# kalenforn/clip-based-cross-modal-hash

Hardware: AMD Instinct MI355X
Metric: Hamming query x gallery pairs/sec (fused mAP@all pass, DCMHT COCO-shaped 64-bit) (higher is better)
Workload: dtype u32; 1 GPU; configs[1] DCMHT COCO 64-bit retrieval: Q=5000 queries x R=117218 gallery items per GPU (x1 GPUs, contiguous shards), K=64 bits, C=80 classes, mAP@all; Q=5000, R_per_gpu=117218, K=64, C=80, parallelism=gallery-shard x1, query_blocks=1

## Files before the change

clip-based-cross-modal-hash_amd/csrc/xmh_scan.hip:

```cpp
#include "xmh_common.h"
#include <atomic>
#include <math.h>
#include <mutex>
#include <string.h>
#include <vector>
#include "xmh_scan_bits.h"
#include "xmh_scan_mfma.h"
#include "xmh_scan_kernels.h"

#include <stdlib.h>
#include <type_traits>

namespace {

constexpr int kSlotBudget64 = 9 * 1024;
constexpr int kSlotBudget32 = 5 * 1024;
constexpr int slots_for(int W, bool tern, int counter_bytes) {
    const int nbmax = (tern ? 64 : 32) * W + 1;
    const int budget = counter_bytes == 8 ? kSlotBudget64 : kSlotBudget32;
    const int cap = W > 8 ? 64 : 8;
    int S = 2;
    while (S < cap && nbmax * (64 / S) * counter_bytes > budget) S *= 2;
    return S;
}
inline int instance_words(int W) { return W <= 1 ? 1 : (W <= 2 ? 2 : (W <= 4 ? 4 : (W <= 8 ? 8 : (W <= 16 ? 16 : (W <= 32 ? 32 : 64))))); }
constexpr bool pair_cache_shape(int W, bool tern) { return !tern && (W == 1 || W == 2 || W == 4 || W == 8); }
template <int W, bool TERN>
constexpr bool kPairCacheShape = pair_cache_shape(W, TERN);
constexpr int cache_slots(int W) { return W <= 2 ? 4 : 8; }
static_assert(slots_for(2, false, 4) == 4 && slots_for(2, false, 8) == 4 && slots_for(4, false, 4) == 8 && slots_for(4, false, 8) == 8 &&
              slots_for(8, false, 4) == 8 && slots_for(8, false, 8) == 8, "33..256 bits: the cache geometry is the uncached kernels' own");
constexpr int waves_for(int W, bool tern) { return (W >= 32 && !tern) ? 8 : 1; }
inline size_t aos_ring_bytes(int W, int LW, bool tern) { return (size_t)64 * (((W * (tern ? 2 : 1) + LW) + 3) / 4 * 4) * 4; }

struct WsLayout {
    size_t chunk_hist, below, tot, dpre, cap, tick, gate, ap_part, pair_cache, total;
};

bool r2_selfcheck_ok();
inline bool mfma_env_on() {
    const char* e = getenv("XMH_SCAN_MFMA");
    return !(e && atoi(e) == 0);
}
struct Overrides {
    int mfma = -1;
    bool masked = false;
    bool describe = false;
};
enum class Family { kValu, kR2, kR2w, kBits, kTBits };
Family pass1_family(int K, bool ternary, const Overrides& ov) {
    if (ov.mfma == 0 || !mfma_env_on()) return Family::kValu;
    if (ternary) return K <= 256 ? Family::kTBits : Family::kValu;
    if (K > 128) return K <= 256 ? Family::kBits : Family::kValu;
    if (ov.mfma < 0 && !r2_selfcheck_ok()) return Family::kValu;
    return K <= 64 ? Family::kR2 : Family::kR2w;
}
inline int tbits_tiles(int K) { return K <= 64 ? 2 : (K <= 128 ? 4 : 8); }
inline int ap_r2_mode() {
    const char* e = getenv("XMH_SCAN_AP_R2");
    return e ? (atoi(e) != 0 ? 1 : 0) : 2;
}
constexpr int kAp2Waves = 4, kAp2Groups = 2;
constexpr int kMfmaWaves = 4;
static_assert(xmh::kScanBitsWaves == kMfmaWaves, "k_scan_hist_b takes the plan's query tiles of 64");
constexpr int kBitsMaxChunk = 24192;
struct R2Geom { int nw, nq, blocks_per_cu; int queries() const { return nw * nq * 16; } };
inline R2Geom r2_geom(int K) { return K <= 32 ? R2Geom{4, 4, 1} : (K <= 64 ? R2Geom{4, 4, 2} : R2Geom{4, 2, 2}); }

inline long long cache_cap_mb() {
    const char* cap_env = getenv("XMH_SCAN_CACHE_MB");
    return cap_env ? atoll(cap_env) : 131072;
}
inline bool ap_c_on() {
    const char* e = getenv("XMH_SCAN_AP_C");
    return !(e && atoi(e) == 0);
}
size_t pair_cache_bytes(const xmh_scan_plan& p, int K, bool ternary, Family f) {
    const long long cap_mb = cache_cap_mb();
    const bool tb = f == Family::kTBits;
    if ((ternary && !tb) || K > 256 || cap_mb <= 0 || (!tb && K <= 32 && f != Family::kR2)) return 0;
    if (f == Family::kR2 && ap_r2_mode() == 1) return 0;
    const int S = tb ? 8 : (K <= 64 ? 4 : 8);
    const size_t bytes = (size_t)p.nchunk * (size_t)(p.nqtile * S) * (size_t)((p.chunk + 63) / 64) * (S == 4 ? 1024 : 64 * 4 * xmh::kCache12Dwords);
    return bytes <= (size_t)cap_mb << 20 ? bytes : 0;
}

WsLayout ws_layout(const xmh_scan_plan& p, size_t cache_bytes) {
    WsLayout L;
    const size_t cells = (size_t)p.nchunk * p.nbuckets * p.qpad;
    size_t o = 0;
    auto take = [&](size_t bytes) {
        const size_t at = o;
        o += (bytes + 255) & ~(size_t)255;
        return at;
    };
    L.chunk_hist = take(cells * 4);
    L.below = take(cells * 8);
    L.tot = take((size_t)p.nbuckets * p.qpad * 8);
    L.dpre = take((size_t)p.nbuckets * p.qpad * 8);
    L.cap = take((size_t)p.qpad * 4);
    L.tick = take((size_t)p.nqtile * 4);
    L.gate = take(256 + 8 * 4096);
    L.ap_part = take((size_t)p.nchunk * p.qpad * 4);
    L.pair_cache = take(cache_bytes);
    L.total = o;
    return L;
}

size_t cache_for_workspace(const xmh_scan_plan& p, int K, bool ternary, Family f, size_t ws_bytes) {
    const size_t c = pair_cache_bytes(p, K, ternary, f);
    return c && ws_bytes < ws_layout(p, c).total ? 0 : c;
}

int make_plan(int64_t Q, int64_t R, int K, int ternary, xmh_scan_plan* p, const Overrides& ov = {}) {
    if (Q <= 0 || R <= 0 || K <= 0) return xmh::fail(XMH_EINVAL, "scan plan: bad shape Q=%lld R=%lld K=%d", (long long)Q, (long long)R, K);
    if (R >= (1ll << 24) || Q >= (1ll << 24)) return xmh::fail(XMH_ENOTSUP, "scan plan: shard too large (R=%lld, Q=%lld)", (long long)R, (long long)Q);
    const int64_t nb = ternary ? 2 * (int64_t)K + 1 : (int64_t)K + 1;
    const int Wd = (K + 31) / 32;
    if (Wd > 64 || (ternary && Wd > 8))
        return xmh::fail(XMH_ENOTSUP, "scan plan: K=%d%s (at most 2048 code bits, 256 with zero planes)", K, ternary ? " ternary" : "");
    const int S64 = slots_for(instance_words(Wd), ternary != 0, 8);
    const int64_t lds_ap = nb * (64 / S64) * 8;
    if (lds_ap > 150 * 1024) return xmh::fail(XMH_ENOTSUP, "scan plan: %lld distance buckets need %lld B of LDS per wave; K=%d%s", (long long)nb, (long long)lds_ap, K, ternary ? " ternary" : "");
    const Family fam = pass1_family(K, ternary != 0, ov);
    const bool r2 = fam == Family::kR2 || fam == Family::kR2w;
    int64_t nqt = xmh::ceil_div(Q, 64);
    const int r2q = r2_geom(K).queries();
    if (r2) {
        int64_t l = r2q;
        while (l % 64) l += r2q;
        nqt = xmh::ceil_div(nqt * 64, l) * l / 64;
    }
    const int64_t wpc = 8;
    const int64_t slots = (int64_t)xmh::device_cu_count() * wpc;
    const bool cache_shape = !ternary && K > 32 && K <= 64 && cache_cap_mb() > 0;
    const int64_t rounds = nb <= 33 ? 3 : (nb <= 65 && !cache_shape ? 2 : 1);
    int64_t nchunk = rounds * slots / nqt;
    if (S64 > 8) nchunk = nchunk * 8 / S64;
    const bool mfma = fam != Family::kValu;
    if (mfma) {
        int64_t bsets = nb <= 129 ? 6 : 3;
        if (const char* e = xmh_experiment_env("XMH_BITS_SETS")) bsets = atoi(e) > 0 ? atoi(e) : bsets;
        nchunk = bsets * xmh::device_cu_count() / nqt;
        if (r2) {
            int sets = K > 32 && K <= 64 ? 1 : 2;
            if (const char* e = xmh_experiment_env("XMH_R2_SETS")) sets = atoi(e) > 0 ? atoi(e) : sets;
            nchunk = (int64_t)sets * xmh::device_cu_count() * r2_geom(K).blocks_per_cu / (nqt * 64 / r2q);
        }
    }
    if (nchunk < 1) nchunk = 1;
    if (nchunk > 8) nchunk = (nchunk + 4) / 8 * 8;
    int64_t chunk = xmh::ceil_div(R, nchunk);
    if (chunk < kMinChunk) chunk = kMinChunk;
    if (chunk > kMaxChunk) chunk = kMaxChunk;
    chunk = xmh::ceil_div(chunk, 8) * 8;
    if (mfma) {
        chunk = xmh::ceil_div(chunk, 64) * 64;
        int64_t bits_max = kBitsMaxChunk;
        if (const char* e = xmh_experiment_env("XMH_BITS_MAX_CHUNK")) bits_max = atoll(e) / 64 * 64 > 0 ? atoll(e) / 64 * 64 : bits_max;
        if (!r2 && chunk > bits_max) {
            nchunk = xmh::ceil_div(xmh::ceil_div(R, bits_max), 8) * 8;
            chunk = xmh::ceil_div(xmh::ceil_div(R, nchunk), 64) * 64;
        }
    }
    nchunk = xmh::ceil_div(R, chunk);
    p->chunk = chunk;
    p->nchunk = nchunk;
    p->nqtile = nqt;
    p->qpad = nqt * 64;
    p->nbuckets = nb;
    p->ws_bytes = ws_layout(*p, pair_cache_bytes(*p, K, ternary != 0, fam)).total;
    return XMH_OK;
}

int lane_order_ok(hipStream_t st) {
    static int cached[64];
    static bool have[64];
    static std::mutex mu;
    int dev = 0;
    if (hipGetDevice(&dev) != hipSuccess || dev < 0 || dev >= 64) return 0;
    if (getenv("XMH_SCAN_MASKED") != nullptr) return 0;
    std::lock_guard<std::mutex> lock(mu);
    if (have[dev]) return cached[dev];
    int ok = 0;
    {
        const char* fe = getenv("XMH_SCAN_PROBE_FAULT");
        const int fault = fe && atoi(fe) != 0;
        uint32_t* flag = nullptr;
        float* sink = nullptr;
        if (hipMalloc(&flag, 8) == hipSuccess && hipMalloc(&sink, 256) == hipSuccess) {
            uint32_t h[2] = {0, 1};
            int cus = xmh::device_cu_count();
            if (hipMemsetAsync(flag, 0, 8, st) == hipSuccess) {
                hipLaunchKernelGGL(k_probe_lane_order, dim3(1), dim3(64), 0, st, flag);
                hipLaunchKernelGGL(k_probe_lane_order_load, dim3((unsigned)(cus * 25)), dim3(64), 0, st, flag + 1, fault, sink);
                if (hipGetLastError() == hipSuccess && hipMemcpyAsync(h, flag, 8, hipMemcpyDeviceToHost, st) == hipSuccess && hipStreamSynchronize(st) == hipSuccess)
                    ok = h[0] == 1u && h[1] == 0u;
            }
        }
        if (flag) (void)hipFree(flag);
        if (sink) (void)hipFree(sink);
        if (!ok)
            fprintf(stderr, "xmh: the lane-order probe FAILED on device %d%s: same-address returning LDS adds are not served in lane order here; "
                            "pass 2 runs the masked kernels (about 2x slower, same results).\n", dev, fault ? " (XMH_SCAN_PROBE_FAULT set: forced)" : "");
    }
    cached[dev] = ok;
    have[dev] = true;
    return ok;
}

struct DevBuf {
    void* p = nullptr;
    ~DevBuf() { if (p) (void)hipFree(p); }
    bool alloc(size_t n) { return hipMalloc(&p, n) == hipSuccess; }
    template <typename T> T* as() { return static_cast<T*>(p); }
};

template <bool TERN, typename F>
int dispatch_shape(int W, int LW, F&& f) {
#define XMH_CASE(WW, LL) \
    if (W == WW && LW == LL) return f(std::integral_constant<int, WW>{}, std::integral_constant<int, LL>{});
    XMH_CASE(1, 1) XMH_CASE(1, 2) XMH_CASE(1, 3) XMH_CASE(1, 4)
    XMH_CASE(2, 1) XMH_CASE(2, 2) XMH_CASE(2, 3) XMH_CASE(2, 4)
    XMH_CASE(4, 1) XMH_CASE(4, 2) XMH_CASE(4, 3) XMH_CASE(4, 4)
    XMH_CASE(8, 1) XMH_CASE(8, 2) XMH_CASE(8, 3) XMH_CASE(8, 4)
    if constexpr (!TERN) {
        XMH_CASE(1, 8) XMH_CASE(2, 8) XMH_CASE(4, 8) XMH_CASE(8, 8)
    }
    if constexpr (!TERN) {
        XMH_CASE(16, 1) XMH_CASE(16, 2) XMH_CASE(16, 3) XMH_CASE(16, 4)
        XMH_CASE(32, 1) XMH_CASE(32, 2) XMH_CASE(32, 3) XMH_CASE(32, 4)
        XMH_CASE(64, 1) XMH_CASE(64, 2) XMH_CASE(64, 3) XMH_CASE(64, 4)
    }
#undef XMH_CASE
    return xmh::fail(XMH_ENOTSUP, "scan: unsupported shape W=%d code words (K in {<=32,64,128,256}, binary also 512,1024,2048), Lw=%d label words (C<=128; binary codes up to 256 bits also exactly 8 words: 129..256 classes)%s",
                     W, LW, TERN ? ", ternary" : "");
}

int packed_rank_bits(int K, int64_t R) {
    const char* e = getenv("XMH_SCAN_PACK32");
    if (e && e[0] == '0') return 0;
    if (!(K > 64 || (e && e[0] == 'a'))) return 0;
    const int64_t rank_max = R + 2;
    int rank_bits = 0;
    while ((1ll << rank_bits) < rank_max) ++rank_bits;
    return rank_bits > 24 ? 0 : rank_bits;
}

enum class Mode { kUnsharded, kBaseAll, kTotals, kAllToAll };
struct ScanCall {
    const uint32_t *qbits, *qzero, *qlab, *rbits, *rzero, *rlab;
    int64_t Q, R; int K, C;
    void* ws; size_t ws_bytes;
    bool tern;
};
struct Pass2 {
    Mode mode; int64_t k;
    double* ap_sum; int32_t* cap;
    double* map_out;
    const uint32_t *base_all = nullptr, *base_rel = nullptr, *nrel_total = nullptr;
    const uint32_t* hist_g = nullptr;
    int world = 0, rank = 0;
};
enum class Kern { kHistS, kHistR2, kHistR2w, kHistB, kApS, kApC, kApR2 };
enum Gate : unsigned {
    kBySize = 1,
    kByWrap = 2,
    kByWidth = 4,
};
struct Launch {
    Kern kern = Kern::kHistS;
    int W = 0, LW = 0;
    bool tern = false, cache = false;
    int S = 0, NW = 1;
    int nml = 0;
    int eb = 0; bool half = false;
    bool p32 = false, masked = false;
    unsigned gate = 0;
    bool stand_in = false;
};
struct ScanRoute {
    Launch p1;
    size_t cache_bytes = 0;
    int rank_bits = 0;
    Launch p2[3];
    int n2 = 0;
};

ScanRoute scan_route(const xmh_scan_plan& p, const ScanCall& c, Mode mode, const Overrides& ov, hipStream_t st) {
    ScanRoute r;
    const int K = c.K, C = c.C; const bool tern = c.tern; const int64_t R = c.R;
    const Family fam = pass1_family(K, tern, ov);
    const int W = ov.describe ? instance_words((K + 31) / 32) : (K + 31) / 32, LW = (C + 31) / 32;
    const bool lane_ok = ov.describe || (!ov.masked && lane_order_ok(st));
    r.cache_bytes = cache_for_workspace(p, K, tern, fam, c.ws_bytes);
    const bool cache = r.cache_bytes != 0;
    const bool mfma = fam != Family::kValu && LW <= 4 && lane_ok;
    Launch& h = r.p1;
    h.W = W; h.LW = LW; h.tern = tern; h.cache = cache; h.nml = LW <= 2 ? 1 : 2;
    if (!mfma) {
        h.cache = cache && pair_cache_shape(W, tern);
        h.S = h.cache ? cache_slots(W) : slots_for(W, tern, 4);
        h.NW = h.S == 64 ? waves_for(W, tern) : 1;
    } else if (fam == Family::kBits || fam == Family::kTBits) {
        h.kern = Kern::kHistB;
        h.S = fam == Family::kTBits ? tbits_tiles(K) : 4;
    } else {
        const R2Geom g = r2_geom(K);
        h.kern = fam == Family::kR2 ? Kern::kHistR2 : Kern::kHistR2w;
        h.NW = g.nw; h.S = g.nq;
    }
    const bool sharded = mode != Mode::kUnsharded;
    const bool masked = !lane_ok;
    const int rank_bits = sharded || masked ? 0 : packed_rank_bits(K, R);
    const bool fits_fb = sharded || R <= kFloatBitsMaxItems;
    const bool apc_on = ap_c_on();
    const bool byte128 = cache && mfma && fam == Family::kR2w;
    const bool tb = cache && mfma && fam == Family::kTBits;
    const bool apc = cache && apc_on && (byte128 || (K <= 64 && rank_bits == 0)) && !tern && !masked && (mode != Mode::kBaseAll || byte128) && fits_fb;
    const bool apr2 = !cache && mfma && fam == Family::kR2 && ap_r2_mode() != 0 && !masked && mode != Mode::kBaseAll && rank_bits == 0 && fits_fb;
    const bool apc16 = cache && apc_on && ((K > 128 && K <= 256 && !tern) || tb) && !masked && !sharded && R <= kFloatBitsMaxItems;
    const unsigned size_gate = sharded && (apc || apr2) ? kBySize : 0u;
    r.rank_bits = byte128 && apc ? 0 : rank_bits;
    auto add = [&](Kern kern, unsigned gate) -> Launch& { Launch& l = r.p2[r.n2++]; l.kern = kern; l.gate = gate; return l; };
    if (apc) {
        Launch& l = add(Kern::kApC, size_gate | (byte128 ? kByWrap : 0u));
        l.eb = 8; l.half = byte128; l.S = byte128 ? 8 : 4;
    }
    if (apr2) {
        Launch& l = add(Kern::kApR2, size_gate);
        l.W = W; l.LW = LW; l.nml = h.nml; l.NW = kAp2Waves; l.S = kAp2Groups;
    }
    if (apc16) {
        Launch& l = add(Kern::kApC, kByWidth);
        l.eb = 16; l.S = 8;
    }
    if ((apc || apr2) && !size_gate && !byte128) return r;
    Launch s;
    s.kern = Kern::kApS; s.W = tb ? 8 : W; s.LW = LW; s.tern = tern && !tb; s.masked = masked;
    s.cache = cache && !byte128 && !masked && pair_cache_shape(s.W, s.tern);
    s.stand_in = byte128 && apc;
    s.gate = size_gate | (s.stand_in ? kByWrap : 0u) | (r.rank_bits ? kByWidth : 0u);
    for (const bool p32 : {true, false}) {
        if (p32 ? r.rank_bits == 0 : apc16) continue;
        s.p32 = p32;
        s.S = s.cache ? cache_slots(s.W) : slots_for(s.W, s.tern, p32 ? 4 : 8);
        s.NW = s.S == 64 ? waves_for(s.W, s.tern) : 1;
        r.p2[r.n2++] = s;
    }
    return r;
}

int describe_launch(const Launch& l, char* out, size_t n) {
    static const char* const tf[2] = {"false", "true"};
    auto exists = [&](auto tern_c) { return dispatch_shape<decltype(tern_c)::value>(l.W, l.LW, [](auto, auto) { return (int)XMH_OK; }); };
    switch (l.kern) {
    case Kern::kHistS:
    case Kern::kApS:
        if (const int rc = l.tern ? exists(std::true_type{}) : exists(std::false_type{})) return rc;
        if (l.kern == Kern::kHistS) snprintf(out, n, "k_scan_hist_s<%d, %d, %s, %d, %d, %s>", l.W, l.LW, tf[l.tern], l.S, l.NW, tf[l.cache]);
        else
            snprintf(out, n, "k_scan_ap_s<%d, %d, %s, %s, %d, %s, %s, %d, %s>", l.W, l.cache ? 1 : l.LW, tf[l.tern], tf[!l.cache], l.S, tf[l.p32], tf[l.masked],
                     l.NW, tf[l.cache]);
        break;
    case Kern::kHistR2:
    case Kern::kHistR2w:
        snprintf(out, n, "k_scan_hist_%s<%d, %d, %d, %s>", l.kern == Kern::kHistR2 ? "r2" : "r2w", l.nml, l.NW, l.S, tf[l.cache]);
        break;
    case Kern::kHistB: {
        int nsh, nqt;
        xmh::scan_hist_bits_shape(l.S, l.tern, &nsh, &nqt);
        snprintf(out, n, "k_scan_hist_b<%d, %d, %d, %d, %s, %s>", l.S, kMfmaWaves, nsh, nqt, tf[l.cache], tf[l.tern]);
        break;
    }
    case Kern::kApC: snprintf(out, n, "k_scan_ap_c<false, %d, %s>", l.eb, tf[l.half]); break;
    case Kern::kApR2: snprintf(out, n, "k_scan_ap_r2<%d, %d, %d, false>", l.nml, l.NW, l.S); break;
    }
    return XMH_OK;
}

int check_common(const char* who, const ScanCall& c, const xmh_scan_plan& p) {
    if (!c.qbits || !c.rbits || !c.qlab || !c.rlab || !c.ws) return xmh::fail(XMH_EINVAL, "%s: null pointer", who);
    if ((c.qzero == nullptr) != (c.rzero == nullptr)) return xmh::fail(XMH_EINVAL, "%s: zero masks must be given for both sides or neither", who);
    if (c.C <= 0) return xmh::fail(XMH_EINVAL, "%s: C=%d", who, c.C);
    const size_t need = ws_layout(p, 0).total;
    if (c.ws_bytes < need) return xmh::fail(XMH_EINVAL, "%s: workspace too small (%zu < %zu; %zu with the pair cache)", who, c.ws_bytes, need, (size_t)p.ws_bytes);
    return XMH_OK;
}

ScanArgs make_args(const ScanCall& c, const xmh_scan_plan& p) {
    return ScanArgs{c.qbits, c.qzero, c.qlab, c.rbits, c.rzero, c.rlab, (int)c.Q, (int)c.R, c.K, (int)p.chunk, (int)p.nchunk, (int)p.nqtile, (int)p.qpad,
                    (int)p.nbuckets, nullptr};
}

MfmaArgs r2_args(const ScanCall& c, const Launch& l, const xmh_scan_plan& p, int nqt) {
    MfmaArgs a{c.qbits, (int)c.Q, (int)c.R, c.K, l.W, (int)p.chunk, (int)p.nchunk, nqt, (int)p.nbuckets, (int)p.qpad};
    a.rbits = c.rbits; a.rlab = c.rlab; a.qlab = c.qlab; a.LW = l.LW;
    return a;
}

struct Geom { unsigned grid, block; size_t lds; int nqt; };
Geom launch_geom(const Launch& l, const xmh_scan_plan& p) {
    const size_t nb = (size_t)p.nbuckets;
    const bool ap = l.kern == Kern::kApS || l.kern == Kern::kApC || l.kern == Kern::kApR2;
    Geom g{0, 64u * (unsigned)l.NW, 0, 0};
    if (l.kern == Kern::kHistS || l.kern == Kern::kApS) {
        g.lds = ((nb * (64 / l.S) * (ap && !l.p32 ? 2 : 1) + 3) & ~(size_t)3) * 4 * l.NW + (ap && l.cache ? 0 : aos_ring_bytes(l.W, l.LW, l.tern));
        g.nqt = (int)p.nqtile * l.S / l.NW;
    } else if (l.kern == Kern::kApC) {
        g.lds = nb * (64 / l.S) * 8; g.nqt = (int)p.nqtile * l.S;
    } else if (l.kern == Kern::kHistB) {
        g.nqt = (int)(p.qpad / (16 * kMfmaWaves));
    } else {
        g.lds = (size_t)l.NW * l.S * nb * 16 * (ap ? 8 : 4); g.nqt = (int)(p.qpad / (l.NW * l.S * 16));
    }
    g.grid = (unsigned)(8 * g.nqt * xmh::ceil_div(p.nchunk, 8));
    return g;
}

template <typename KernT, typename... Args>
int start(const char* who, const Launch& l, const Geom& g, hipStream_t st, KernT kern, int S, int NW, bool cache, Args... args) {
    if (l.S != S || l.NW != NW || l.cache != cache)
        return xmh::fail(XMH_ENOTSUP, "%s: the route names an instance with S=%d NW=%d cache=%d, the one compiled for W=%d LW=%d has S=%d NW=%d cache=%d", who, l.S,
                         l.NW, (int)l.cache, l.W, l.LW, S, NW, (int)cache);
    if (const int rc = xmh::raise_dynamic_lds(reinterpret_cast<const void*>(kern), g.lds, who)) return rc;
    hipLaunchKernelGGL(kern, dim3(g.grid), dim3(g.block), g.lds, st, args...);
    return XMH_OK;
}

struct ScanCtx {
    const ScanCall& c;
    hipStream_t st;
    xmh_scan_plan p;
    ScanRoute r;
    WsLayout L;
    ScanArgs a;
    uint32_t kcap = 0xffffffffu;
    bool capped = false;
    template <typename T> T* at(size_t off) const { return reinterpret_cast<T*>(static_cast<char*>(c.ws) + off); }
    uint32_t* chunk_hist() const { return at<uint32_t>(L.chunk_hist); }
    const uint2* below() const { return at<uint2>(L.below); }
    uint2* tot() const { return at<uint2>(L.tot); }
    uint2* dpre() const { return at<uint2>(L.dpre); }
    uint32_t* cap_ws() const { return at<uint32_t>(L.cap); }
    float* ap_part() const { return at<float>(L.ap_part); }
    ScanArgs args(const Geom& g, bool cached) const { ScanArgs as = a; as.nqt = g.nqt; as.pair_cache = cached ? pair_cache() : nullptr; return as; }
    uint32_t* gate(int word = 0) const { return at<uint32_t>(L.gate) + word; }
    const uint32_t* gate_if(const Launch& l, unsigned g, int word) const { return (l.gate & g) ? gate(word) : nullptr; }
    uint4* pair_cache() const { return r.cache_bytes ? at<uint4>(L.pair_cache) : nullptr; }
};

int plan_call(const char* who, ScanCtx& x, const Overrides& ov) {
    if (const int rc = make_plan(x.c.Q, x.c.R, x.c.K, x.c.tern, &x.p, ov)) return rc;
    return check_common(who, x.c, x.p);
}
void route_call(ScanCtx& x, Mode mode, const Overrides& ov) {
    x.r = scan_route(x.p, x.c, mode, ov, x.st);
    x.a = make_args(x.c, x.p);
    x.L = ws_layout(x.p, x.r.cache_bytes);
}

int valu_hist(const ScanCtx& x) {
    const Launch& h = x.r.p1;
    const Geom g = launch_geom(h, x.p);
    const ScanArgs as = x.args(g, h.cache);
    auto go = [&](auto kern, int S, int NW, bool cache) {
        xmh::ProfScope prof("scan_hist", x.st);
        return start("xmh_hamming_hist", h, g, x.st, kern, S, NW, cache, as, x.chunk_hist());
    };
    auto launch = [&](auto tern_c) {
        constexpr bool T = decltype(tern_c)::value;
        return dispatch_shape<T>(h.W, h.LW, [&](auto w, auto l) {
            constexpr int WW = decltype(w)::value, LL = decltype(l)::value;
            if constexpr (kPairCacheShape<WW, T>) {
                if (h.cache) return go(k_scan_hist_s<WW, LL, T, cache_slots(WW), 1, true>, cache_slots(WW), 1, true);
            }
            constexpr int S = slots_for(WW, T, 4);
            constexpr int NW = S == 64 ? waves_for(WW, T) : 1;
            return go(k_scan_hist_s<WW, LL, T, S, NW, false>, S, NW, false);
        });
    };
    return h.tern ? launch(std::true_type{}) : launch(std::false_type{});
}

int mfma_hist(const ScanCtx& x) {
    const Launch& h = x.r.p1;
    const xmh_scan_plan& p = x.p;
    const Geom g = launch_geom(h, p);
    uint32_t* chunk_hist = x.chunk_hist();
    uint4* cache = x.pair_cache();
    if (h.kern == Kern::kHistB) {
        xmh::ScanBitsArgs a{x.c.rbits, x.c.rlab, x.c.qbits, x.c.qlab, (int)x.c.Q, (int)x.c.R, x.c.K, h.W, h.LW, (int)p.chunk, (int)p.nchunk, g.nqt,
                            (int)p.nbuckets, (int)p.qpad};
        a.rzero = x.c.rzero; a.qzero = x.c.qzero;
        return xmh::launch_scan_hist_bits(a, h.S, chunk_hist, cache, x.st);
    }
    hipLaunchKernelGGL(k_scan_touch, dim3((unsigned)(8 * kTouchPerChunk * xmh::ceil_div(p.nchunk, 8))), dim3(256), 0, x.st, x.c.rbits, x.c.rlab, x.c.R, h.W, h.LW,
                       p.chunk, (int)p.nchunk, x.at<uint32_t>(x.L.tick), (int)((x.L.gate + 256 - x.L.tick) / 4));
    XMH_LAUNCH_CHECK("xmh_hamming_hist control words");
    const MfmaArgs a = r2_args(x.c, h, p, g.nqt);
    xmh::ProfScope prof("scan_hist", x.st);
    auto go = [&](auto kern, int NW, int NQ, bool cached, auto... wrap_word) { return start("xmh_hamming_hist", h, g, x.st, kern, NQ, NW, cached, a, chunk_hist, cache, wrap_word...); };
    if (h.kern == Kern::kHistR2w) {
        uint32_t* ovf = x.gate(kGateWrapped);
        return h.nml == 1 ? (h.cache ? go(k_scan_hist_r2w<1, 4, 2, true>, 4, 2, true, ovf) : go(k_scan_hist_r2w<1, 4, 2, false>, 4, 2, false, ovf))
                          : (h.cache ? go(k_scan_hist_r2w<2, 4, 2, true>, 4, 2, true, ovf) : go(k_scan_hist_r2w<2, 4, 2, false>, 4, 2, false, ovf));
    }
    return h.nml == 1 ? (h.cache ? go(k_scan_hist_r2<1, 4, 4, true>, 4, 4, true) : go(k_scan_hist_r2<1, 4, 4, false>, 4, 4, false))
                      : (h.cache ? go(k_scan_hist_r2<2, 4, 4, true>, 4, 4, true) : go(k_scan_hist_r2<2, 4, 4, false>, 4, 4, false));
}

int hamming_hist_impl(const ScanCall& c, uint32_t* hist_all, uint32_t* hist_rel, xmh_stream_t stream, const Overrides& ov) {
    ScanCtx x{c, xmh::as_stream(stream)};
    if (const int rc = plan_call("xmh_hamming_hist", x, ov)) return rc;
    route_call(x, Mode::kUnsharded, ov);
    const xmh_scan_plan& p = x.p;
    const Kern kern = x.r.p1.kern;
    if (kern == Kern::kHistS || kern == Kern::kHistB) XMH_HIP(hipMemsetAsync(x.at<char>(x.L.tick), 0, x.L.gate + 256 - x.L.tick, x.st));
    if (const int rc = kern == Kern::kHistS ? valu_hist(x) : mfma_hist(x)) return rc;
    XMH_LAUNCH_CHECK("xmh_hamming_hist");
    hipLaunchKernelGGL(k_scan_below, dim3((unsigned)p.nqtile, (unsigned)xmh::ceil_div(p.nbuckets, 4)), dim3(256), 0, x.st, x.chunk_hist(), (int)p.qpad,
                       (int)p.nbuckets, (int)p.nchunk, kern != Kern::kHistS ? kRelHi16 : 0u, x.at<uint2>(x.L.below), x.tot(), x.at<uint32_t>(x.L.tick), (int)c.Q, x.dpre(),
                       x.cap_ws(), x.gate(), hist_all, hist_rel);
    XMH_LAUNCH_CHECK("xmh_hamming_hist below");
    return XMH_OK;
}

}

extern "C" int xmh_scan_plan_make(int64_t Q, int64_t R, int K, int ternary, xmh_scan_plan* plan_host) {
    if (!plan_host) return xmh::fail(XMH_EINVAL, "xmh_scan_plan_make: null plan");
    return make_plan(Q, R, K, ternary, plan_host);
}

extern "C" size_t xmh_scan_pair_cache_bytes(int64_t Q, int64_t R, int K, int ternary) {
    xmh_scan_plan p;
    if (make_plan(Q, R, K, ternary, &p)) return 0;
    return pair_cache_bytes(p, K, ternary != 0, pass1_family(K, ternary != 0, {}));
}

extern "C" size_t xmh_scan_pair_cache_offset(int64_t Q, int64_t R, int K, int ternary) {
    xmh_scan_plan p;
    if (make_plan(Q, R, K, ternary, &p)) return (size_t)-1;
    return ws_layout(p, 0).pair_cache;
}

extern "C" size_t xmh_scan_ws_bytes_nocache(int64_t Q, int64_t R, int K, int ternary) {
    xmh_scan_plan p;
    if (make_plan(Q, R, K, ternary, &p)) return 0;
    return ws_layout(p, 0).total;
}

extern "C" int xmh_scan_describe(int64_t Q, int64_t R, int K, int C, int ternary, char* out, size_t out_bytes) {
    if (!out || out_bytes < 64) return xmh::fail(XMH_EINVAL, "xmh_scan_describe: buffer too small");
    xmh_scan_plan p;
    if (const int rc = make_plan(Q, R, K, ternary, &p)) return rc;
    Overrides ov;
    ov.describe = true;
    const ScanCall c{nullptr, nullptr, nullptr, nullptr, nullptr, nullptr, Q, R, K, C, nullptr, (size_t)p.ws_bytes, ternary != 0};
    const ScanRoute r = scan_route(p, c, Mode::kUnsharded, ov, nullptr);
    char p1[160], p2[200] = "", one[120];
    if (const int rc = describe_launch(r.p1, p1, sizeof(p1))) return rc;
    for (const bool p32 : {true, false})
        for (int i = 0; i < r.n2; ++i) {
            if (r.p2[i].stand_in || r.p2[i].p32 != p32) continue;
            if (const int rc = describe_launch(r.p2[i], one, sizeof(one))) return rc;
            const size_t at = strlen(p2);
            snprintf(p2 + at, sizeof(p2) - at, "%s%s", at ? "|" : "", one);
        }
    if ((size_t)snprintf(out, out_bytes, "pass1=%s;pass2=%s", p1, p2) >= out_bytes) return xmh::fail(XMH_EINVAL, "xmh_scan_describe: buffer too small");
    return XMH_OK;
}

extern "C" int xmh_hamming_hist(const uint32_t* qbits, const uint32_t* qzero, const uint32_t* qlab,
                                const uint32_t* rbits, const uint32_t* rzero, const uint32_t* rlab, int64_t Q, int64_t R,
                                int K, int C, void* ws, size_t ws_bytes, uint32_t* hist_all, uint32_t* hist_rel,
                                xmh_stream_t stream) {
    XMH_RANGE("xmh_hamming_hist (pass 1)");
    const ScanCall c{qbits, qzero, qlab, rbits, rzero, rlab, Q, R, K, C, ws, ws_bytes, qzero != nullptr};
    return hamming_hist_impl(c, hist_all, hist_rel, stream, {});
}

namespace {
int ap_offsets(const ScanCtx& x, const Pass2& o) {
    const xmh_scan_plan& p = x.p;
    if (o.mode == Mode::kUnsharded) return XMH_OK;
    if (o.mode == Mode::kAllToAll)
        hipLaunchKernelGGL(k_shard_scatter_offsets, dim3((unsigned)xmh::ceil_div(p.qpad, 256), (unsigned)p.nbuckets + 1), dim3(256), 0, x.st,
                           reinterpret_cast<const uint2*>(o.hist_g), (int)p.nbuckets, (int)(p.qpad / o.world), (int)x.c.Q, (int)p.qpad, o.k, x.dpre(), x.cap_ws(),
                           o.cap, x.gate(2));
    else if (o.mode == Mode::kTotals)
        hipLaunchKernelGGL(k_shard_offsets_dpre, dim3((unsigned)p.nqtile), dim3(256), 0, x.st, reinterpret_cast<const uint2*>(o.hist_g), o.world, o.rank,
                           (int)x.c.Q, (int)p.qpad, (int)p.nbuckets, o.k, x.dpre(), x.cap_ws(), o.cap, x.gate(2));
    else
        hipLaunchKernelGGL(k_scan_dpre, dim3((unsigned)p.nqtile), dim3(256), 0, x.st, (const uint2*)x.tot(), (int)x.c.Q, (int)p.qpad, (int)p.nbuckets, o.base_all,
                           o.base_rel, o.nrel_total, o.k, x.dpre(), x.cap_ws(), o.cap, (uint32_t*)nullptr, (uint32_t*)nullptr, (uint32_t*)nullptr, x.gate(2));
    XMH_LAUNCH_CHECK(o.mode == Mode::kAllToAll ? "xmh_hamming_map_sharded_offsets scatter" : (o.mode == Mode::kTotals ? "xmh_hamming_map_sharded offsets" : "xmh_hamming_ap dpre"));
    return XMH_OK;
}

int ap_launch_c(const ScanCtx& x, const Launch& l) {
    const Geom g = launch_geom(l, x.p);
    const ScanArgs as = x.args(g, true);
    xmh::ProfScope prof("scan_ap", x.st);
    auto go = [&](auto kc, int S) {
        return start("xmh_hamming_ap", l, g, x.st, kc, S, 1, l.cache, as, x.below(), (const uint2*)x.dpre(), (const uint32_t*)x.cap_ws(), x.ap_part(),
                     x.gate_if(l, kBySize, 2), x.kcap, x.gate_if(l, kByWrap, kGateWrapped), x.gate_if(l, kByWidth, 0), l.gate & kByWidth ? x.r.rank_bits : 0);
    };
    if (l.eb == 16) return x.capped ? go(k_scan_ap_c<true, 16>, 8) : go(k_scan_ap_c<false, 16>, 8);
    if (l.half) return x.capped ? go(k_scan_ap_c<true, 8, true>, 8) : go(k_scan_ap_c<false, 8, true>, 8);
    return x.capped ? go(k_scan_ap_c<true, 8>, 4) : go(k_scan_ap_c<false, 8>, 4);
}

int ap_launch_r2(const ScanCtx& x, const Launch& l) {
    const Geom g = launch_geom(l, x.p);
    const MfmaArgs ma = r2_args(x.c, l, x.p, g.nqt);
    xmh::ProfScope prof("scan_ap", x.st);
    auto go = [&](auto kern) {
        return start("xmh_hamming_ap", l, g, x.st, kern, kAp2Groups, kAp2Waves, l.cache, ma, x.below(), (const uint2*)x.dpre(), (const uint32_t*)x.cap_ws(), x.ap_part(),
                     x.gate_if(l, kBySize, 2), x.kcap);
    };
    return l.nml == 1 ? (x.capped ? go(k_scan_ap_r2<1, kAp2Waves, kAp2Groups, true>) : go(k_scan_ap_r2<1, kAp2Waves, kAp2Groups, false>))
                      : (x.capped ? go(k_scan_ap_r2<2, kAp2Waves, kAp2Groups, true>) : go(k_scan_ap_r2<2, kAp2Waves, kAp2Groups, false>));
}

int ap_launch_s(const ScanCtx& x, const Launch& l) {
    const Geom g = launch_geom(l, x.p);
    const ScanArgs as = x.args(g, l.cache);
    auto go = [&](auto kern, int S, int NW, bool cache, const uint32_t* run_if) {
        xmh::ProfScope prof(l.p32 ? "scan_ap32" : "scan_ap", x.st);
        return start("xmh_hamming_ap", l, g, x.st, kern, S, NW, cache, as, x.below(), (const uint2*)x.dpre(), (const uint32_t*)x.cap_ws(), x.ap_part(),
                     (const uint32_t*)x.gate(), x.r.rank_bits, x.kcap, x.gate_if(l, kBySize, 2), run_if);
    };
    auto by_shape = [&](auto tern_c, auto cap_c, auto p32_c, auto masked_c) {
        constexpr bool T = decltype(tern_c)::value, CP = decltype(cap_c)::value, P32 = decltype(p32_c)::value, MK = decltype(masked_c)::value;
        return dispatch_shape<T>(l.W, l.LW, [&](auto w, auto lw) {
            constexpr int WW = decltype(w)::value, LL = decltype(lw)::value;
            if constexpr (P32 && MK) return xmh::fail(XMH_ENOTSUP, "xmh_hamming_ap: the masked fallback runs 64-bit counters only");
            else {
                if constexpr (kPairCacheShape<WW, T> && !MK) {
                    if (l.cache)
                        return go(k_scan_ap_s<WW, 1, T, CP, cache_slots(WW), P32, MK, 1, true>, cache_slots(WW), 1, true, nullptr);
                }
                (void)CP;
                constexpr int S = slots_for(WW, T, P32 ? 4 : 8);
                constexpr int NW = S == 64 ? waves_for(WW, T) : 1;
                return go(k_scan_ap_s<WW, LL, T, true, S, P32, MK, NW, false>, S, NW, false, x.gate_if(l, kByWrap, kGateWrapped));
            }
        });
    };
    using T1 = std::true_type; using T0 = std::false_type;
    auto by_mask = [&](auto t, auto c, auto w) { return l.masked ? by_shape(t, c, w, T1{}) : by_shape(t, c, w, T0{}); };
    auto by_width = [&](auto t, auto c) { return l.p32 ? by_mask(t, c, T1{}) : by_mask(t, c, T0{}); };
    auto by_cap = [&](auto t) { return x.capped ? by_width(t, T1{}) : by_width(t, T0{}); };
    return l.tern ? by_cap(T1{}) : by_cap(T0{});
}

int ap_reduce(const ScanCtx& x, const Pass2& o) {
    const int64_t Q = x.c.Q;
    const unsigned nred = (unsigned)xmh::ceil_div(Q, 64);
    if (o.map_out && nred <= 4096) {
        hipLaunchKernelGGL(k_ap_reduce_map, dim3(nred), dim3(256), 0, x.st, (const float*)x.ap_part(), (int)Q, (int)x.p.qpad, (int)x.p.nchunk,
                           (const uint32_t*)x.cap_ws(), x.kcap, o.cap, o.ap_sum, x.at<double>(x.L.gate + 256), x.gate(1), o.map_out);
        XMH_LAUNCH_CHECK("xmh_hamming_map reduce+finalize");
        return XMH_OK;
    }
    hipLaunchKernelGGL(k_ap_reduce, dim3(nred), dim3(256), 0, x.st, (const float*)x.ap_part(), (int)Q, (int)x.p.qpad, (int)x.p.nchunk, o.ap_sum,
                       o.mode != Mode::kUnsharded ? (const uint32_t*)nullptr : (const uint32_t*)x.cap_ws(), x.kcap, o.cap);
    XMH_LAUNCH_CHECK("xmh_hamming_ap reduce");
    if (o.map_out) {
        hipLaunchKernelGGL(k_map_finalize, dim3(1), dim3(256), 0, x.st, (const double*)o.ap_sum, (const int32_t*)o.cap, Q, o.map_out);
        XMH_LAUNCH_CHECK("xmh_hamming_map finalize");
    }
    return XMH_OK;
}

static std::atomic<int> g_verify{0};
constexpr int XMH_EVERIFY_CODE = -74;

int hamming_ap_impl(const ScanCall& c, const Pass2& o, xmh_stream_t stream, const Overrides& ov);

int verify_against_masked(const ScanCall& c, const Pass2& o, xmh_stream_t stream) {
    hipStream_t st = xmh::as_stream(stream);
    const int64_t Q = c.Q;
    std::vector<double> a1((size_t)Q), a0((size_t)Q);
    std::vector<int32_t> c1((size_t)Q), c0((size_t)Q);
    XMH_HIP(hipMemcpyAsync(a1.data(), o.ap_sum, (size_t)Q * 8, hipMemcpyDeviceToHost, st));
    XMH_HIP(hipMemcpyAsync(c1.data(), o.cap, (size_t)Q * 4, hipMemcpyDeviceToHost, st));
    XMH_HIP(hipStreamSynchronize(st));
    Overrides ov;
    ov.mfma = 0;
    ov.masked = true;
    xmh_scan_plan p;
    if (const int rc = make_plan(Q, c.R, c.K, c.tern, &p, ov)) return rc;
    const size_t small = ws_layout(p, 0).total;
    DevBuf ws2, ap2, cap2;
    if (!ws2.alloc(small) || !ap2.alloc((size_t)Q * 8) || !cap2.alloc((size_t)Q * 4))
        return xmh::fail(XMH_ENOMEM, "xmh_scan_verify: no room for the second evaluation (%zu bytes)", small);
    ScanCall again = c; again.ws = ws2.p; again.ws_bytes = small;
    const Pass2 o2{Mode::kUnsharded, o.k, ap2.as<double>(), cap2.as<int32_t>(), nullptr};
    if (const int rc = hamming_hist_impl(again, nullptr, nullptr, stream, ov)) return rc;
    if (const int rc = hamming_ap_impl(again, o2, stream, ov)) return rc;
    XMH_HIP(hipMemcpyAsync(a0.data(), ap2.p, (size_t)Q * 8, hipMemcpyDeviceToHost, st));
    XMH_HIP(hipMemcpyAsync(c0.data(), cap2.p, (size_t)Q * 4, hipMemcpyDeviceToHost, st));
    XMH_HIP(hipStreamSynchronize(st));
    if (const char* fe = getenv("XMH_SCAN_VERIFY_FAULT")) {
        const int64_t at = atoll(fe) % Q;
        a1[(size_t)at] *= 1.0 + 1e-3;
    }
    int64_t bad = -1, nbad = 0;
    for (int64_t i = 0; i < Q; ++i) {
        const bool same = c1[(size_t)i] == c0[(size_t)i] && fabs(a1[(size_t)i] - a0[(size_t)i]) <= 4e-6 * fabs(a0[(size_t)i]) + 1e-9;
        if (!same) { if (bad < 0) bad = i; ++nbad; }
    }
    if (nbad)
        return xmh::fail(XMH_EVERIFY_CODE, "xmh_scan_verify: %lld of %lld queries differ between the lane-order kernels and the masked re-derivation "
                         "(first: query %lld, AP sum %.9g vs %.9g, divisor %d vs %d)", (long long)nbad, (long long)Q, (long long)bad, a1[(size_t)bad], a0[(size_t)bad],
                         c1[(size_t)bad], c0[(size_t)bad]);
    return XMH_OK;
}

int hamming_ap_impl(const ScanCall& c, const Pass2& o, xmh_stream_t stream, const Overrides& ov) {
    ScanCtx x{c, xmh::as_stream(stream)};
    if (const int rc = plan_call("xmh_hamming_ap", x, ov)) return rc;
    if (!o.ap_sum || !o.cap) return xmh::fail(XMH_EINVAL, "xmh_hamming_ap: null output");
    const int ext = (o.base_all != nullptr) + (o.base_rel != nullptr) + (o.nrel_total != nullptr);
    if (ext != 0 && ext != 3) return xmh::fail(XMH_EINVAL, "xmh_hamming_ap: base_all, base_rel and nrel_total go together");
    route_call(x, o.mode, ov);
    x.kcap = o.k > 0 && o.k < (int64_t)0xffffffffll ? (uint32_t)o.k : 0xffffffffu;
    x.capped = o.k > 0;
    if (const int rc = ap_offsets(x, o)) return rc;
    for (int i = 0; i < x.r.n2; ++i) {
        const Launch& l = x.r.p2[i];
        if (const int rc = l.kern == Kern::kApC ? ap_launch_c(x, l) : (l.kern == Kern::kApR2 ? ap_launch_r2(x, l) : ap_launch_s(x, l))) return rc;
        XMH_LAUNCH_CHECK("xmh_hamming_ap");
    }
    if (const int rc = ap_reduce(x, o)) return rc;
    if (g_verify.load(std::memory_order_relaxed) && !ov.masked && o.mode == Mode::kUnsharded) return verify_against_masked(c, o, stream);
    return XMH_OK;
}

bool selfcheck_eval(const ScanCall& c, int force, std::vector<uint32_t>& hist, std::vector<double>& ap, std::vector<int32_t>& cap) {
    Overrides ov;
    ov.mfma = force;
    const int64_t Q = c.Q;
    xmh_scan_plan p;
    if (make_plan(Q, c.R, c.K, 0, &p, ov) != XMH_OK) return false;
    const size_t nb = (size_t)p.nbuckets;
    DevBuf ws, dh, dap, dcap;
    if (!ws.alloc(p.ws_bytes) || !dh.alloc(2 * Q * nb * 4) || !dap.alloc(Q * 8) || !dcap.alloc(Q * 4)) return false;
    ScanCall run = c; run.ws = ws.p; run.ws_bytes = p.ws_bytes;
    const Pass2 o{Mode::kUnsharded, 0, dap.as<double>(), dcap.as<int32_t>(), nullptr};
    uint32_t* h = dh.as<uint32_t>();
    if (hamming_hist_impl(run, h, h + Q * nb, nullptr, ov) != XMH_OK) return false;
    if (hamming_ap_impl(run, o, nullptr, ov) != XMH_OK) return false;
    hist.resize(2 * Q * nb); ap.resize(Q); cap.resize(Q);
    if (hipDeviceSynchronize() != hipSuccess) return false;
    return hipMemcpy(hist.data(), dh.p, hist.size() * 4, hipMemcpyDeviceToHost) == hipSuccess && hipMemcpy(ap.data(), dap.p, Q * 8, hipMemcpyDeviceToHost) == hipSuccess &&
           hipMemcpy(cap.data(), dcap.p, Q * 4, hipMemcpyDeviceToHost) == hipSuccess;
}

bool r2_selfcheck_ok() {
    static int state[64];
    static std::mutex mu;
    int dev = 0;
    if (hipGetDevice(&dev) != hipSuccess || dev < 0 || dev >= 64) return true;
    const char* e = getenv("XMH_SCAN_M2_SELFCHECK");
    if (e && atoi(e) == 0) return true;
    std::lock_guard<std::mutex> lock(mu);
    if (state[dev]) return state[dev] == 1;
    state[dev] = 1;
    const int64_t Q = 200, R = 9000;
    const int C = 80, LW = 3;
    bool same = true, ran = true;
    for (int K : {64, 40, 16, 100}) {
        const int W = (K + 31) / 32;
        std::vector<uint32_t> qb(Q * W), ql(Q * LW), rb(R * W), rl(R * LW);
        uint64_t x = 0x9E3779B97F4A7C15ull ^ (uint64_t)K;
        auto rnd = [&]() { x ^= x << 13; x ^= x >> 7; x ^= x << 17; return (uint32_t)(x >> 16); };
        const uint32_t last = K % 32 ? (1u << (K % 32)) - 1 : 0xffffffffu;
        for (auto& v : qb) v = rnd();
        for (int64_t i = 0; i < R; ++i)
            for (int w = 0; w < W; ++w) rb[i * W + w] = (i > 64 && (rnd() & 3) == 0) ? rb[(rnd() % 64) * W + w] : rnd();
        for (int64_t i = 0; i < Q; ++i) qb[i * W + W - 1] &= last;
        for (int64_t i = 0; i < R; ++i) rb[i * W + W - 1] &= last;
        for (int64_t i = 0; i < Q * LW; ++i) ql[i] = rnd() & rnd() & rnd() & (i % LW == LW - 1 ? 0xffffu : 0xffffffffu);
        for (int64_t i = 0; i < R * LW; ++i) rl[i] = rnd() & rnd() & rnd() & (i % LW == LW - 1 ? 0xffffu : 0xffffffffu);
        for (int64_t i = 0; i < Q; ++i) ql[i * LW] |= 1u;
        for (int64_t i = 0; i < R; i += 7) rl[i * LW] |= 1u;
        std::vector<uint32_t> h1, h0;
        std::vector<double> a1, a0;
        std::vector<int32_t> c1, c0;
        DevBuf dq, dql, dr, drl;
        auto up = [](DevBuf& d, const std::vector<uint32_t>& v) { return d.alloc(v.size() * 4) && hipMemcpy(d.p, v.data(), v.size() * 4, hipMemcpyHostToDevice) == hipSuccess; };
        if (!up(dq, qb) || !up(dql, ql) || !up(dr, rb) || !up(drl, rl)) { ran = false; break; }
        const ScanCall c{dq.as<uint32_t>(), nullptr, dql.as<uint32_t>(), dr.as<uint32_t>(), nullptr, drl.as<uint32_t>(), Q, R, K, C, nullptr, 0, false};
        if (!selfcheck_eval(c, 1, h1, a1, c1) || !selfcheck_eval(c, 0, h0, a0, c0)) { ran = false; break; }
        bool ap_close = true;
        for (int64_t i = 0; i < Q; ++i) ap_close = ap_close && fabs(a1[i] - a0[i]) <= 4e-6 * fabs(a0[i]) + 1e-9;
        if (h1 != h0 || c1 != c0 || !ap_close) { same = false; break; }
    }
    if (e && atoi(e) == 2) same = false;
    if (!ran) {
        state[dev] = 0;
        return true;
    }
    if (!same) {
        state[dev] = 2;
        fprintf(stderr, "xmh: k_scan_hist_r2 self-check FAILED on device %d (results differ from the VALU kernels): falling back to the VALU scan "
                        "for this process.  Please report the hipcc / ROCm versions.\n", dev);
    }
    return state[dev] == 1;
}
}

extern "C" int xmh_scan_verify(int on) {
    g_verify.store(on != 0 ? 1 : 0, std::memory_order_relaxed);
    return XMH_OK;
}

extern "C" int xmh_hamming_ap(const uint32_t* qbits, const uint32_t* qzero, const uint32_t* qlab, const uint32_t* rbits,
                              const uint32_t* rzero, const uint32_t* rlab, int64_t Q, int64_t R, int K, int C, void* ws,
                              size_t ws_bytes, const uint32_t* base_all, const uint32_t* base_rel,
                              const uint32_t* nrel_total, int64_t k, double* ap_sum, int32_t* cap, xmh_stream_t stream) {
    XMH_RANGE("xmh_hamming_ap (pass 2)");
    const ScanCall c{qbits, qzero, qlab, rbits, rzero, rlab, Q, R, K, C, ws, ws_bytes, qzero != nullptr};
    Pass2 o{base_all ? Mode::kBaseAll : Mode::kUnsharded, k, ap_sum, cap, nullptr};
    o.base_all = base_all; o.base_rel = base_rel; o.nrel_total = nrel_total;
    return hamming_ap_impl(c, o, stream, {});
}

extern "C" int xmh_hamming_map(const uint32_t* qbits, const uint32_t* qzero, const uint32_t* qlab, const uint32_t* rbits,
                               const uint32_t* rzero, const uint32_t* rlab, int64_t Q, int64_t R, int K, int C, void* ws,
                               size_t ws_bytes, int64_t k, double* ap_sum, int32_t* cap, double* map_out, xmh_stream_t stream) {
    XMH_RANGE("xmh_hamming_map (pass 2 + mean)");
    if (!map_out) return xmh::fail(XMH_EINVAL, "xmh_hamming_map: null output");
    const ScanCall c{qbits, qzero, qlab, rbits, rzero, rlab, Q, R, K, C, ws, ws_bytes, qzero != nullptr};
    return hamming_ap_impl(c, Pass2{Mode::kUnsharded, k, ap_sum, cap, map_out}, stream, {});
}

extern "C" size_t xmh_scan_totals_offset(int64_t Q, int64_t R, int K, int ternary, size_t* bytes) {
    xmh_scan_plan p;
    if (make_plan(Q, R, K, ternary, &p)) return (size_t)-1;
    if (bytes) *bytes = (size_t)p.nbuckets * p.qpad * 8;
    return ws_layout(p, 0).tot;
}

extern "C" int xmh_hamming_map_sharded(const uint32_t* qbits, const uint32_t* qzero, const uint32_t* qlab, const uint32_t* rbits,
                                       const uint32_t* rzero, const uint32_t* rlab, int64_t Q, int64_t R, int K, int C, void* ws,
                                       size_t ws_bytes, const uint32_t* hist_gathered, int world, int rank, int64_t k, double* ap_sum,
                                       int32_t* cap, double* map_partial, xmh_stream_t stream) {
    XMH_RANGE("xmh_hamming_map_sharded (pass 2)");
    if (!hist_gathered || !map_partial) return xmh::fail(XMH_EINVAL, "xmh_hamming_map_sharded: null pointer");
    if (world <= 0 || rank < 0 || rank >= world) return xmh::fail(XMH_EINVAL, "xmh_hamming_map_sharded: bad world=%d rank=%d", world, rank);
    const ScanCall c{qbits, qzero, qlab, rbits, rzero, rlab, Q, R, K, C, ws, ws_bytes, qzero != nullptr};
    Pass2 o{Mode::kTotals, k, ap_sum, cap, map_partial};
    o.hist_g = hist_gathered; o.world = world; o.rank = rank;
    return hamming_ap_impl(c, o, stream, {});
}

extern "C" int xmh_shard_slice_offsets(const uint32_t* totals_slices, int world, int nbuckets, int slice, uint32_t* offsets_out, xmh_stream_t stream) {
    XMH_RANGE("xmh_shard_slice_offsets");
    if (!totals_slices || !offsets_out) return xmh::fail(XMH_EINVAL, "xmh_shard_slice_offsets: null pointer");
    if (world <= 0 || nbuckets <= 0 || slice <= 0) return xmh::fail(XMH_EINVAL, "xmh_shard_slice_offsets: bad arguments (world=%d nb=%d slice=%d)", world, nbuckets, slice);
    hipLaunchKernelGGL(k_shard_slice_offsets, dim3((unsigned)xmh::ceil_div(slice, 64)), dim3(256), 0, xmh::as_stream(stream),
                       reinterpret_cast<const uint2*>(totals_slices), world, nbuckets, slice, reinterpret_cast<uint2*>(offsets_out));
    XMH_LAUNCH_CHECK("xmh_shard_slice_offsets");
    return XMH_OK;
}

extern "C" int xmh_hamming_map_sharded_offsets(const uint32_t* qbits, const uint32_t* qzero, const uint32_t* qlab, const uint32_t* rbits,
                                               const uint32_t* rzero, const uint32_t* rlab, int64_t Q, int64_t R, int K, int C, void* ws,
                                               size_t ws_bytes, const uint32_t* offsets, int world, int64_t k, double* ap_sum, int32_t* cap,
                                               double* map_partial, xmh_stream_t stream) {
    XMH_RANGE("xmh_hamming_map_sharded_offsets (pass 2)");
    if (!offsets || !map_partial) return xmh::fail(XMH_EINVAL, "xmh_hamming_map_sharded_offsets: null pointer");
    const ScanCall c{qbits, qzero, qlab, rbits, rzero, rlab, Q, R, K, C, ws, ws_bytes, qzero != nullptr};
    xmh_scan_plan p;
    if (const int rc = make_plan(Q, R, K, c.tern, &p)) return rc;
    if (world <= 0 || p.qpad % world) return xmh::fail(XMH_EINVAL, "xmh_hamming_map_sharded_offsets: qpad=%lld is not a multiple of world=%d", (long long)p.qpad, world);
    Pass2 o{Mode::kAllToAll, k, ap_sum, cap, map_partial};
    o.hist_g = offsets; o.world = world;
    return hamming_ap_impl(c, o, stream, {});
}

extern "C" int xmh_map_finalize(const double* ap_sum, const int32_t* cap, int64_t Q, double* map_out, xmh_stream_t stream) {
    XMH_RANGE("xmh_map_finalize");
    if (!ap_sum || !cap || !map_out || Q <= 0) return xmh::fail(XMH_EINVAL, "xmh_map_finalize: bad arguments");
    hipLaunchKernelGGL(k_map_finalize, dim3(1), dim3(256), 0, xmh::as_stream(stream), ap_sum, cap, Q, map_out);
    XMH_LAUNCH_CHECK("xmh_map_finalize");
    return XMH_OK;
}

extern "C" int xmh_shard_offsets(const uint32_t* hist_gathered, int world, int rank, int64_t Q, int nbuckets, uint32_t* base_all,
                                 uint32_t* base_rel, uint32_t* nrel_total, xmh_stream_t stream) {
    XMH_RANGE("xmh_shard_offsets");
    if (!hist_gathered || !base_all || !base_rel || !nrel_total) return xmh::fail(XMH_EINVAL, "xmh_shard_offsets: null pointer");
    if (world <= 0 || rank < 0 || rank >= world || Q <= 0 || nbuckets <= 0 || Q >= (1ll << 24))
        return xmh::fail(XMH_EINVAL, "xmh_shard_offsets: bad arguments (world=%d rank=%d Q=%lld nb=%d)", world, rank, (long long)Q, nbuckets);
    hipLaunchKernelGGL(k_shard_offsets, dim3((unsigned)Q), dim3(64), 0, xmh::as_stream(stream), hist_gathered, world, rank, (int)Q, nbuckets,
                       base_all, base_rel, nrel_total);
    XMH_LAUNCH_CHECK("xmh_shard_offsets");
    return XMH_OK;
}
```

clip-based-cross-modal-hash_amd/csrc/xmh_scan_mfma.h:

```cpp
#pragma once
#include "xmh_common.h"
#include <type_traits>

namespace {

constexpr int kMaxChunk = 32768;
constexpr uint32_t kF23 = 0x4B000000u;
constexpr int64_t kFloatBitsMaxItems = (1ll << 23) - 3;
constexpr int kMinChunk = 256;

struct ScanArgs {
    const uint32_t* qbits;
    const uint32_t* qzero;
    const uint32_t* qlab;
    const uint32_t* rbits;
    const uint32_t* rzero;
    const uint32_t* rlab;
    int Q, R, K;
    int chunk, nchunk, nqt, qpad, nb;
    uint4* pair_cache;
};

__device__ __forceinline__ bool map_block(const ScanArgs& a, int& chunk_id, int& qtile) {
    const int b = blockIdx.x;
    const int xcd = b & 7;
    const int t = b >> 3;
    qtile = t % a.nqt;
    chunk_id = xcd + 8 * (t / a.nqt);
    return chunk_id < a.nchunk;
}

typedef int v4i __attribute__((ext_vector_type(4)));

struct MfmaArgs {
    const uint32_t* qbits;
    int Q, R, K, W;
    int chunk, nchunk, nqt, nb, qpad;
    const uint32_t* rbits = nullptr;
    const uint32_t* rlab = nullptr;
    const uint32_t* qlab = nullptr;
    int LW = 0;
};

__device__ __forceinline__ bool mfma_map_block(const MfmaArgs& a, int& chunk_id, int& qtile) {
    const int b = blockIdx.x;
    const int xcd = b & 7, t = b >> 3;
    qtile = t % a.nqt;
    chunk_id = xcd + 8 * (t / a.nqt);
    return chunk_id < a.nchunk;
}

template <int NML, int NW, int NQ, bool CACHE>
__device__ __forceinline__ void scan_hist_r2_body(const MfmaArgs& a, uint32_t* __restrict__ chunk_hist, uint4* __restrict__ pair_cache) {
    constexpr int NMI = 1 + NML, NMQ = 2 + NML;
    constexpr bool REGS = true;
    extern __shared__ __attribute__((aligned(16))) uint32_t lds[];
    int chunk_id, qtile;
    if (!mfma_map_block(a, chunk_id, qtile)) return;
    const int lane = threadIdx.x & 63, wave = threadIdx.x >> 6;
    const int ql = lane & 15, slot = lane >> 4;
    const int t16 = (qtile * NW + wave) * NQ;
    const int ncell = a.nb * 16;
    uint32_t* cnt = lds + (wave * NQ) * ncell;
    for (int e = lane; e < NQ * ncell; e += 64) cnt[e] = 0u;
    v4i bq[NQ][NMQ], cq[NQ], kqv[REGS ? NQ : 1];
    bool valid[NQ];
    const int rsh = 4 * (slot & 1), rwi = slot >> 1;
#pragma unroll
    for (int h = 0; h < NQ; ++h) {
        valid[h] = (t16 + h) * 16 + ql < a.Q;
        int pcq = 0;
        {
            const int64_t q = (int64_t)(t16 + h) * 16 + ql;
            uint32_t qw = 0u;
            if (valid[h]) {
                for (int w = 0; w < a.W; ++w) pcq += __popc(a.qbits[q * a.W + w]);
                if (rwi < a.W) qw = a.qbits[q * a.W + rwi];
            }
            qw >>= rsh;
#pragma unroll
            for (int j = 0; j < 4; ++j) {
                const uint32_t t = (qw >> j) & 0x01010101u;
                const bool on = valid[h] && rwi < a.W;
                if (j & 1) {
                    bq[h][0][j] = on ? (int)(0x20202020u ^ (t * 0xc0u)) : 0;
                    bq[h][1][j] = on ? (int)(0x01010101u ^ (t * 0xfeu)) : 0;
                } else {
                    bq[h][0][j] = on ? (int)(0x40404040u ^ (t << 7)) : 0;
                    bq[h][1][j] = on ? (int)(0x02020202u ^ (t * 0xfcu)) : 0;
                }
            }
#pragma unroll
            for (int m = 0; m < NML; ++m) {
                uint32_t lw = 0u;
                if (valid[h] && 2 * m + rwi < a.LW) lw = a.qlab[q * a.LW + 2 * m + rwi];
                lw >>= rsh;
#pragma unroll
                for (int j = 0; j < 4; ++j) bq[h][2 + m][j] = (int)((lw >> j) & 0x01010101u);
            }
            const int k2 = 2 * pcq;
            kqv[h] = v4i{k2, k2, k2, k2};
        }
        const int c0 = (int)(uint32_t)(uintptr_t)(__attribute__((address_space(3))) uint32_t*)(cnt + h * ncell) + ql * 4 + (valid[h] ? 64 * pcq : 0);
        cq[h] = v4i{c0, c0, c0, c0};
    }
    v4i lab0 = {0x10000, 0x10000, 0x10000, 0x10000};
    asm volatile("" : "+v"(lab0));
#pragma unroll
    for (int h = 0; h < NQ; ++h) asm volatile("" : "+v"(cq[h]));
#pragma unroll
    for (int h = 0; h < (REGS ? NQ : 1); ++h) asm volatile("" : "+v"(kqv[h]));
    const int64_t lo = (int64_t)chunk_id * a.chunk;
    const int64_t hi = (lo + a.chunk < a.R) ? lo + a.chunk : a.R;
    const int nbat = (int)((hi - lo + 63) >> 6);
    const int64_t bat0 = lo >> 6;
    uint4* crow[NQ];
#pragma unroll
    for (int h = 0; h < NQ; ++h)
        crow[h] = CACHE ? pair_cache + ((int64_t)chunk_id * (a.qpad >> 4) + (t16 + h)) * ((a.chunk + 63) >> 6) * 64 + lane : nullptr;
    uint32_t wcur[4][NMI], wnxt[4][NMI];
    const int ritem = 4 * (lane & 3) + ((lane & 15) >> 2);
    const int wi_c = rwi < a.W ? rwi : a.W - 1;
    int wi_l[NML];
#pragma unroll
    for (int m = 0; m < NML; ++m) wi_l[m] = 2 * m + rwi < a.LW ? 2 * m + rwi : (a.LW > 0 ? a.LW - 1 : 0);
    auto load_words = [&](int64_t batch, uint32_t (&w)[4][NMI]) {
        const int64_t first = batch * 64;
        if (first + 64 <= (int64_t)a.R) {
            const uint32_t* __restrict__ pc = a.rbits + (first + ritem) * a.W + wi_c;
            const uint32_t* __restrict__ pl = a.rlab + (first + ritem) * a.LW;
#pragma unroll
            for (int g = 0; g < 4; ++g) {
                w[g][0] = pc[g * 16 * a.W];
#pragma unroll
                for (int m = 0; m < NML; ++m) w[g][1 + m] = pl[g * 16 * a.LW + wi_l[m]];
            }
        } else {
#pragma unroll
            for (int g = 0; g < 4; ++g) {
                const int64_t item = first + g * 16 + ritem;
                const int64_t it = item < a.R ? item : (int64_t)a.R - 1;
                const uint32_t ok = item < a.R ? 0xffffffffu : 0u;
                w[g][0] = a.rbits[it * a.W + wi_c] & ok;
#pragma unroll
                for (int m = 0; m < NML; ++m) w[g][1 + m] = a.rlab[it * a.LW + wi_l[m]] & ok;
            }
        }
    };
    auto build = [&](v4i (&At)[NMI], const uint32_t (&w)[NMI]) {
        const uint32_t xa = w[0] >> rsh, xb = w[0] >> (rsh + 2);
        At[0][0] = (int)(xa & 0x01010101u);
        At[0][1] = (int)(xa & 0x02020202u);
        At[0][2] = (int)(xb & 0x01010101u);
        At[0][3] = (int)(xb & 0x02020202u);
#pragma unroll
        for (int m = 1; m < NMI; ++m) {
            const uint32_t y = w[m] >> rsh;
#pragma unroll
            for (int j = 0; j < 4; ++j) At[m][j] = (int)(y & (0x01010101u << j));
        }
    };
    load_words(bat0, wcur);
#ifdef XMH_ABL_NOBUILD
    v4i A[4][NMI];
#endif
    for (int i = 0; i < nbat; ++i) {
#ifdef XMH_ABL_NOLOADW
        if (i == 0) load_words(bat0, wnxt);
#else
        load_words(bat0 + (i + 1 < nbat ? i + 1 : i), wnxt);
#endif
#ifndef XMH_ABL_NOBUILD
        v4i A[REGS ? 4 : 2][NMI];
#endif
        uint32_t cw[NQ][4];
        v4i addr_p, d2_p, lab_p;
#ifndef XMH_R2_NOPS
#define XMH_R2_NOPS 0
#endif
#if XMH_R2_NOPS == 0
#define XMH_R2_OPEN "s_nop 3\n\t"
#define XMH_R2_EVAL_CLOSE "s_nop 7"
#define XMH_R2_TAIL "s_nop 7\n\ts_nop 3"
#elif XMH_R2_NOPS == 1
#define XMH_R2_OPEN "s_nop 1\n\t"
#define XMH_R2_EVAL_CLOSE "s_nop 7"
#define XMH_R2_TAIL "s_nop 7\n\ts_nop 3"
#elif XMH_R2_NOPS == 2
#define XMH_R2_OPEN ""
#define XMH_R2_EVAL_CLOSE "s_nop 7"
#define XMH_R2_TAIL "s_nop 7\n\ts_nop 3"
#elif XMH_R2_NOPS == 3
#define XMH_R2_OPEN "s_nop 1\n\t"
#define XMH_R2_EVAL_CLOSE "s_nop 3"
#define XMH_R2_TAIL "s_nop 1"
#else
#define XMH_R2_OPEN ""
#define XMH_R2_EVAL_CLOSE "s_nop 3"
#define XMH_R2_TAIL "s_nop 1"
#endif
#ifdef XMH_ABL_NOMIN
#define XMH_VMIN "; "
#else
#define XMH_VMIN "v_min_u32 "
#endif
#ifdef XMH_ABL_MINFULL
#undef XMH_VMIN
#define XMH_VMIN "v_and_b32 "
#endif
#ifdef XMH_ABL_NOADD
#define XMH_ADD(A, D) "s_nop 0\n\t"
#else
#define XMH_ADD(A, D) "ds_add_u32 " A ", " D "\n\t"
#endif
#ifdef XMH_ABL_NOMFMA
#define XMH_MFMA(D, A, B, C) "s_nop 0\n\t"
#else
#define XMH_MFMA(D, A, B, C) "v_mfma_i32_16x16x64_i8 " D ", " A ", " B ", " C "\n\t"
#endif
#define XMH_SDWA(J) "dst_sel:BYTE_" #J " dst_unused:UNUSED_PRESERVE src0_sel:BYTE_0 src1_sel:BYTE_0\n\t"
        auto fused = [&](const v4i (&At)[NMI], int h, v4i& addr, v4i& d2, v4i& lab, uint32_t& w) {
            uint32_t i0, i1, i2, i3;
            if (NML == 2 && CACHE) {
                asm volatile(
                    XMH_R2_OPEN XMH_MFMA("%0", "%8", "%9", "%10")
                    XMH_VMIN "%4, 0x10001, %26\n\t" XMH_VMIN "%5, 0x10001, %27\n\t" XMH_VMIN "%6, 0x10001, %28\n\t"
                    XMH_MFMA("%0", "%11", "%12", "%0")
                    XMH_VMIN "%7, 0x10001, %29\n\t"
                    "v_or_b32_sdwa %3, %18, %4 dst_sel:BYTE_0 dst_unused:UNUSED_PAD src0_sel:BYTE_0 src1_sel:BYTE_0\n\t"
                    XMH_ADD("%22", "%4")
                    XMH_MFMA("%1", "%13", "%14", "%15")
                    "v_or_b32_sdwa %3, %19, %5 " XMH_SDWA(1) XMH_ADD("%23", "%5") "v_or_b32_sdwa %3, %20, %6 " XMH_SDWA(2)
                    XMH_MFMA("%2", "%13", "%16", "%17")
                    XMH_ADD("%24", "%6") "v_or_b32_sdwa %3, %21, %7 " XMH_SDWA(3) XMH_ADD("%25", "%7")
                    : "=&v"(lab), "=&v"(addr), "=&v"(d2), "=&v"(w), "=&v"(i0), "=&v"(i1), "=&v"(i2), "=&v"(i3)
                    : "v"(At[1]), "v"(bq[h][2]), "v"(lab0), "v"(At[NMI - 1]), "v"(bq[h][NMQ - 1]), "v"(At[0]), "v"(bq[h][0]), "v"(cq[h]), "v"(bq[h][1]), "v"(kqv[REGS ? h : 0]),
                      "v"(d2_p[0]), "v"(d2_p[1]), "v"(d2_p[2]), "v"(d2_p[3]), "v"(addr_p[0]), "v"(addr_p[1]), "v"(addr_p[2]), "v"(addr_p[3]),
                      "v"(lab_p[0]), "v"(lab_p[1]), "v"(lab_p[2]), "v"(lab_p[3])
                    : "memory");
            } else if (NML == 2) {
                asm volatile(
                    XMH_R2_OPEN XMH_MFMA("%0", "%6", "%7", "%8")
                    XMH_VMIN "%2, 0x10001, %18\n\t" XMH_VMIN "%3, 0x10001, %19\n\t" XMH_VMIN "%4, 0x10001, %20\n\t"
                    XMH_MFMA("%0", "%9", "%10", "%0")
                    XMH_VMIN "%5, 0x10001, %21\n\t" XMH_ADD("%14", "%2") XMH_ADD("%15", "%3")
                    XMH_MFMA("%1", "%11", "%12", "%13")
                    XMH_ADD("%16", "%4") XMH_ADD("%17", "%5")
                    : "=&v"(lab), "=&v"(addr), "=&v"(i0), "=&v"(i1), "=&v"(i2), "=&v"(i3)
                    : "v"(At[1]), "v"(bq[h][2]), "v"(lab0), "v"(At[NMI - 1]), "v"(bq[h][NMQ - 1]), "v"(At[0]), "v"(bq[h][0]), "v"(cq[h]),
                      "v"(addr_p[0]), "v"(addr_p[1]), "v"(addr_p[2]), "v"(addr_p[3]), "v"(lab_p[0]), "v"(lab_p[1]), "v"(lab_p[2]), "v"(lab_p[3])
                    : "memory");
            } else if (CACHE) {
                asm volatile(
                    XMH_R2_OPEN XMH_MFMA("%0", "%8", "%9", "%10")
                    XMH_VMIN "%4, 0x10001, %24\n\t" XMH_VMIN "%5, 0x10001, %25\n\t" XMH_VMIN "%6, 0x10001, %26\n\t" XMH_VMIN "%7, 0x10001, %27\n\t"
                    "v_or_b32_sdwa %3, %16, %4 dst_sel:BYTE_0 dst_unused:UNUSED_PAD src0_sel:BYTE_0 src1_sel:BYTE_0\n\t"
                    XMH_ADD("%20", "%4")
                    XMH_MFMA("%1", "%11", "%12", "%13")
                    "v_or_b32_sdwa %3, %17, %5 " XMH_SDWA(1) XMH_ADD("%21", "%5") "v_or_b32_sdwa %3, %18, %6 " XMH_SDWA(2)
                    XMH_MFMA("%2", "%11", "%14", "%15")
                    XMH_ADD("%22", "%6") "v_or_b32_sdwa %3, %19, %7 " XMH_SDWA(3) XMH_ADD("%23", "%7")
                    : "=&v"(lab), "=&v"(addr), "=&v"(d2), "=&v"(w), "=&v"(i0), "=&v"(i1), "=&v"(i2), "=&v"(i3)
                    : "v"(At[1]), "v"(bq[h][2]), "v"(lab0), "v"(At[0]), "v"(bq[h][0]), "v"(cq[h]), "v"(bq[h][1]), "v"(kqv[REGS ? h : 0]),
                      "v"(d2_p[0]), "v"(d2_p[1]), "v"(d2_p[2]), "v"(d2_p[3]), "v"(addr_p[0]), "v"(addr_p[1]), "v"(addr_p[2]), "v"(addr_p[3]),
                      "v"(lab_p[0]), "v"(lab_p[1]), "v"(lab_p[2]), "v"(lab_p[3])
                    : "memory");
            } else {
                asm volatile(
                    XMH_R2_OPEN XMH_MFMA("%0", "%6", "%7", "%8")
                    XMH_VMIN "%2, 0x10001, %16\n\t" XMH_VMIN "%3, 0x10001, %17\n\t" XMH_VMIN "%4, 0x10001, %18\n\t" XMH_VMIN "%5, 0x10001, %19\n\t"
                    XMH_MFMA("%1", "%9", "%10", "%11")
                    XMH_ADD("%12", "%2") XMH_ADD("%13", "%3") XMH_ADD("%14", "%4") XMH_ADD("%15", "%5")
                    : "=&v"(lab), "=&v"(addr), "=&v"(i0), "=&v"(i1), "=&v"(i2), "=&v"(i3)
                    : "v"(At[1]), "v"(bq[h][2]), "v"(lab0), "v"(At[0]), "v"(bq[h][0]), "v"(cq[h]),
                      "v"(addr_p[0]), "v"(addr_p[1]), "v"(addr_p[2]), "v"(addr_p[3]), "v"(lab_p[0]), "v"(lab_p[1]), "v"(lab_p[2]), "v"(lab_p[3])
                    : "memory");
            }
        };
        auto evaluate = [&](const v4i (&At)[NMI], int h, v4i& addr, v4i& d2, v4i& lab) {
            if (NML == 2 && CACHE) {
                asm volatile(XMH_R2_OPEN XMH_MFMA("%0", "%3", "%4", "%5") XMH_MFMA("%0", "%6", "%7", "%0")
                             XMH_MFMA("%1", "%8", "%9", "%10") XMH_MFMA("%2", "%8", "%11", "%12") XMH_R2_EVAL_CLOSE
                             : "=&v"(lab), "=&v"(addr), "=&v"(d2)
                             : "v"(At[1]), "v"(bq[h][2]), "v"(lab0), "v"(At[NMI - 1]), "v"(bq[h][NMQ - 1]), "v"(At[0]), "v"(bq[h][0]), "v"(cq[h]),
                               "v"(bq[h][1]), "v"(kqv[REGS ? h : 0]));
            } else if (NML == 2) {
                asm volatile(XMH_R2_OPEN XMH_MFMA("%0", "%2", "%3", "%4") XMH_MFMA("%0", "%5", "%6", "%0")
                             XMH_MFMA("%1", "%7", "%8", "%9") XMH_R2_EVAL_CLOSE
                             : "=&v"(lab), "=&v"(addr)
                             : "v"(At[1]), "v"(bq[h][2]), "v"(lab0), "v"(At[NMI - 1]), "v"(bq[h][NMQ - 1]), "v"(At[0]), "v"(bq[h][0]), "v"(cq[h]));
            } else if (CACHE) {
                asm volatile(XMH_R2_OPEN XMH_MFMA("%0", "%3", "%4", "%5") XMH_MFMA("%1", "%6", "%7", "%8")
                             XMH_MFMA("%2", "%6", "%9", "%10") XMH_R2_EVAL_CLOSE
                             : "=&v"(lab), "=&v"(addr), "=&v"(d2)
                             : "v"(At[1]), "v"(bq[h][2]), "v"(lab0), "v"(At[0]), "v"(bq[h][0]), "v"(cq[h]), "v"(bq[h][1]), "v"(kqv[REGS ? h : 0]));
            } else {
                asm volatile(XMH_R2_OPEN XMH_MFMA("%0", "%2", "%3", "%4") XMH_MFMA("%1", "%5", "%6", "%7") XMH_R2_EVAL_CLOSE
                             : "=&v"(lab), "=&v"(addr)
                             : "v"(At[1]), "v"(bq[h][2]), "v"(lab0), "v"(At[0]), "v"(bq[h][0]), "v"(cq[h]));
            }
        };
        auto consume = [&](uint32_t& w, const v4i (&live)[NMI]) {
            uint32_t i0, i1, i2, i3;
            if (CACHE) {
                asm volatile(
                    XMH_VMIN "%1, 0x10001, %5\n\t" XMH_VMIN "%2, 0x10001, %6\n\t" XMH_VMIN "%3, 0x10001, %7\n\t" XMH_VMIN "%4, 0x10001, %8\n\t"
                    "v_or_b32_sdwa %0, %9, %1 dst_sel:BYTE_0 dst_unused:UNUSED_PAD src0_sel:BYTE_0 src1_sel:BYTE_0\n\t"
                    XMH_ADD("%13", "%1")
                    "v_or_b32_sdwa %0, %10, %2 " XMH_SDWA(1) XMH_ADD("%14", "%2") "v_or_b32_sdwa %0, %11, %3 " XMH_SDWA(2)
                    XMH_ADD("%15", "%3") "v_or_b32_sdwa %0, %12, %4 " XMH_SDWA(3) XMH_ADD("%16", "%4")
                    : "=&v"(w), "=&v"(i0), "=&v"(i1), "=&v"(i2), "=&v"(i3)
                    : "v"(lab_p[0]), "v"(lab_p[1]), "v"(lab_p[2]), "v"(lab_p[3]), "v"(d2_p[0]), "v"(d2_p[1]), "v"(d2_p[2]), "v"(d2_p[3]), "v"(addr_p[0]),
                      "v"(addr_p[1]), "v"(addr_p[2]), "v"(addr_p[3]), "v"(live[0]), "v"(live[1]), "v"(live[NMI - 1])
                    : "memory");
            } else {
                asm volatile(
                    XMH_VMIN "%0, 0x10001, %4\n\t" XMH_VMIN "%1, 0x10001, %5\n\t" XMH_VMIN "%2, 0x10001, %6\n\t" XMH_VMIN "%3, 0x10001, %7\n\t"
                    XMH_ADD("%8", "%0") XMH_ADD("%9", "%1") XMH_ADD("%10", "%2") XMH_ADD("%11", "%3")
                    : "=&v"(i0), "=&v"(i1), "=&v"(i2), "=&v"(i3)
                    : "v"(lab_p[0]), "v"(lab_p[1]), "v"(lab_p[2]), "v"(lab_p[3]), "v"(addr_p[0]), "v"(addr_p[1]), "v"(addr_p[2]), "v"(addr_p[3]), "v"(live[0]),
                      "v"(live[1]), "v"(live[NMI - 1])
                    : "memory");
            }
        };
#undef XMH_SDWA
#undef XMH_ADD
#undef XMH_MFMA
        auto group = [&](auto gc) {
            constexpr int G = decltype(gc)::value;
            constexpr int SET = REGS ? G : (G & 1);
#pragma unroll
            for (int h = 0; h < NQ; ++h) {
                v4i addr, d2, lab;
                if (G == 0 && h == 0) evaluate(A[SET], h, addr, d2, lab);
                else fused(A[SET], h, addr, d2, lab, cw[(h + NQ - 1) % NQ][h == 0 ? G - 1 : G]);
                addr_p = addr; d2_p = d2; lab_p = lab;
                if (REGS && G > 0 && h == 0) {
                    if constexpr (NMI == 2) asm volatile("" ::"v"(A[REGS ? G - 1 : 0][0]), "v"(A[REGS ? G - 1 : 0][1]));
                    else asm volatile("" ::"v"(A[REGS ? G - 1 : 0][0]), "v"(A[REGS ? G - 1 : 0][1]), "v"(A[REGS ? G - 1 : 0][NMI - 1]));
                }
            }
        };
#ifdef XMH_ABL_NOBUILD
        if (i == 0) {
#endif
        build(A[0], wcur[0]);
        build(A[1], wcur[1]);
        build(A[2], wcur[2]);
        build(A[3], wcur[3]);
#ifdef XMH_ABL_NOBUILD
        }
#endif
        group(std::integral_constant<int, 0>{});
        group(std::integral_constant<int, 1>{});
        group(std::integral_constant<int, 2>{});
        group(std::integral_constant<int, 3>{});
        asm volatile(XMH_R2_TAIL ::: "memory");
        consume(cw[NQ - 1][3], A[3]);
#ifdef XMH_ABL_NOSTORE
        if (CACHE && a.Q < 0) {
#else
        if (CACHE) {
#endif
#pragma unroll
            for (int h = 0; h < NQ; ++h) {
                uint4* dst = crow[h] + (int64_t)i * 64;
                __builtin_nontemporal_store(cw[h][0], &dst->x);
                __builtin_nontemporal_store(cw[h][1], &dst->y);
                __builtin_nontemporal_store(cw[h][2], &dst->z);
                __builtin_nontemporal_store(cw[h][3], &dst->w);
            }
        }
#pragma unroll
        for (int g = 0; g < 4; ++g)
#pragma unroll
            for (int m = 0; m < NMI; ++m) wcur[g][m] = wnxt[g][m];
    }
    const int npad = nbat * 64 - (int)(hi - lo);
    asm volatile("s_waitcnt lgkmcnt(0)" ::: "memory");
    if (npad > 0 && slot == 0) {
#pragma unroll
        for (int h = 0; h < NQ; ++h) {
            if (!valid[h]) continue;
            const int64_t q = (int64_t)(t16 + h) * 16 + ql;
            int dpad = 0;
            for (int w = 0; w < a.W; ++w) dpad += __popc(a.qbits[q * a.W + w]);
            cnt[h * ncell + dpad * 16 + ql] -= (uint32_t)npad << 16;
        }
    }
#pragma unroll
    for (int h = 0; h < NQ; ++h) {
        uint32_t* __restrict__ out = chunk_hist + ((int64_t)chunk_id * a.nb) * a.qpad + (t16 + h) * 16;
        for (int e = lane; e < ncell; e += 64) out[(int64_t)(e >> 4) * a.qpad + (e & 15)] = cnt[h * ncell + e];
    }
}

constexpr int kTouchPerChunk = 8;
__global__ __launch_bounds__(256) void k_scan_touch(const uint32_t* __restrict__ rbits, const uint32_t* __restrict__ rlab, int64_t R, int W, int LW, int64_t chunk,
                                                    int nchunk, uint32_t* __restrict__ ctl, int ctl_words) {
    if (blockIdx.x == 0)
        for (int e = threadIdx.x; e < ctl_words; e += 256) ctl[e] = 0u;
    const int b = blockIdx.x;
    const int c = (b & 7) + 8 * ((b >> 3) / kTouchPerChunk), sub = (b >> 3) % kTouchPerChunk;
    if (c >= nchunk) return;
    const int64_t lo = (int64_t)c * chunk, hi = lo + chunk < R ? lo + chunk : R;
    uint32_t acc = 0u;
    auto sweep = [&](const uint32_t* base, int64_t w0, int64_t w1) {
        for (int64_t w = w0 + ((int64_t)sub * 256 + threadIdx.x) * 32; w < w1; w += (int64_t)kTouchPerChunk * 256 * 32) acc ^= base[w];
    };
    sweep(rbits, lo * W, hi * W);
    sweep(rlab, lo * LW, hi * LW);
    asm volatile("" ::"v"(acc));
}

#ifndef XMH_R2_ATTR
#define XMH_R2_ATTR
#endif
template <int NML, int NW, int NQ, bool CACHE>
__global__ __launch_bounds__(64 * NW) XMH_R2_ATTR void k_scan_hist_r2(MfmaArgs a, uint32_t* __restrict__ chunk_hist, uint4* __restrict__ pair_cache) {
    scan_hist_r2_body<NML, NW, NQ, CACHE>(a, chunk_hist, pair_cache);
}

#define XMH_W_MFMA(D, A, B, C) "v_mfma_i32_16x16x64_i8 %[" D "], %[" A "], %[" B "], %[" C "]\n\t"
#define XMH_W_MIN(I, L) "v_min_u32 %[" I "], 0x10001, %[" L "]\n\t"
#define XMH_W_ADD(A, D) "ds_add_u32 %[" A "], %[" D "]\n\t"
template <int NML, int NW, int NQ, bool CACHE>
__global__ __launch_bounds__(64 * NW) void k_scan_hist_r2w(MfmaArgs a, uint32_t* __restrict__ chunk_hist, uint4* __restrict__ pair_cache,
                                                           uint32_t* __restrict__ ovf) {
    constexpr int NMC = 2, NMI = NMC + NML;
    extern __shared__ __attribute__((aligned(16))) uint32_t lds[];
    int chunk_id, qtile;
    if (!mfma_map_block(a, chunk_id, qtile)) return;
    const int lane = threadIdx.x & 63, wave = threadIdx.x >> 6;
    const int ql = lane & 15, slot = lane >> 4;
    const int t16 = (qtile * NW + wave) * NQ;
    const int ncell = a.nb * 16;
    uint32_t* cnt = lds + (wave * NQ) * ncell;
    for (int e = lane; e < NQ * ncell; e += 64) cnt[e] = 0u;
    const int rsh = 4 * (slot & 1), rwi = slot >> 1;
    v4i bA[NQ][NMC], bD[NQ][NMC], bL[NQ][NML], cq[NQ], kq[NQ];
    bool valid[NQ];
#pragma unroll
    for (int h = 0; h < NQ; ++h) {
        const int64_t q = (int64_t)(t16 + h) * 16 + ql;
        valid[h] = q < a.Q;
        int pcq = 0;
        if (valid[h])
            for (int w = 0; w < a.W; ++w) pcq += __popc(a.qbits[q * a.W + w]);
#pragma unroll
        for (int c = 0; c < NMC; ++c) {
            const int wi = 2 * c + rwi;
            const bool on = valid[h] && wi < a.W;
            const uint32_t qw = (on ? a.qbits[q * a.W + wi] : 0u) >> rsh;
#pragma unroll
            for (int j = 0; j < 4; ++j) {
                const uint32_t t = (qw >> j) & 0x01010101u;
                if (j & 1) {
                    bA[h][c][j] = on ? (int)(0x20202020u ^ (t * 0xc0u)) : 0;
                    bD[h][c][j] = on ? (int)(0x01010101u ^ (t * 0xfeu)) : 0;
                } else {
                    bA[h][c][j] = on ? (int)(0x40404040u ^ (t << 7)) : 0;
                    bD[h][c][j] = on ? (int)(0x02020202u ^ (t * 0xfcu)) : 0;
                }
            }
        }
#pragma unroll
        for (int m = 0; m < NML; ++m) {
            uint32_t lw = 0u;
            if (valid[h] && 2 * m + rwi < a.LW) lw = a.qlab[q * a.LW + 2 * m + rwi];
            lw >>= rsh;
#pragma unroll
            for (int j = 0; j < 4; ++j) bL[h][m][j] = (int)((lw >> j) & 0x01010101u);
        }
        const int c0 = (int)(uint32_t)(uintptr_t)(__attribute__((address_space(3))) uint32_t*)(cnt + h * ncell) + ql * 4 + (valid[h] ? 64 * pcq : 0);
        const int k2 = valid[h] ? 2 * pcq : 0;
        cq[h] = v4i{c0, c0, c0, c0};
        kq[h] = v4i{k2, k2, k2, k2};
    }
    v4i lab0 = {0x10000, 0x10000, 0x10000, 0x10000};
    asm volatile("" : "+v"(lab0));
#pragma unroll
    for (int h = 0; h < NQ; ++h) asm volatile("" : "+v"(cq[h]), "+v"(kq[h]));
    const int64_t lo = (int64_t)chunk_id * a.chunk;
    const int64_t hi = (lo + a.chunk < a.R) ? lo + a.chunk : a.R;
    const int nbat = (int)((hi - lo + 63) >> 6);
    const int64_t bat0 = lo >> 6;
    uint4* crow[NQ];
#pragma unroll
    for (int h = 0; h < NQ; ++h)
        crow[h] = CACHE ? pair_cache + ((int64_t)chunk_id * (a.qpad >> 4) + (t16 + h)) * ((a.chunk + 63) >> 6) * 64 + lane : nullptr;
    uint32_t wcur[4][NMI], wnxt[4][NMI];
    const int ritem = 4 * (lane & 3) + ((lane & 15) >> 2);
    int wi_c[NMC], wi_l[NML];
#pragma unroll
    for (int c = 0; c < NMC; ++c) wi_c[c] = 2 * c + rwi < a.W ? 2 * c + rwi : a.W - 1;
#pragma unroll
    for (int m = 0; m < NML; ++m) wi_l[m] = 2 * m + rwi < a.LW ? 2 * m + rwi : (a.LW > 0 ? a.LW - 1 : 0);
    auto load_words = [&](int64_t batch, uint32_t (&w)[4][NMI]) {
        const int64_t first = batch * 64;
        if (first + 64 <= (int64_t)a.R) {
            const uint32_t* __restrict__ pc = a.rbits + (first + ritem) * a.W;
            const uint32_t* __restrict__ pl = a.rlab + (first + ritem) * a.LW;
#pragma unroll
            for (int g = 0; g < 4; ++g) {
#pragma unroll
                for (int c = 0; c < NMC; ++c) w[g][c] = pc[g * 16 * a.W + wi_c[c]];
#pragma unroll
                for (int m = 0; m < NML; ++m) w[g][NMC + m] = pl[g * 16 * a.LW + wi_l[m]];
            }
        } else {
#pragma unroll
            for (int g = 0; g < 4; ++g) {
                const int64_t item = first + g * 16 + ritem;
                const int64_t it = item < a.R ? item : (int64_t)a.R - 1;
                const uint32_t ok = item < a.R ? 0xffffffffu : 0u;
#pragma unroll
                for (int c = 0; c < NMC; ++c) w[g][c] = a.rbits[it * a.W + wi_c[c]] & ok;
#pragma unroll
                for (int m = 0; m < NML; ++m) w[g][NMC + m] = a.rlab[it * a.LW + wi_l[m]] & ok;
            }
        }
    };
    auto build = [&](v4i (&At)[NMI], const uint32_t (&w)[NMI]) {
#pragma unroll
        for (int c = 0; c < NMC; ++c) {
            const uint32_t xa = w[c] >> rsh, xb = w[c] >> (rsh + 2);
            At[c][0] = (int)(xa & 0x01010101u);
            At[c][1] = (int)(xa & 0x02020202u);
            At[c][2] = (int)(xb & 0x01010101u);
            At[c][3] = (int)(xb & 0x02020202u);
        }
#pragma unroll
        for (int m = 0; m < NML; ++m) {
            const uint32_t y = w[NMC + m] >> rsh;
#pragma unroll
            for (int j = 0; j < 4; ++j) At[NMC + m][j] = (int)(y & (0x01010101u << j));
        }
    };
    uint32_t dmax = 0u;
    load_words(bat0, wcur);
    for (int i = 0; i < nbat; ++i) {
        load_words(bat0 + (i + 1 < nbat ? i + 1 : i), wnxt);
        v4i A[4][NMI];
        uint32_t cw[NQ][4];
        v4i addr_p = {0, 0, 0, 0}, d2_p = {0, 0, 0, 0}, lab_p = {0, 0, 0, 0};
        auto fused = [&](const v4i (&At)[NMI], int h, v4i& addr, v4i& d2, v4i& lab, uint32_t& i0, uint32_t& i1, uint32_t& i2, uint32_t& i3) {
            if (NML == 2 && CACHE) {
                asm volatile("s_nop 3\n\t" XMH_W_MFMA("lab", "al0", "bl0", "lab0") XMH_W_MIN("i0", "lp0") XMH_W_MIN("i1", "lp1") XMH_W_MIN("i2", "lp2")
                             XMH_W_MFMA("lab", "al1", "bl1", "lab") XMH_W_MIN("i3", "lp3") XMH_W_ADD("ap0", "i0") XMH_W_MFMA("addr", "a0", "ba0", "cq")
                             XMH_W_ADD("ap1", "i1") XMH_W_MFMA("addr", "a1", "ba1", "addr") XMH_W_ADD("ap2", "i2") XMH_W_MFMA("d2", "a0", "bd0", "kq")
                             XMH_W_ADD("ap3", "i3") XMH_W_MFMA("d2", "a1", "bd1", "d2")
                             : [lab] "=&v"(lab), [addr] "=&v"(addr), [d2] "=&v"(d2), [i0] "=&v"(i0), [i1] "=&v"(i1), [i2] "=&v"(i2), [i3] "=&v"(i3)
                             : [a0] "v"(At[0]), [a1] "v"(At[1]), [al0] "v"(At[2]), [al1] "v"(At[NMI - 1]), [ba0] "v"(bA[h][0]), [ba1] "v"(bA[h][1]),
                               [bd0] "v"(bD[h][0]), [bd1] "v"(bD[h][1]), [bl0] "v"(bL[h][0]), [bl1] "v"(bL[h][NML - 1]), [lab0] "v"(lab0), [cq] "v"(cq[h]),
                               [kq] "v"(kq[h]), [lp0] "v"(lab_p[0]), [lp1] "v"(lab_p[1]), [lp2] "v"(lab_p[2]), [lp3] "v"(lab_p[3]), [ap0] "v"(addr_p[0]),
                               [ap1] "v"(addr_p[1]), [ap2] "v"(addr_p[2]), [ap3] "v"(addr_p[3])
                             : "memory");
            } else if (NML == 2) {
                asm volatile("s_nop 3\n\t" XMH_W_MFMA("lab", "al0", "bl0", "lab0") XMH_W_MIN("i0", "lp0") XMH_W_MIN("i1", "lp1") XMH_W_MIN("i2", "lp2")
                             XMH_W_MFMA("lab", "al1", "bl1", "lab") XMH_W_MIN("i3", "lp3") XMH_W_ADD("ap0", "i0") XMH_W_ADD("ap1", "i1")
                             XMH_W_MFMA("addr", "a0", "ba0", "cq") XMH_W_ADD("ap2", "i2") XMH_W_ADD("ap3", "i3") XMH_W_MFMA("addr", "a1", "ba1", "addr")
                             : [lab] "=&v"(lab), [addr] "=&v"(addr), [i0] "=&v"(i0), [i1] "=&v"(i1), [i2] "=&v"(i2), [i3] "=&v"(i3)
                             : [a0] "v"(At[0]), [a1] "v"(At[1]), [al0] "v"(At[2]), [al1] "v"(At[NMI - 1]), [ba0] "v"(bA[h][0]), [ba1] "v"(bA[h][1]),
                               [bl0] "v"(bL[h][0]), [bl1] "v"(bL[h][NML - 1]), [lab0] "v"(lab0), [cq] "v"(cq[h]), [lp0] "v"(lab_p[0]), [lp1] "v"(lab_p[1]),
                               [lp2] "v"(lab_p[2]), [lp3] "v"(lab_p[3]), [ap0] "v"(addr_p[0]), [ap1] "v"(addr_p[1]), [ap2] "v"(addr_p[2]), [ap3] "v"(addr_p[3])
                             : "memory");
            } else if (CACHE) {
                asm volatile("s_nop 3\n\t" XMH_W_MFMA("lab", "al0", "bl0", "lab0") XMH_W_MIN("i0", "lp0") XMH_W_MIN("i1", "lp1") XMH_W_MIN("i2", "lp2")
                             XMH_W_MIN("i3", "lp3") XMH_W_ADD("ap0", "i0") XMH_W_MFMA("addr", "a0", "ba0", "cq") XMH_W_ADD("ap1", "i1")
                             XMH_W_MFMA("addr", "a1", "ba1", "addr") XMH_W_ADD("ap2", "i2") XMH_W_MFMA("d2", "a0", "bd0", "kq") XMH_W_ADD("ap3", "i3")
                             XMH_W_MFMA("d2", "a1", "bd1", "d2")
                             : [lab] "=&v"(lab), [addr] "=&v"(addr), [d2] "=&v"(d2), [i0] "=&v"(i0), [i1] "=&v"(i1), [i2] "=&v"(i2), [i3] "=&v"(i3)
                             : [a0] "v"(At[0]), [a1] "v"(At[1]), [al0] "v"(At[2]), [ba0] "v"(bA[h][0]), [ba1] "v"(bA[h][1]), [bd0] "v"(bD[h][0]),
                               [bd1] "v"(bD[h][1]), [bl0] "v"(bL[h][0]), [lab0] "v"(lab0), [cq] "v"(cq[h]), [kq] "v"(kq[h]), [lp0] "v"(lab_p[0]),
                               [lp1] "v"(lab_p[1]), [lp2] "v"(lab_p[2]), [lp3] "v"(lab_p[3]), [ap0] "v"(addr_p[0]), [ap1] "v"(addr_p[1]), [ap2] "v"(addr_p[2]),
                               [ap3] "v"(addr_p[3])
                             : "memory");
            } else {
                asm volatile("s_nop 3\n\t" XMH_W_MFMA("lab", "al0", "bl0", "lab0") XMH_W_MIN("i0", "lp0") XMH_W_MIN("i1", "lp1") XMH_W_MIN("i2", "lp2")
                             XMH_W_MIN("i3", "lp3") XMH_W_ADD("ap0", "i0") XMH_W_ADD("ap1", "i1") XMH_W_MFMA("addr", "a0", "ba0", "cq") XMH_W_ADD("ap2", "i2")
                             XMH_W_ADD("ap3", "i3") XMH_W_MFMA("addr", "a1", "ba1", "addr")
                             : [lab] "=&v"(lab), [addr] "=&v"(addr), [i0] "=&v"(i0), [i1] "=&v"(i1), [i2] "=&v"(i2), [i3] "=&v"(i3)
                             : [a0] "v"(At[0]), [a1] "v"(At[1]), [al0] "v"(At[2]), [ba0] "v"(bA[h][0]), [ba1] "v"(bA[h][1]), [bl0] "v"(bL[h][0]), [lab0] "v"(lab0),
                               [cq] "v"(cq[h]), [lp0] "v"(lab_p[0]), [lp1] "v"(lab_p[1]), [lp2] "v"(lab_p[2]), [lp3] "v"(lab_p[3]), [ap0] "v"(addr_p[0]),
                               [ap1] "v"(addr_p[1]), [ap2] "v"(addr_p[2]), [ap3] "v"(addr_p[3])
                             : "memory");
            }
        };
        auto pack = [&](uint32_t& w, const v4i& d, uint32_t i0, uint32_t i1, uint32_t i2, uint32_t i3) {
            uint32_t wb;
            asm volatile("v_or_b32_sdwa %[wa], %[d0], %[i0] dst_sel:BYTE_0 dst_unused:UNUSED_PAD src0_sel:BYTE_0 src1_sel:BYTE_0\n\t"
                         "v_or_b32_sdwa %[wb], %[d1], %[i1] dst_sel:BYTE_1 dst_unused:UNUSED_PAD src0_sel:BYTE_0 src1_sel:BYTE_0\n\t"
                         "v_max3_u32 %[mx], %[d0], %[d1], %[mx]\n\t"
                         "v_or_b32_sdwa %[wa], %[d2], %[i2] dst_sel:BYTE_2 dst_unused:UNUSED_PRESERVE src0_sel:BYTE_0 src1_sel:BYTE_0\n\t"
                         "v_or_b32_sdwa %[wb], %[d3], %[i3] dst_sel:BYTE_3 dst_unused:UNUSED_PRESERVE src0_sel:BYTE_0 src1_sel:BYTE_0\n\t"
                         "v_max3_u32 %[mx], %[d2], %[d3], %[mx]\n\t"
                         "v_or_b32 %[wa], %[wa], %[wb]"
                         : [wa] "=&v"(w), [wb] "=&v"(wb), [mx] "+v"(dmax)
                         : [d0] "v"(d[0]), [d1] "v"(d[1]), [d2] "v"(d[2]), [d3] "v"(d[3]), [i0] "v"(i0), [i1] "v"(i1), [i2] "v"(i2), [i3] "v"(i3));
        };
        auto evaluate = [&](const v4i (&At)[NMI], int h, v4i& addr, v4i& d2, v4i& lab) {
            if (NML == 2) {
                asm volatile("s_nop 3\n\t" XMH_W_MFMA("lab", "al0", "bl0", "lab0") XMH_W_MFMA("lab", "al1", "bl1", "lab")
                             : [lab] "=&v"(lab)
                             : [al0] "v"(At[2]), [al1] "v"(At[NMI - 1]), [bl0] "v"(bL[h][0]), [bl1] "v"(bL[h][NML - 1]), [lab0] "v"(lab0));
            } else {
                asm volatile("s_nop 3\n\t" XMH_W_MFMA("lab", "al0", "bl0", "lab0") : [lab] "=&v"(lab) : [al0] "v"(At[2]), [bl0] "v"(bL[h][0]), [lab0] "v"(lab0));
            }
            if (CACHE) {
                asm volatile("s_nop 3\n\t" XMH_W_MFMA("addr", "a0", "ba0", "cq") XMH_W_MFMA("addr", "a1", "ba1", "addr") XMH_W_MFMA("d2", "a0", "bd0", "kq")
                             XMH_W_MFMA("d2", "a1", "bd1", "d2") "s_nop 7"
                             : [addr] "=&v"(addr), [d2] "=&v"(d2)
                             : [a0] "v"(At[0]), [a1] "v"(At[1]), [ba0] "v"(bA[h][0]), [ba1] "v"(bA[h][1]), [bd0] "v"(bD[h][0]), [bd1] "v"(bD[h][1]), [cq] "v"(cq[h]),
                               [kq] "v"(kq[h]));
            } else {
                asm volatile("s_nop 3\n\t" XMH_W_MFMA("addr", "a0", "ba0", "cq") XMH_W_MFMA("addr", "a1", "ba1", "addr") "s_nop 7"
                             : [addr] "=&v"(addr)
                             : [a0] "v"(At[0]), [a1] "v"(At[1]), [ba0] "v"(bA[h][0]), [ba1] "v"(bA[h][1]), [cq] "v"(cq[h]));
            }
        };
        auto consume = [&](uint32_t& i0, uint32_t& i1, uint32_t& i2, uint32_t& i3, const v4i (&live)[NMI]) {
            if constexpr (NMI == 4) {
                asm volatile(XMH_W_MIN("i0", "lp0") XMH_W_MIN("i1", "lp1") XMH_W_MIN("i2", "lp2") XMH_W_MIN("i3", "lp3") XMH_W_ADD("ap0", "i0")
                             XMH_W_ADD("ap1", "i1") XMH_W_ADD("ap2", "i2") XMH_W_ADD("ap3", "i3")
                             : [i0] "=&v"(i0), [i1] "=&v"(i1), [i2] "=&v"(i2), [i3] "=&v"(i3)
                             : [lp0] "v"(lab_p[0]), [lp1] "v"(lab_p[1]), [lp2] "v"(lab_p[2]), [lp3] "v"(lab_p[3]), [ap0] "v"(addr_p[0]), [ap1] "v"(addr_p[1]),
                               [ap2] "v"(addr_p[2]), [ap3] "v"(addr_p[3]), "v"(live[0]), "v"(live[1]), "v"(live[2]), "v"(live[3])
                             : "memory");
            } else {
                asm volatile(XMH_W_MIN("i0", "lp0") XMH_W_MIN("i1", "lp1") XMH_W_MIN("i2", "lp2") XMH_W_MIN("i3", "lp3") XMH_W_ADD("ap0", "i0")
                             XMH_W_ADD("ap1", "i1") XMH_W_ADD("ap2", "i2") XMH_W_ADD("ap3", "i3")
                             : [i0] "=&v"(i0), [i1] "=&v"(i1), [i2] "=&v"(i2), [i3] "=&v"(i3)
                             : [lp0] "v"(lab_p[0]), [lp1] "v"(lab_p[1]), [lp2] "v"(lab_p[2]), [lp3] "v"(lab_p[3]), [ap0] "v"(addr_p[0]), [ap1] "v"(addr_p[1]),
                               [ap2] "v"(addr_p[2]), [ap3] "v"(addr_p[3]), "v"(live[0]), "v"(live[1]), "v"(live[2])
                             : "memory");
            }
        };
        auto group = [&](auto gc) {
            constexpr int G = decltype(gc)::value;
#pragma unroll
            for (int h = 0; h < NQ; ++h) {
                v4i addr, d2 = d2_p, lab;
                if (G == 0 && h == 0) {
                    evaluate(A[G], h, addr, d2, lab);
                } else {
                    uint32_t i0, i1, i2, i3;
                    fused(A[G], h, addr, d2, lab, i0, i1, i2, i3);
                    if (CACHE) pack(cw[(h + NQ - 1) % NQ][h == 0 ? G - 1 : G], d2_p, i0, i1, i2, i3);
                }
                addr_p = addr; d2_p = d2; lab_p = lab;
                if (G > 0 && h == 0) {
                    if constexpr (NMI == 4) asm volatile("" ::"v"(A[G > 0 ? G - 1 : 0][0]), "v"(A[G > 0 ? G - 1 : 0][1]), "v"(A[G > 0 ? G - 1 : 0][2]), "v"(A[G > 0 ? G - 1 : 0][3]));
                    else asm volatile("" ::"v"(A[G > 0 ? G - 1 : 0][0]), "v"(A[G > 0 ? G - 1 : 0][1]), "v"(A[G > 0 ? G - 1 : 0][2]));
                }
            }
        };
        build(A[0], wcur[0]);
        build(A[1], wcur[1]);
        build(A[2], wcur[2]);
        build(A[3], wcur[3]);
        group(std::integral_constant<int, 0>{});
        group(std::integral_constant<int, 1>{});
        group(std::integral_constant<int, 2>{});
        group(std::integral_constant<int, 3>{});
        asm volatile("s_nop 7\n\ts_nop 3" ::: "memory");
        {
            uint32_t i0, i1, i2, i3;
            consume(i0, i1, i2, i3, A[3]);
            if (CACHE) pack(cw[NQ - 1][3], d2_p, i0, i1, i2, i3);
        }
#ifdef XMH_ABL_NOSTORE
        if (CACHE && a.Q < 0) {
#else
        if (CACHE) {
#endif
#pragma unroll
            for (int h = 0; h < NQ; ++h) {
                uint4* dst = crow[h] + (int64_t)i * 64;
                __builtin_nontemporal_store(cw[h][0], &dst->x);
                __builtin_nontemporal_store(cw[h][1], &dst->y);
                __builtin_nontemporal_store(cw[h][2], &dst->z);
                __builtin_nontemporal_store(cw[h][3], &dst->w);
            }
        }
#pragma unroll
        for (int g = 0; g < 4; ++g)
#pragma unroll
            for (int m = 0; m < NMI; ++m) wcur[g][m] = wnxt[g][m];
    }
    const int npad = nbat * 64 - (int)(hi - lo);
    asm volatile("s_waitcnt lgkmcnt(0)" ::: "memory");
    if (npad > 0 && slot == 0) {
#pragma unroll
        for (int h = 0; h < NQ; ++h) {
            if (!valid[h]) continue;
            const int64_t q = (int64_t)(t16 + h) * 16 + ql;
            int dpad = 0;
            for (int w = 0; w < a.W; ++w) dpad += __popc(a.qbits[q * a.W + w]);
            cnt[h * ncell + dpad * 16 + ql] -= (uint32_t)npad << 16;
        }
    }
#pragma unroll
    for (int h = 0; h < NQ; ++h) {
        uint32_t* __restrict__ out = chunk_hist + ((int64_t)chunk_id * a.nb) * a.qpad + (t16 + h) * 16;
        for (int e = lane; e < ncell; e += 64) out[(int64_t)(e >> 4) * a.qpad + (e & 15)] = cnt[h * ncell + e];
    }
    if (CACHE && dmax >= 256u) *ovf = 1u;
}
#undef XMH_W_MFMA
#undef XMH_W_MIN
#undef XMH_W_ADD

template <bool CAPPED, int EB, bool HALF = false>
__global__ __launch_bounds__(64) void k_scan_ap_c(ScanArgs a, const uint2* __restrict__ below, const uint2* __restrict__ dpre,
                                                  const uint32_t* __restrict__ cap_ws, float* __restrict__ ap_part,
                                                  const uint32_t* __restrict__ items_total, uint32_t kcap, const uint32_t* __restrict__ skip_if = nullptr,
                                                  const uint32_t* __restrict__ nrel_max = nullptr, int rank_bits = 0) {
    static_assert(!HALF || EB == 8, "the 8 x 8 geometry on one-byte entries");
    constexpr int QW = HALF ? 8 : 128 / EB, LOG_QW = QW == 16 ? 4 : 3, S = 64 / QW, EPW = HALF ? 2 : 32 / EB;
    extern __shared__ __attribute__((aligned(16))) uint32_t lds[];
    int chunk_id, qtile;
    if (!map_block(a, chunk_id, qtile)) return;
    if (items_total && (int64_t)*items_total > kFloatBitsMaxItems) return;
    if (skip_if && *skip_if != 0u) return;
    if (nrel_max && rank_bits > 0 && (uint64_t)(*nrel_max) + 2 < (1ull << (32 - rank_bits))) return;
    const int lane = threadIdx.x & 63;
    const int ql = lane & (QW - 1), slot = lane >> LOG_QW;
    const int q0 = qtile * QW, q = q0 + ql;
    const int ncell = a.nb * QW;
    unsigned long long* cnt = reinterpret_cast<unsigned long long*>(lds);
    {
        const uint2* __restrict__ pb = below + ((int64_t)chunk_id * a.nb) * a.qpad + q0;
        const uint2* __restrict__ pd = dpre + q0;
        auto pack = [](uint2 x, uint2 y) {
            return (unsigned long long)(kF23 + x.x + y.x + 1u) | ((unsigned long long)(kF23 + (0x7fffffu - (x.y + y.y + 1u))) << 32);
        };
        int e = lane;
        for (; e + 7 * 64 < ncell; e += 8 * 64) {
            uint2 x[8], y[8];
#pragma unroll
            for (int j = 0; j < 8; ++j) {
                const int ee = e + j * 64;
                const int64_t at = (int64_t)(ee >> LOG_QW) * a.qpad + (ee & (QW - 1));
                x[j] = pb[at];
                y[j] = pd[at];
            }
#pragma unroll
            for (int j = 0; j < 8; ++j) cnt[e + j * 64] = pack(x[j], y[j]);
        }
        for (; e < ncell; e += 64) {
            const int64_t at = (int64_t)(e >> LOG_QW) * a.qpad + (e & (QW - 1));
            cnt[e] = pack(pb[at], pd[at]);
        }
    }
    const uint32_t cntbase = (uint32_t)(uintptr_t)(__attribute__((address_space(3))) uint32_t*)lds + ql * 8;
    const float capf = CAPPED ? (float)min(cap_ws[q], kcap) : 0.0f;
    const int64_t lo = (int64_t)chunk_id * a.chunk;
    const int64_t hi = (lo + a.chunk < a.R) ? lo + a.chunk : a.R;
    float acc = 0.0f;
    auto credit = [&](unsigned long long old, uint32_t m) {
        const float rank = __uint_as_float((uint32_t)old) - 8388608.0f;
        const float ord = 16777215.0f - __uint_as_float((uint32_t)(old >> 32));
        if (CAPPED) m = ord <= capf ? m : 0u;
#ifdef XMH_ABL_AP_NORCP
        acc = fmaf(ord, __uint_as_float(__float_as_uint(rank) & m), acc);
#else
        acc = fmaf(ord, __uint_as_float(__float_as_uint(__builtin_amdgcn_rcpf(rank)) & m), acc);
#endif
    };
    const uint32_t hoff = HALF ? 8u * (uint32_t)(slot >> 2) : 0u;
    const uint32_t hb0 = hoff, hb1 = hoff + 16u, hd0 = hoff + 1u, hd1 = hoff + 17u;
    auto issue1 = [&](uint32_t w, int j, unsigned long long& old, uint32_t& m) {
        uint32_t d;
        if (HALF) {
            m = (uint32_t)__builtin_amdgcn_sbfe((int)w, j ? hb1 : hb0, 1);
            d = __builtin_amdgcn_ubfe(w, j ? hd1 : hd0, EB - 1);
        } else if (EB == 16) {
            m = (uint32_t)__builtin_amdgcn_sbfe((int)w, j, 1);
            d = __builtin_amdgcn_ubfe(w, j + 1, 11);
        } else {
            m = (uint32_t)__builtin_amdgcn_sbfe((int)w, EB * j, 1);
            d = __builtin_amdgcn_ubfe(w, EB * j + 1, EB - 1);
        }
        uint32_t addr;
        if (QW == 16) asm("v_lshl_add_u32 %0, %1, 7, %2" : "=v"(addr) : "v"(d), "v"(cntbase));
        else asm("v_lshl_add_u32 %0, %1, 6, %2" : "=v"(addr) : "v"(d), "v"(cntbase));
        const unsigned long long inc = 1ull | ((unsigned long long)m << 32);
#ifdef XMH_ABL_AP_NOATOMIC
        old = ((unsigned long long)addr << 3) | inc;
        asm volatile("" : "+v"(old));
#else
        asm volatile("ds_add_rtn_u64 %0, %1, %2" : "=v"(old) : "v"(addr), "v"(inc) : "memory");
#endif
    };
    unsigned long long oldA[8], oldB[8];
    uint32_t mA[8], mB[8];
    constexpr bool kFourBatchIterations = true;
    auto issue = [&](unsigned long long (&old)[8], uint32_t (&m)[8], uint32_t wa, uint32_t wb, uint32_t wc, uint32_t wd) {
        if constexpr (EB == 16) {
            const uint32_t sx = __builtin_amdgcn_alignbit(wb, wa, 24), sy = __builtin_amdgcn_alignbit(wc, wb, 28);
#pragma unroll
            for (int u = 0; u < 8; ++u) issue1(XMH_CACHE12_WORD(u, wa, wb, wc, sx, sy), XMH_CACHE12_BIT(u), old[u], m[u]);
        } else {
#pragma unroll
            for (int u = 0; u < 8; ++u) {
                const int wi = u / EPW;
                issue1(wi == 0 ? wa : (wi == 1 ? wb : (wi == 2 ? wc : wd)), u % EPW, old[u], m[u]);
            }
        }
    };
    auto drain8 = [&](unsigned long long (&old)[8], uint32_t (&m)[8]) {
        asm volatile("s_waitcnt lgkmcnt(8)" : "+v"(old[0]), "+v"(old[1]), "+v"(old[2]), "+v"(old[3]), "+v"(old[4]), "+v"(old[5]), "+v"(old[6]), "+v"(old[7])::"memory");
#pragma unroll
        for (int u = 0; u < 8; ++u) credit(old[u], m[u]);
    };
    auto drain0 = [&](unsigned long long (&old)[8], uint32_t (&m)[8]) {
        asm volatile("s_waitcnt lgkmcnt(0)" : "+v"(old[0]), "+v"(old[1]), "+v"(old[2]), "+v"(old[3]), "+v"(old[4]), "+v"(old[5]), "+v"(old[6]), "+v"(old[7])::"memory");
#pragma unroll
        for (int u = 0; u < 8; ++u) credit(old[u], m[u]);
    };
    const int nbatch = (a.chunk + 63) >> 6;
    const uint4* crow = HALF ? a.pair_cache + ((int64_t)chunk_id * (a.nqt >> 1) + (qtile >> 1)) * nbatch * 64 + (slot & 3) * 16 + (qtile & 1) * 8 + ql
                             : a.pair_cache + ((int64_t)chunk_id * a.nqt + qtile) * nbatch * 64 + lane;
    const int nfull = (int)((hi - lo) >> 6);
    asm volatile("s_waitcnt lgkmcnt(0)" ::: "memory");
    const uint32_t* crow12 = reinterpret_cast<const uint32_t*>(a.pair_cache) + (((int64_t)chunk_id * a.nqt + qtile) * nbatch * 64 + lane) * xmh::kCache12Dwords;
    auto cache_words = [&](int64_t batch) -> uint4 {
        if constexpr (EB == 16) {
            typedef uint32_t u32x3_t __attribute__((ext_vector_type(3)));
            const u32x3_t v = __builtin_nontemporal_load(reinterpret_cast<const u32x3_t*>(crow12 + batch * 64 * xmh::kCache12Dwords));
            return make_uint4(v.x, v.y, v.z, 0u);
        } else {
#ifdef XMH_ABL_AP_PLAIN
            return crow[batch * 64];
#else
            typedef uint32_t u32x4_t __attribute__((ext_vector_type(4)));
            const u32x4_t v = __builtin_nontemporal_load(reinterpret_cast<const u32x4_t*>(crow + batch * 64));
            return make_uint4(v.x, v.y, v.z, v.w);
#endif
        }
    };
    uint4 cw = cache_words(0);
    uint4 nw = cache_words(1 < nbatch ? 1 : 0);
    auto next_words = [&](int bi) {
#ifdef XMH_ABL_AP_NOLOAD
        const uint4 nw2 = make_uint4(0x10203040u + bi + lane, 0x18283848u ^ lane, 0x11223344u + 3 * lane, 0x21314151u + bi);
#else
        const uint4 nw2 = cache_words(bi + 2 < nbatch ? bi + 2 : nbatch - 1);
#endif
        return nw2;
    };
    auto slow_batch = [&](const uint4& w4, int count) {
        const uint32_t sx = EB == 16 ? __builtin_amdgcn_alignbit(w4.y, w4.x, 24) : 0u, sy = EB == 16 ? __builtin_amdgcn_alignbit(w4.z, w4.y, 28) : 0u;
#pragma unroll
        for (int t = 0; t < QW; ++t) {
            if (t * S + slot < count) {
                const uint32_t w = EB == 16 ? XMH_CACHE12_WORD(t, w4.x, w4.y, w4.z, sx, sy) : (t < EPW ? w4.x : (t < 2 * EPW ? w4.y : (t < 3 * EPW ? w4.z : w4.w)));
                const uint32_t bit = EB == 16 ? (uint32_t)XMH_CACHE12_BIT(t) : (HALF ? hoff + 16u * (t % EPW) : (uint32_t)(EB * (t % EPW)));
                const uint32_t m = (uint32_t)__builtin_amdgcn_sbfe((int)w, bit, 1), d = __builtin_amdgcn_ubfe(w, bit + 1u, EB == 16 ? 11 : EB - 1);
                const unsigned long long o = atomicAdd(&cnt[d * QW + ql], 1ull | ((unsigned long long)m << 32));
                credit(o, m);
            }
        }
    };
    if (EB == 8 && !HALF) {
        int bi = 0;
        if (kFourBatchIterations) {
            for (; bi + 3 < nfull; bi += 4) {
                const uint4 n0 = next_words(bi);
                issue(oldA, mA, cw.x, cw.y, 0u, 0u);
                issue(oldB, mB, cw.z, cw.w, 0u, 0u);
                drain8(oldA, mA);
                cw = nw;
                nw = n0;
#pragma unroll
                for (int t = 1; t < 4; ++t) {
                    const uint4 nt = next_words(bi + t);
                    issue(oldA, mA, cw.x, cw.y, 0u, 0u);
                    drain8(oldB, mB);
                    issue(oldB, mB, cw.z, cw.w, 0u, 0u);
                    drain8(oldA, mA);
                    cw = nw;
                    nw = nt;
                }
                drain0(oldB, mB);
            }
        }
        for (; bi + 1 < nfull; bi += 2) {
            const uint4 nw2 = next_words(bi);
            issue(oldA, mA, cw.x, cw.y, 0u, 0u);
            issue(oldB, mB, cw.z, cw.w, 0u, 0u);
            drain8(oldA, mA);
            cw = nw;
            nw = nw2;
            const uint4 nw3 = next_words(bi + 1);
            issue(oldA, mA, cw.x, cw.y, 0u, 0u);
            drain8(oldB, mB);
            issue(oldB, mB, cw.z, cw.w, 0u, 0u);
            drain8(oldA, mA);
            drain0(oldB, mB);
            cw = nw;
            nw = nw3;
        }
        if (bi < nfull) {
            const uint4 nw2 = next_words(bi);
            issue(oldA, mA, cw.x, cw.y, 0u, 0u);
            issue(oldB, mB, cw.z, cw.w, 0u, 0u);
            drain8(oldA, mA);
            drain0(oldB, mB);
            cw = nw;
            nw = nw2;
        }
    } else {
        auto words_at = [&](int b) { return cache_words(b < nbatch ? b : nbatch - 1); };
        auto issue4 = [&](unsigned long long (&old)[8], uint32_t (&m)[8], const uint4& r) { issue(old, m, r.x, r.y, r.z, r.w); };
        uint4 r0 = cw, r1 = nw, r2 = words_at(2), r3 = words_at(3);
        int bi = 0;
        for (; bi + 3 < nfull; bi += 4) {
            issue4(oldA, mA, r0);
            r0 = words_at(bi + 4);
            issue4(oldB, mB, r1);
            r1 = words_at(bi + 5);
            drain8(oldA, mA);
            issue4(oldA, mA, r2);
            r2 = words_at(bi + 6);
            drain8(oldB, mB);
            issue4(oldB, mB, r3);
            r3 = words_at(bi + 7);
            drain8(oldA, mA);
            drain0(oldB, mB);
        }
        const int rem = nfull - bi;
        if (rem >= 2) {
            issue4(oldA, mA, r0);
            issue4(oldB, mB, r1);
            drain8(oldA, mA);
            drain0(oldB, mB);
            if (rem == 3) {
                issue4(oldA, mA, r2);
                drain0(oldA, mA);
            }
        } else if (rem == 1) {
            issue4(oldA, mA, r0);
            drain0(oldA, mA);
        }
        cw = rem == 0 ? r0 : (rem == 1 ? r1 : (rem == 2 ? r2 : r3));
    }
    const int cntb = (int)(hi - lo) - nfull * 64;
    slow_batch(cw, cntb);
#pragma unroll
    for (int o = QW; o < 64; o <<= 1) acc += __shfl_xor(acc, o, 64);
    if (slot == 0) ap_part[(int64_t)chunk_id * a.qpad + q] = acc;
}

#define XMH_AP2_SETA "v113", "v115", "v117", "v119", "v[112:113]", "v[114:115]", "v[116:117]", "v[118:119]"
#define XMH_AP2_SETB "v121", "v123", "v125", "v127", "v[120:121]", "v[122:123]", "v[124:125]", "v[126:127]"
#define XMH_AP2_MFMA(D, A, B, C) "v_mfma_i32_16x16x64_i8 %[" D "], %[" A "], %[" B "], " C "\n\t"
#define XMH_AP2_MAX(H, L) "v_max_i32 " H ", -1, %[" L "]\n\t"
#define XMH_AP2_ADD(O, A, P) "ds_add_rtn_u64 %[" O "], %[" A "], " P "\n\t"
#define XMH_AP2_FUSED2_(H0, H1, H2, H3, P0, P1, P2, P3)                                                                                   \
    "s_nop 3\n\t" XMH_AP2_MFMA("lab", "a1", "q1", "0") XMH_AP2_MAX(H0, "l0") XMH_AP2_MAX(H1, "l1") XMH_AP2_MAX(H2, "l2")                \
    XMH_AP2_MFMA("lab", "a2", "q2", "%[lab]") XMH_AP2_MAX(H3, "l3") XMH_AP2_ADD("o0", "p0", P0) XMH_AP2_ADD("o1", "p1", P1)            \
    XMH_AP2_MFMA("addr", "a0", "q0", "%[c0]") XMH_AP2_ADD("o2", "p2", P2) XMH_AP2_ADD("o3", "p3", P3)
#define XMH_AP2_FUSED1_(H0, H1, H2, H3, P0, P1, P2, P3)                                                                                   \
    "s_nop 3\n\t" XMH_AP2_MFMA("lab", "a1", "q1", "0") XMH_AP2_MAX(H0, "l0") XMH_AP2_MAX(H1, "l1") XMH_AP2_MAX(H2, "l2") XMH_AP2_MAX(H3, "l3") \
    XMH_AP2_MFMA("addr", "a0", "q0", "%[c0]") XMH_AP2_ADD("o0", "p0", P0) XMH_AP2_ADD("o1", "p1", P1) XMH_AP2_ADD("o2", "p2", P2)       \
    XMH_AP2_ADD("o3", "p3", P3)
#define XMH_AP2_TAIL_(H0, H1, H2, H3, P0, P1, P2, P3)                                                                                     \
    XMH_AP2_MAX(H0, "l0") XMH_AP2_MAX(H1, "l1") XMH_AP2_MAX(H2, "l2") XMH_AP2_MAX(H3, "l3") XMH_AP2_ADD("o0", "p0", P0)                   \
    XMH_AP2_ADD("o1", "p1", P1) XMH_AP2_ADD("o2", "p2", P2) XMH_AP2_ADD("o3", "p3", P3)
#define XMH_AP2_FUSED2(...) XMH_AP2_FUSED2_(__VA_ARGS__)
#define XMH_AP2_FUSED1(...) XMH_AP2_FUSED1_(__VA_ARGS__)
#define XMH_AP2_TAIL(...) XMH_AP2_TAIL_(__VA_ARGS__)
template <int NML, int NW, int NQ, bool CAPPED>
__global__ __launch_bounds__(64 * NW) void k_scan_ap_r2(MfmaArgs a, const uint2* __restrict__ below, const uint2* __restrict__ dpre,
                                                        const uint32_t* __restrict__ cap_ws, float* __restrict__ ap_part,
                                                        const uint32_t* __restrict__ items_total, uint32_t kcap) {
    using u64 = unsigned long long;
    constexpr int NMI = 1 + NML;
    extern __shared__ __attribute__((aligned(16))) uint32_t lds[];
    int chunk_id, qtile;
    if (!mfma_map_block(a, chunk_id, qtile)) return;
    if (items_total && (int64_t)*items_total > kFloatBitsMaxItems) return;
    const int lane = threadIdx.x & 63, wave = threadIdx.x >> 6;
    const int ql = lane & 15, slot = lane >> 4;
    const int t16 = (qtile * NW + wave) * NQ;
    const int ncell = a.nb * 16;
    u64* cnt = reinterpret_cast<u64*>(lds) + (wave * NQ) * ncell;
    auto pack = [](uint2 x, uint2 y) {
        return (u64)(kF23 + x.x + y.x + 1u) | ((u64)(kF23 + (0x7fffffu - (x.y + y.y + 1u))) << 32);
    };
#pragma unroll
    for (int h = 0; h < NQ; ++h) {
        const uint2* __restrict__ pb = below + ((int64_t)chunk_id * a.nb) * a.qpad + (t16 + h) * 16;
        const uint2* __restrict__ pd = dpre + (t16 + h) * 16;
        u64* c = cnt + h * ncell;
        auto cell = [&](int e) { return e; };
        int e = lane;
        for (; e + 3 * 64 < ncell; e += 4 * 64) {
            uint2 x[4], y[4];
#pragma unroll
            for (int j = 0; j < 4; ++j) {
                const int ee = e + j * 64;
                const int64_t at = (int64_t)(ee >> 4) * a.qpad + (ee & 15);
                x[j] = pb[at];
                y[j] = pd[at];
            }
#pragma unroll
            for (int j = 0; j < 4; ++j) c[cell(e + j * 64)] = pack(x[j], y[j]);
        }
        for (; e < ncell; e += 64) {
            const int64_t at = (int64_t)(e >> 4) * a.qpad + (e & 15);
            c[cell(e)] = pack(pb[at], pd[at]);
        }
    }
    v4i bq[NQ], bl[NQ][NML], cq[NQ];
    float capf[NQ], acc[NQ];
    const int rsh = 4 * (slot & 1), rwi = slot >> 1;
#pragma unroll
    for (int h = 0; h < NQ; ++h) {
        const int64_t q = (int64_t)(t16 + h) * 16 + ql;
        const bool valid = q < a.Q;
        int pcq = 0;
        uint32_t qw = 0u;
        if (valid) {
            for (int w = 0; w < a.W; ++w) pcq += __popc(a.qbits[q * a.W + w]);
            if (rwi < a.W) qw = a.qbits[q * a.W + rwi];
        }
        qw >>= rsh;
        const bool on = valid && rwi < a.W;
#pragma unroll
        for (int j = 0; j < 4; ++j) {
            const uint32_t t = (qw >> j) & 0x01010101u;
            if (j & 1) bq[h][j] = on ? (int)(0x20202020u ^ (t * 0xc0u)) : 0;
            else bq[h][j] = on ? (int)(0x40404040u ^ (t << 7)) : 0;
        }
#pragma unroll
        for (int m = 0; m < NML; ++m) {
            uint32_t lw = 0u;
            if (valid && 2 * m + rwi < a.LW) lw = a.qlab[q * a.LW + 2 * m + rwi];
            lw >>= rsh;
#pragma unroll
            for (int j = 0; j < 4; ++j) bl[h][m][j] = (int)(((lw >> j) & 0x01010101u) * 0xffu);
        }
        const int c0 = (int)(uint32_t)(uintptr_t)(__attribute__((address_space(3))) u64*)(cnt + h * ncell) + ql * 8 + (valid ? 128 * pcq : 0);
        cq[h] = v4i{c0, c0, c0, c0};
        asm volatile("" : "+v"(cq[h]));
        capf[h] = CAPPED ? (float)min(cap_ws[q], kcap) : 0.0f;
        acc[h] = 0.0f;
    }
    const int64_t lo = (int64_t)chunk_id * a.chunk;
    const int64_t hi = (lo + a.chunk < a.R) ? lo + a.chunk : a.R;
    const int nbat = (int)((hi - lo + 63) >> 6);
    const int64_t bat0 = lo >> 6;
    uint32_t wcur[4][NMI], wnxt[4][NMI];
    const int ritem = 4 * (lane & 3) + ((lane & 15) >> 2);
    const int wi_c = rwi < a.W ? rwi : a.W - 1;
    int wi_l[NML];
#pragma unroll
    for (int m = 0; m < NML; ++m) wi_l[m] = 2 * m + rwi < a.LW ? 2 * m + rwi : (a.LW > 0 ? a.LW - 1 : 0);
    auto load_words = [&](int64_t batch, uint32_t (&w)[4][NMI]) {
        const int64_t first = batch * 64;
        if (first + 64 <= (int64_t)a.R) {
            const uint32_t* __restrict__ pc = a.rbits + (first + ritem) * a.W + wi_c;
            const uint32_t* __restrict__ pl = a.rlab + (first + ritem) * a.LW;
#pragma unroll
            for (int g = 0; g < 4; ++g) {
                w[g][0] = pc[g * 16 * a.W];
#pragma unroll
                for (int m = 0; m < NML; ++m) w[g][1 + m] = pl[g * 16 * a.LW + wi_l[m]];
            }
        } else {
#pragma unroll
            for (int g = 0; g < 4; ++g) {
                const int64_t item = first + g * 16 + ritem;
                const int64_t it = item < a.R ? item : (int64_t)a.R - 1;
                const uint32_t ok = item < a.R ? 0xffffffffu : 0u;
                w[g][0] = a.rbits[it * a.W + wi_c] & ok;
#pragma unroll
                for (int m = 0; m < NML; ++m) w[g][1 + m] = a.rlab[it * a.LW + wi_l[m]] & ok;
            }
        }
    };
    const uint32_t rot_a = (uint32_t)(rsh + 31) & 31u, rot_b = (uint32_t)rsh + 1u;
    auto build = [&](v4i (&At)[NMI], const uint32_t (&w)[NMI]) {
        const uint32_t xa = __builtin_amdgcn_alignbit(w[0], w[0], rot_a), xb = __builtin_amdgcn_alignbit(w[0], w[0], rot_b);
        At[0][0] = (int)(xa & 0x02020202u);
        At[0][1] = (int)(xa & 0x04040404u);
        At[0][2] = (int)(xb & 0x02020202u);
        At[0][3] = (int)(xb & 0x04040404u);
#pragma unroll
        for (int m = 1; m < NMI; ++m) {
            const uint32_t y = w[m] >> rsh;
#pragma unroll
            for (int j = 0; j < 4; ++j) At[m][j] = (int)(y & (0x01010101u << j));
        }
    };
    auto credit = [&](u64 old, uint32_t m, int h) {
        const float rank = __uint_as_float((uint32_t)old) - 8388608.0f;
        const float ord = 16777215.0f - __uint_as_float((uint32_t)(old >> 32));
        if (CAPPED) m = ord <= capf[h] ? m : 0u;
        acc[h] = fmaf(ord, __uint_as_float(__float_as_uint(__builtin_amdgcn_rcpf(rank)) & m), acc[h]);
    };
    v4i incA01 = {1, 0, 1, 0}, incA23 = {1, 0, 1, 0}, incB01 = {1, 0, 1, 0}, incB23 = {1, 0, 1, 0};
    asm volatile("" : "+{v[112:115]}"(incA01), "+{v[116:119]}"(incA23), "+{v[120:123]}"(incB01), "+{v[124:127]}"(incB23));
    asm volatile("s_waitcnt lgkmcnt(0)" ::: "memory");
    load_words(bat0, wcur);
    for (int i = 0; i < nbat; ++i) {
        load_words(bat0 + (i + 1 < nbat ? i + 1 : i), wnxt);
        v4i A[4][NMI];
        build(A[0], wcur[0]);
        build(A[1], wcur[1]);
        build(A[2], wcur[2]);
        build(A[3], wcur[3]);
        u64 oldA[4], oldB[4];
        v4i addr_p, lab_p;
        auto evaluate = [&](const v4i (&At)[NMI], int h, v4i& addr, v4i& lab) {
            if constexpr (NML == 2)
                asm volatile("s_nop 3\n\t" XMH_AP2_MFMA("lab", "a1", "q1", "0") XMH_AP2_MFMA("lab", "a2", "q2", "%[lab]") XMH_AP2_MFMA("addr", "a0", "q0", "%[c0]") "s_nop 7"
                             : [lab] "=&v"(lab), [addr] "=&v"(addr)
                             : [a1] "v"(At[1]), [q1] "v"(bl[h][0]), [a2] "v"(At[NMI - 1]), [q2] "v"(bl[h][NML - 1]), [a0] "v"(At[0]), [q0] "v"(bq[h]), [c0] "v"(cq[h]));
            else
                asm volatile("s_nop 3\n\t" XMH_AP2_MFMA("lab", "a1", "q1", "0") XMH_AP2_MFMA("addr", "a0", "q0", "%[c0]") "s_nop 7"
                             : [lab] "=&v"(lab), [addr] "=&v"(addr)
                             : [a1] "v"(At[1]), [q1] "v"(bl[h][0]), [a0] "v"(At[0]), [q0] "v"(bq[h]), [c0] "v"(cq[h]));
        };
#define XMH_AP2_OUTS(OLD) [lab] "=&v"(lab), [addr] "=&v"(addr), [o0] "=&v"(OLD[0]), [o1] "=&v"(OLD[1]), [o2] "=&v"(OLD[2]), [o3] "=&v"(OLD[3])
#define XMH_AP2_PREV [p0] "v"(addr_p[0]), [p1] "v"(addr_p[1]), [p2] "v"(addr_p[2]), [p3] "v"(addr_p[3]), [l0] "v"(lab_p[0]), [l1] "v"(lab_p[1]), [l2] "v"(lab_p[2]), [l3] "v"(lab_p[3])
        auto fusedA = [&](const v4i (&At)[NMI], int h, v4i& addr, v4i& lab) {
            if constexpr (NML == 2)
                asm volatile(XMH_AP2_FUSED2(XMH_AP2_SETA)
                             : XMH_AP2_OUTS(oldA), "+{v[112:115]}"(incA01), "+{v[116:119]}"(incA23)
                             : [a1] "v"(At[1]), [q1] "v"(bl[h][0]), [a2] "v"(At[NMI - 1]), [q2] "v"(bl[h][NML - 1]), [a0] "v"(At[0]), [q0] "v"(bq[h]), [c0] "v"(cq[h]), XMH_AP2_PREV
                             : "memory");
            else
                asm volatile(XMH_AP2_FUSED1(XMH_AP2_SETA)
                             : XMH_AP2_OUTS(oldA), "+{v[112:115]}"(incA01), "+{v[116:119]}"(incA23)
                             : [a1] "v"(At[1]), [q1] "v"(bl[h][0]), [a0] "v"(At[0]), [q0] "v"(bq[h]), [c0] "v"(cq[h]), XMH_AP2_PREV
                             : "memory");
        };
        auto fusedB = [&](const v4i (&At)[NMI], int h, v4i& addr, v4i& lab) {
            if constexpr (NML == 2)
                asm volatile(XMH_AP2_FUSED2(XMH_AP2_SETB)
                             : XMH_AP2_OUTS(oldB), "+{v[120:123]}"(incB01), "+{v[124:127]}"(incB23)
                             : [a1] "v"(At[1]), [q1] "v"(bl[h][0]), [a2] "v"(At[NMI - 1]), [q2] "v"(bl[h][NML - 1]), [a0] "v"(At[0]), [q0] "v"(bq[h]), [c0] "v"(cq[h]), XMH_AP2_PREV
                             : "memory");
            else
                asm volatile(XMH_AP2_FUSED1(XMH_AP2_SETB)
                             : XMH_AP2_OUTS(oldB), "+{v[120:123]}"(incB01), "+{v[124:127]}"(incB23)
                             : [a1] "v"(At[1]), [q1] "v"(bl[h][0]), [a0] "v"(At[0]), [q0] "v"(bq[h]), [c0] "v"(cq[h]), XMH_AP2_PREV
                             : "memory");
        };
        auto drainA = [&](int h, auto newer) {
            if constexpr (decltype(newer)::value == 4) asm volatile("s_waitcnt lgkmcnt(4)" : "+v"(oldA[0]), "+v"(oldA[1]), "+v"(oldA[2]), "+v"(oldA[3])::"memory");
            else asm volatile("s_waitcnt lgkmcnt(0)" : "+v"(oldA[0]), "+v"(oldA[1]), "+v"(oldA[2]), "+v"(oldA[3])::"memory");
            credit(oldA[0], (uint32_t)incA01[1], h);
            credit(oldA[1], (uint32_t)incA01[3], h);
            credit(oldA[2], (uint32_t)incA23[1], h);
            credit(oldA[3], (uint32_t)incA23[3], h);
        };
        auto drainB = [&](int h, auto newer) {
            if constexpr (decltype(newer)::value == 4) asm volatile("s_waitcnt lgkmcnt(4)" : "+v"(oldB[0]), "+v"(oldB[1]), "+v"(oldB[2]), "+v"(oldB[3])::"memory");
            else asm volatile("s_waitcnt lgkmcnt(0)" : "+v"(oldB[0]), "+v"(oldB[1]), "+v"(oldB[2]), "+v"(oldB[3])::"memory");
            credit(oldB[0], (uint32_t)incB01[1], h);
            credit(oldB[1], (uint32_t)incB01[3], h);
            credit(oldB[2], (uint32_t)incB23[1], h);
            credit(oldB[3], (uint32_t)incB23[3], h);
        };
        using N4 = std::integral_constant<int, 4>;
        using N0 = std::integral_constant<int, 0>;
        auto step = [&](auto pc) {
            constexpr int P = decltype(pc)::value, G = P / NQ, H = P % NQ;
            v4i addr, lab;
            if constexpr (P == 0) evaluate(A[0], 0, addr, lab);
            else if constexpr ((P - 1) & 1) fusedB(A[G], H, addr, lab);
            else fusedA(A[G], H, addr, lab);
            addr_p = addr; lab_p = lab;
            if constexpr (G > 0 && H == 0) {
                if constexpr (NMI == 2) asm volatile("" ::"v"(A[G - 1][0]), "v"(A[G - 1][1]));
                else asm volatile("" ::"v"(A[G - 1][0]), "v"(A[G - 1][1]), "v"(A[G - 1][NMI - 1]));
            }
            if constexpr (P >= 2) {
                if constexpr ((P - 2) & 1) drainB((P - 2) % NQ, N4{});
                else drainA((P - 2) % NQ, N4{});
            }
        };
        auto run = [&](auto self, auto pc) -> void {
            step(pc);
            if constexpr (decltype(pc)::value + 1 < 4 * NQ) self(self, std::integral_constant<int, decltype(pc)::value + 1>{});
        };
        run(run, std::integral_constant<int, 0>{});
        asm volatile("s_nop 7\n\ts_nop 3" ::: "memory");
        {
            constexpr int PL = 4 * NQ - 1;
            static_assert(PL & 1, "the last pair of a batch goes to set B");
            asm volatile(XMH_AP2_TAIL(XMH_AP2_SETB)
                         : [o0] "=&v"(oldB[0]), [o1] "=&v"(oldB[1]), [o2] "=&v"(oldB[2]), [o3] "=&v"(oldB[3]), "+{v[120:123]}"(incB01), "+{v[124:127]}"(incB23)
                         : XMH_AP2_PREV, "v"(A[3][0]), "v"(A[3][1]), "v"(A[3][NMI - 1])
                         : "memory");
            drainA((PL - 1) % NQ, N4{});
            drainB(PL % NQ, N0{});
        }
#pragma unroll
        for (int g = 0; g < 4; ++g)
#pragma unroll
            for (int m = 0; m < NMI; ++m) wcur[g][m] = wnxt[g][m];
    }
#undef XMH_AP2_OUTS
#undef XMH_AP2_PREV
#pragma unroll
    for (int h = 0; h < NQ; ++h) {
        float s = acc[h];
        s += __shfl_xor(s, 16, 64);
        s += __shfl_xor(s, 32, 64);
        if (slot == 0) ap_part[(int64_t)chunk_id * a.qpad + (t16 + h) * 16 + ql] = s;
    }
}


}
```

Measured before the change: 1663 billion pairs/s.

## Use one FP4 MFMA for 65-128 class labels instead of two i8 MFMAs

For label widths above 64 classes, the kernel now encodes label bits as FP4 nibbles and computes the label-overlap tile with a single v_mfma_f32_16x16x128_f8f6f4 instead of two chained i8 MFMAs. Each lane now loads one label word per item, and the code paths for the two tile counts are merged into shared macros. The aim is to cut MFMA issue slots and label loads in the hot scan loop. The risk is that FP4 encoding or float accumulation of the overlap test could go wrong, so the self-check adds cases with 128 classes and sparse labels.

```diff
diff --git a/clip-based-cross-modal-hash_amd/csrc/xmh_scan.hip b/clip-based-cross-modal-hash_amd/csrc/xmh_scan.hip
--- a/clip-based-cross-modal-hash_amd/csrc/xmh_scan.hip
+++ b/clip-based-cross-modal-hash_amd/csrc/xmh_scan.hip
@@ -771,9 +771,10 @@
     if (state[dev]) return state[dev] == 1;
     state[dev] = 1;
     const int64_t Q = 200, R = 9000;
-    const int C = 80, LW = 3;
     bool same = true, ran = true;
-    for (int K : {64, 40, 16, 100}) {
+    const int cases[6][2] = {{64, 80}, {40, 80}, {16, 80}, {100, 80}, {64, 128}, {100, 128}};
+    for (const auto& kc : cases) {
+        const int K = kc[0], C = kc[1], LW = (C + 31) / 32;
         const int W = (K + 31) / 32;
         std::vector<uint32_t> qb(Q * W), ql(Q * LW), rb(R * W), rl(R * LW);
         uint64_t x = 0x9E3779B97F4A7C15ull ^ (uint64_t)K;
@@ -784,10 +785,21 @@
             for (int w = 0; w < W; ++w) rb[i * W + w] = (i > 64 && (rnd() & 3) == 0) ? rb[(rnd() % 64) * W + w] : rnd();
         for (int64_t i = 0; i < Q; ++i) qb[i * W + W - 1] &= last;
         for (int64_t i = 0; i < R; ++i) rb[i * W + W - 1] &= last;
-        for (int64_t i = 0; i < Q * LW; ++i) ql[i] = rnd() & rnd() & rnd() & (i % LW == LW - 1 ? 0xffffu : 0xffffffffu);
-        for (int64_t i = 0; i < R * LW; ++i) rl[i] = rnd() & rnd() & rnd() & (i % LW == LW - 1 ? 0xffffu : 0xffffffffu);
-        for (int64_t i = 0; i < Q; ++i) ql[i * LW] |= 1u;
-        for (int64_t i = 0; i < R; i += 7) rl[i * LW] |= 1u;
+        const uint32_t lastl = C % 32 ? (1u << (C % 32)) - 1 : 0xffffffffu;
+        for (int64_t i = 0; i < Q * LW; ++i) ql[i] = rnd() & rnd() & rnd() & (i % LW == LW - 1 ? lastl : 0xffffffffu);
+        for (int64_t i = 0; i < R * LW; ++i) rl[i] = rnd() & rnd() & rnd() & (i % LW == LW - 1 ? lastl : 0xffffffffu);
+        if (C == 80) {
+            for (int64_t i = 0; i < Q; ++i) ql[i * LW] |= 1u;
+            for (int64_t i = 0; i < R; i += 7) rl[i * LW] |= 1u;
+        } else {
+            auto one = [&](uint32_t* l, int c) { for (int w = 0; w < LW; ++w) l[w] = 0u; l[c >> 5] = 1u << (c & 31); };
+            for (int64_t i = 0; i < Q; i += 2) one(&ql[i * LW], i % 8 == 0 ? (int)(i * 3 % 64) : 64 + (int)(i * 7 % 64));
+            for (int64_t i = 0; i < R; ++i) {
+                if (i % 3 == 0) one(&rl[i * LW], 64 + (int)(i * 5 % 64));
+                else if (i % 3 == 1) for (int w = 0; w < LW; ++w) rl[i * LW + w] = 0u;
+            }
+            for (int w = 0; w < LW; ++w) ql[1 * LW + w] = rl[2 * LW + w] = rl[5000 * LW + w] = 0xffffffffu;
+        }
         std::vector<uint32_t> h1, h0;
         std::vector<double> a1, a0;
         std::vector<int32_t> c1, c0;
diff --git a/clip-based-cross-modal-hash_amd/csrc/xmh_scan_mfma.h b/clip-based-cross-modal-hash_amd/csrc/xmh_scan_mfma.h
--- a/clip-based-cross-modal-hash_amd/csrc/xmh_scan_mfma.h
+++ b/clip-based-cross-modal-hash_amd/csrc/xmh_scan_mfma.h
@@ -50,9 +50,21 @@
     return chunk_id < a.nchunk;
 }
 
+__device__ __forceinline__ v4i label_query_f4(uint32_t w, uint32_t one) {
+    v4i r;
+#pragma unroll
+    for (int j = 0; j < 4; ++j) r[j] = (int)(((w >> j) & 0x11111111u) * one);
+    return r;
+}
+__device__ __forceinline__ v4i label_item_f4(uint32_t w) {
+    return v4i{(int)(w & 0x11111111u), (int)(w & 0x22222222u), (int)(w & 0x44444444u), (int)((w >> 1) & 0x44444444u)};
+}
+
 template <int NML, int NW, int NQ, bool CACHE>
 __device__ __forceinline__ void scan_hist_r2_body(const MfmaArgs& a, uint32_t* __restrict__ chunk_hist, uint4* __restrict__ pair_cache) {
-    constexpr int NMI = 1 + NML, NMQ = 2 + NML;
+    static_assert(NML == 1 || NML == 2, "one i8 label tile (at most 64 classes) or one FP4 label tile (65-128 classes)");
+    constexpr bool F4 = NML == 2;
+    constexpr int NMI = 2, NMQ = 3;
     constexpr bool REGS = true;
     extern __shared__ __attribute__((aligned(16))) uint32_t lds[];
     int chunk_id, qtile;
@@ -90,13 +102,14 @@
                     bq[h][1][j] = on ? (int)(0x02020202u ^ (t * 0xfcu)) : 0;
                 }
             }
-#pragma unroll
-            for (int m = 0; m < NML; ++m) {
+            if constexpr (F4) {
+                bq[h][2] = label_query_f4(valid[h] && slot < a.LW ? a.qlab[q * a.LW + slot] : 0u, 0x2u);
+            } else {
                 uint32_t lw = 0u;
-                if (valid[h] && 2 * m + rwi < a.LW) lw = a.qlab[q * a.LW + 2 * m + rwi];
+                if (valid[h] && rwi < a.LW) lw = a.qlab[q * a.LW + rwi];
                 lw >>= rsh;
 #pragma unroll
-                for (int j = 0; j < 4; ++j) bq[h][2 + m][j] = (int)((lw >> j) & 0x01010101u);
+                for (int j = 0; j < 4; ++j) bq[h][2][j] = (int)((lw >> j) & 0x01010101u);
             }
             const int k2 = 2 * pcq;
             kqv[h] = v4i{k2, k2, k2, k2};
@@ -121,19 +134,17 @@
     uint32_t wcur[4][NMI], wnxt[4][NMI];
     const int ritem = 4 * (lane & 3) + ((lane & 15) >> 2);
     const int wi_c = rwi < a.W ? rwi : a.W - 1;
-    int wi_l[NML];
-#pragma unroll
-    for (int m = 0; m < NML; ++m) wi_l[m] = 2 * m + rwi < a.LW ? 2 * m + rwi : (a.LW > 0 ? a.LW - 1 : 0);
+    const int lwi = F4 ? slot : rwi;
+    const int wi_l = lwi < a.LW ? lwi : (a.LW > 0 ? a.LW - 1 : 0);
     auto load_words = [&](int64_t batch, uint32_t (&w)[4][NMI]) {
         const int64_t first = batch * 64;
         if (first + 64 <= (int64_t)a.R) {
             const uint32_t* __restrict__ pc = a.rbits + (first + ritem) * a.W + wi_c;
-            const uint32_t* __restrict__ pl = a.rlab + (first + ritem) * a.LW;
+            const uint32_t* __restrict__ pl = a.rlab + (first + ritem) * a.LW + wi_l;
 #pragma unroll
             for (int g = 0; g < 4; ++g) {
                 w[g][0] = pc[g * 16 * a.W];
-#pragma unroll
-                for (int m = 0; m < NML; ++m) w[g][1 + m] = pl[g * 16 * a.LW + wi_l[m]];
+                w[g][1] = pl[g * 16 * a.LW];
             }
         } else {
 #pragma unroll
@@ -142,8 +153,7 @@
                 const int64_t it = item < a.R ? item : (int64_t)a.R - 1;
                 const uint32_t ok = item < a.R ? 0xffffffffu : 0u;
                 w[g][0] = a.rbits[it * a.W + wi_c] & ok;
-#pragma unroll
-                for (int m = 0; m < NML; ++m) w[g][1 + m] = a.rlab[it * a.LW + wi_l[m]] & ok;
+                w[g][1] = a.rlab[it * a.LW + wi_l] & ok;
             }
         }
     };
@@ -153,11 +163,12 @@
         At[0][1] = (int)(xa & 0x02020202u);
         At[0][2] = (int)(xb & 0x01010101u);
         At[0][3] = (int)(xb & 0x02020202u);
-#pragma unroll
-        for (int m = 1; m < NMI; ++m) {
-            const uint32_t y = w[m] >> rsh;
-#pragma unroll
-            for (int j = 0; j < 4; ++j) At[m][j] = (int)(y & (0x01010101u << j));
+        if constexpr (F4) {
+            At[1] = label_item_f4(w[1]);
+        } else {
+            const uint32_t y = w[1] >> rsh;
+#pragma unroll
+            for (int j = 0; j < 4; ++j) At[1][j] = (int)(y & (0x01010101u << j));
         }
     };
     load_words(bat0, wcur);
@@ -215,90 +226,55 @@
 #endif
 #ifdef XMH_ABL_NOMFMA
 #define XMH_MFMA(D, A, B, C) "s_nop 0\n\t"
+#define XMH_MFMA_F4(D, A, B, C) "s_nop 0\n\t"
 #else
 #define XMH_MFMA(D, A, B, C) "v_mfma_i32_16x16x64_i8 " D ", " A ", " B ", " C "\n\t"
+#define XMH_MFMA_F4(D, A, B, C) "v_mfma_f32_16x16x128_f8f6f4 " D ", " A ", " B ", " C " cbsz:4 blgp:4\n\t"
 #endif
 #define XMH_SDWA(J) "dst_sel:BYTE_" #J " dst_unused:UNUSED_PRESERVE src0_sel:BYTE_0 src1_sel:BYTE_0\n\t"
+#define XMH_R2_FUSED_CACHE(LAB)                                                                                                                   \
+    asm volatile(XMH_R2_OPEN LAB("%0", "%8", "%9", "%10")                                                                                         \
+                 XMH_VMIN "%4, 0x10001, %24\n\t" XMH_VMIN "%5, 0x10001, %25\n\t" XMH_VMIN "%6, 0x10001, %26\n\t" XMH_VMIN "%7, 0x10001, %27\n\t" \
+                 "v_or_b32_sdwa %3, %16, %4 dst_sel:BYTE_0 dst_unused:UNUSED_PAD src0_sel:BYTE_0 src1_sel:BYTE_0\n\t"                            \
+                 XMH_ADD("%20", "%4")                                                                                                             \
+                 XMH_MFMA("%1", "%11", "%12", "%13")                                                                                              \
+                 "v_or_b32_sdwa %3, %17, %5 " XMH_SDWA(1) XMH_ADD("%21", "%5") "v_or_b32_sdwa %3, %18, %6 " XMH_SDWA(2)                           \
+                 XMH_MFMA("%2", "%11", "%14", "%15")                                                                                              \
+                 XMH_ADD("%22", "%6") "v_or_b32_sdwa %3, %19, %7 " XMH_SDWA(3) XMH_ADD("%23", "%7")                                               \
+                 : "=&v"(lab), "=&v"(addr), "=&v"(d2), "=&v"(w), "=&v"(i0), "=&v"(i1), "=&v"(i2), "=&v"(i3)                                        \
+                 : "v"(At[1]), "v"(bq[h][2]), "v"(lab0), "v"(At[0]), "v"(bq[h][0]), "v"(cq[h]), "v"(bq[h][1]), "v"(kqv[REGS ? h : 0]),             \
+                   "v"(d2_p[0]), "v"(d2_p[1]), "v"(d2_p[2]), "v"(d2_p[3]), "v"(addr_p[0]), "v"(addr_p[1]), "v"(addr_p[2]), "v"(addr_p[3]),         \
+                   "v"(lab_p[0]), "v"(lab_p[1]), "v"(lab_p[2]), "v"(lab_p[3])                                                                      \
+                 : "memory")
+#define XMH_R2_FUSED_PLAIN(LAB)                                                                                                                   \
+    asm volatile(XMH_R2_OPEN LAB("%0", "%6", "%7", "%8")                                                                                          \
+                 XMH_VMIN "%2, 0x10001, %16\n\t" XMH_VMIN "%3, 0x10001, %17\n\t" XMH_VMIN "%4, 0x10001, %18\n\t" XMH_VMIN "%5, 0x10001, %19\n\t" \
+                 XMH_MFMA("%1", "%9", "%10", "%11")                                                                                               \
+                 XMH_ADD("%12", "%2") XMH_ADD("%13", "%3") XMH_ADD("%14", "%4") XMH_ADD("%15", "%5")                                              \
+                 : "=&v"(lab), "=&v"(addr), "=&v"(i0), "=&v"(i1), "=&v"(i2), "=&v"(i3)                                                             \
+                 : "v"(At[1]), "v"(bq[h][2]), "v"(lab0), "v"(At[0]), "v"(bq[h][0]), "v"(cq[h]),                                                    \
+                   "v"(addr_p[0]), "v"(addr_p[1]), "v"(addr_p[2]), "v"(addr_p[3]), "v"(lab_p[0]), "v"(lab_p[1]), "v"(lab_p[2]), "v"(lab_p[3])      \
+                 : "memory")
+#define XMH_R2_EVAL_CACHE(LAB)                                                                                                                    \
+    asm volatile(XMH_R2_OPEN LAB("%0", "%3", "%4", "%5") XMH_MFMA("%1", "%6", "%7", "%8") XMH_MFMA("%2", "%6", "%9", "%10") XMH_R2_EVAL_CLOSE     \
+                 : "=&v"(lab), "=&v"(addr), "=&v"(d2)                                                                                             \
+                 : "v"(At[1]), "v"(bq[h][2]), "v"(lab0), "v"(At[0]), "v"(bq[h][0]), "v"(cq[h]), "v"(bq[h][1]), "v"(kqv[REGS ? h : 0]))
+#define XMH_R2_EVAL_PLAIN(LAB)                                                                                                                    \
+    asm volatile(XMH_R2_OPEN LAB("%0", "%2", "%3", "%4") XMH_MFMA("%1", "%5", "%6", "%7") XMH_R2_EVAL_CLOSE                                       \
+                 : "=&v"(lab), "=&v"(addr)                                                                                                        \
+                 : "v"(At[1]), "v"(bq[h][2]), "v"(lab0), "v"(At[0]), "v"(bq[h][0]), "v"(cq[h]))
         auto fused = [&](const v4i (&At)[NMI], int h, v4i& addr, v4i& d2, v4i& lab, uint32_t& w) {
             uint32_t i0, i1, i2, i3;
-            if (NML == 2 && CACHE) {
-                asm volatile(
-                    XMH_R2_OPEN XMH_MFMA("%0", "%8", "%9", "%10")
-                    XMH_VMIN "%4, 0x10001, %26\n\t" XMH_VMIN "%5, 0x10001, %27\n\t" XMH_VMIN "%6, 0x10001, %28\n\t"
-                    XMH_MFMA("%0", "%11", "%12", "%0")
-                    XMH_VMIN "%7, 0x10001, %29\n\t"
-                    "v_or_b32_sdwa %3, %18, %4 dst_sel:BYTE_0 dst_unused:UNUSED_PAD src0_sel:BYTE_0 src1_sel:BYTE_0\n\t"
-                    XMH_ADD("%22", "%4")
-                    XMH_MFMA("%1", "%13", "%14", "%15")
-                    "v_or_b32_sdwa %3, %19, %5 " XMH_SDWA(1) XMH_ADD("%23", "%5") "v_or_b32_sdwa %3, %20, %6 " XMH_SDWA(2)
-                    XMH_MFMA("%2", "%13", "%16", "%17")
-                    XMH_ADD("%24", "%6") "v_or_b32_sdwa %3, %21, %7 " XMH_SDWA(3) XMH_ADD("%25", "%7")
-                    : "=&v"(lab), "=&v"(addr), "=&v"(d2), "=&v"(w), "=&v"(i0), "=&v"(i1), "=&v"(i2), "=&v"(i3)
-                    : "v"(At[1]), "v"(bq[h][2]), "v"(lab0), "v"(At[NMI - 1]), "v"(bq[h][NMQ - 1]), "v"(At[0]), "v"(bq[h][0]), "v"(cq[h]), "v"(bq[h][1]), "v"(kqv[REGS ? h : 0]),
-                      "v"(d2_p[0]), "v"(d2_p[1]), "v"(d2_p[2]), "v"(d2_p[3]), "v"(addr_p[0]), "v"(addr_p[1]), "v"(addr_p[2]), "v"(addr_p[3]),
-                      "v"(lab_p[0]), "v"(lab_p[1]), "v"(lab_p[2]), "v"(lab_p[3])
-                    : "memory");
-            } else if (NML == 2) {
-                asm volatile(
-                    XMH_R2_OPEN XMH_MFMA("%0", "%6", "%7", "%8")
-                    XMH_VMIN "%2, 0x10001, %18\n\t" XMH_VMIN "%3, 0x10001, %19\n\t" XMH_VMIN "%4, 0x10001, %20\n\t"
-                    XMH_MFMA("%0", "%9", "%10", "%0")
-                    XMH_VMIN "%5, 0x10001, %21\n\t" XMH_ADD("%14", "%2") XMH_ADD("%15", "%3")
-                    XMH_MFMA("%1", "%11", "%12", "%13")
-                    XMH_ADD("%16", "%4") XMH_ADD("%17", "%5")
-                    : "=&v"(lab), "=&v"(addr), "=&v"(i0), "=&v"(i1), "=&v"(i2), "=&v"(i3)
-                    : "v"(At[1]), "v"(bq[h][2]), "v"(lab0), "v"(At[NMI - 1]), "v"(bq[h][NMQ - 1]), "v"(At[0]), "v"(bq[h][0]), "v"(cq[h]),
-                      "v"(addr_p[0]), "v"(addr_p[1]), "v"(addr_p[2]), "v"(addr_p[3]), "v"(lab_p[0]), "v"(lab_p[1]), "v"(lab_p[2]), "v"(lab_p[3])
-                    : "memory");
-            } else if (CACHE) {
-                asm volatile(
-                    XMH_R2_OPEN XMH_MFMA("%0", "%8", "%9", "%10")
-                    XMH_VMIN "%4, 0x10001, %24\n\t" XMH_VMIN "%5, 0x10001, %25\n\t" XMH_VMIN "%6, 0x10001, %26\n\t" XMH_VMIN "%7, 0x10001, %27\n\t"
-                    "v_or_b32_sdwa %3, %16, %4 dst_sel:BYTE_0 dst_unused:UNUSED_PAD src0_sel:BYTE_0 src1_sel:BYTE_0\n\t"
-                    XMH_ADD("%20", "%4")
-                    XMH_MFMA("%1", "%11", "%12", "%13")
-                    "v_or_b32_sdwa %3, %17, %5 " XMH_SDWA(1) XMH_ADD("%21", "%5") "v_or_b32_sdwa %3, %18, %6 " XMH_SDWA(2)
-                    XMH_MFMA("%2", "%11", "%14", "%15")
-                    XMH_ADD("%22", "%6") "v_or_b32_sdwa %3, %19, %7 " XMH_SDWA(3) XMH_ADD("%23", "%7")
-                    : "=&v"(lab), "=&v"(addr), "=&v"(d2), "=&v"(w), "=&v"(i0), "=&v"(i1), "=&v"(i2), "=&v"(i3)
-                    : "v"(At[1]), "v"(bq[h][2]), "v"(lab0), "v"(At[0]), "v"(bq[h][0]), "v"(cq[h]), "v"(bq[h][1]), "v"(kqv[REGS ? h : 0]),
-                      "v"(d2_p[0]), "v"(d2_p[1]), "v"(d2_p[2]), "v"(d2_p[3]), "v"(addr_p[0]), "v"(addr_p[1]), "v"(addr_p[2]), "v"(addr_p[3]),
-                      "v"(lab_p[0]), "v"(lab_p[1]), "v"(lab_p[2]), "v"(lab_p[3])
-                    : "memory");
-            } else {
-                asm volatile(
-                    XMH_R2_OPEN XMH_MFMA("%0", "%6", "%7", "%8")
-                    XMH_VMIN "%2, 0x10001, %16\n\t" XMH_VMIN "%3, 0x10001, %17\n\t" XMH_VMIN "%4, 0x10001, %18\n\t" XMH_VMIN "%5, 0x10001, %19\n\t"
-                    XMH_MFMA("%1", "%9", "%10", "%11")
-                    XMH_ADD("%12", "%2") XMH_ADD("%13", "%3") XMH_ADD("%14", "%4") XMH_ADD("%15", "%5")
-                    : "=&v"(lab), "=&v"(addr), "=&v"(i0), "=&v"(i1), "=&v"(i2), "=&v"(i3)
-                    : "v"(At[1]), "v"(bq[h][2]), "v"(lab0), "v"(At[0]), "v"(bq[h][0]), "v"(cq[h]),
-                      "v"(addr_p[0]), "v"(addr_p[1]), "v"(addr_p[2]), "v"(addr_p[3]), "v"(lab_p[0]), "v"(lab_p[1]), "v"(lab_p[2]), "v"(lab_p[3])
-                    : "memory");
-            }
+            if constexpr (F4 && CACHE) XMH_R2_FUSED_CACHE(XMH_MFMA_F4);
+            else if constexpr (F4) XMH_R2_FUSED_PLAIN(XMH_MFMA_F4);
+            else if constexpr (CACHE) XMH_R2_FUSED_CACHE(XMH_MFMA);
+            else XMH_R2_FUSED_PLAIN(XMH_MFMA);
         };
         auto evaluate = [&](const v4i (&At)[NMI], int h, v4i& addr, v4i& d2, v4i& lab) {
-            if (NML == 2 && CACHE) {
-                asm volatile(XMH_R2_OPEN XMH_MFMA("%0", "%3", "%4", "%5") XMH_MFMA("%0", "%6", "%7", "%0")
-                             XMH_MFMA("%1", "%8", "%9", "%10") XMH_MFMA("%2", "%8", "%11", "%12") XMH_R2_EVAL_CLOSE
-                             : "=&v"(lab), "=&v"(addr), "=&v"(d2)
-                             : "v"(At[1]), "v"(bq[h][2]), "v"(lab0), "v"(At[NMI - 1]), "v"(bq[h][NMQ - 1]), "v"(At[0]), "v"(bq[h][0]), "v"(cq[h]),
-                               "v"(bq[h][1]), "v"(kqv[REGS ? h : 0]));
-            } else if (NML == 2) {
-                asm volatile(XMH_R2_OPEN XMH_MFMA("%0", "%2", "%3", "%4") XMH_MFMA("%0", "%5", "%6", "%0")
-                             XMH_MFMA("%1", "%7", "%8", "%9") XMH_R2_EVAL_CLOSE
-                             : "=&v"(lab), "=&v"(addr)
-                             : "v"(At[1]), "v"(bq[h][2]), "v"(lab0), "v"(At[NMI - 1]), "v"(bq[h][NMQ - 1]), "v"(At[0]), "v"(bq[h][0]), "v"(cq[h]));
-            } else if (CACHE) {
-                asm volatile(XMH_R2_OPEN XMH_MFMA("%0", "%3", "%4", "%5") XMH_MFMA("%1", "%6", "%7", "%8")
-                             XMH_MFMA("%2", "%6", "%9", "%10") XMH_R2_EVAL_CLOSE
-                             : "=&v"(lab), "=&v"(addr), "=&v"(d2)
-                             : "v"(At[1]), "v"(bq[h][2]), "v"(lab0), "v"(At[0]), "v"(bq[h][0]), "v"(cq[h]), "v"(bq[h][1]), "v"(kqv[REGS ? h : 0]));
-            } else {
-                asm volatile(XMH_R2_OPEN XMH_MFMA("%0", "%2", "%3", "%4") XMH_MFMA("%1", "%5", "%6", "%7") XMH_R2_EVAL_CLOSE
-                             : "=&v"(lab), "=&v"(addr)
-                             : "v"(At[1]), "v"(bq[h][2]), "v"(lab0), "v"(At[0]), "v"(bq[h][0]), "v"(cq[h]));
-            }
+            if constexpr (F4 && CACHE) XMH_R2_EVAL_CACHE(XMH_MFMA_F4);
+            else if constexpr (F4) XMH_R2_EVAL_PLAIN(XMH_MFMA_F4);
+            else if constexpr (CACHE) XMH_R2_EVAL_CACHE(XMH_MFMA);
+            else XMH_R2_EVAL_PLAIN(XMH_MFMA);
         };
         auto consume = [&](uint32_t& w, const v4i (&live)[NMI]) {
             uint32_t i0, i1, i2, i3;
@@ -323,8 +299,13 @@
                     : "memory");
             }
         };
+#undef XMH_R2_EVAL_PLAIN
+#undef XMH_R2_EVAL_CACHE
+#undef XMH_R2_FUSED_PLAIN
+#undef XMH_R2_FUSED_CACHE
 #undef XMH_SDWA
 #undef XMH_ADD
+#undef XMH_MFMA_F4
 #undef XMH_MFMA
         auto group = [&](auto gc) {
             constexpr int G = decltype(gc)::value;
@@ -422,12 +403,35 @@
 }
 
 #define XMH_W_MFMA(D, A, B, C) "v_mfma_i32_16x16x64_i8 %[" D "], %[" A "], %[" B "], %[" C "]\n\t"
+#define XMH_W_MFMA_F4(D, A, B, C) "v_mfma_f32_16x16x128_f8f6f4 %[" D "], %[" A "], %[" B "], %[" C "] cbsz:4 blgp:4\n\t"
 #define XMH_W_MIN(I, L) "v_min_u32 %[" I "], 0x10001, %[" L "]\n\t"
 #define XMH_W_ADD(A, D) "ds_add_u32 %[" A "], %[" D "]\n\t"
+#define XMH_W_FUSED_CACHE(LAB) \
+    asm volatile("s_nop 3\n\t" LAB("lab", "al0", "bl0", "lab0") XMH_W_MIN("i0", "lp0") XMH_W_MIN("i1", "lp1") XMH_W_MIN("i2", "lp2")                \
+                 XMH_W_MIN("i3", "lp3") XMH_W_ADD("ap0", "i0") XMH_W_MFMA("addr", "a0", "ba0", "cq") XMH_W_ADD("ap1", "i1")                         \
+                 XMH_W_MFMA("addr", "a1", "ba1", "addr") XMH_W_ADD("ap2", "i2") XMH_W_MFMA("d2", "a0", "bd0", "kq") XMH_W_ADD("ap3", "i3")          \
+                 XMH_W_MFMA("d2", "a1", "bd1", "d2")                                                                                                \
+                 : [lab] "=&v"(lab), [addr] "=&v"(addr), [d2] "=&v"(d2), [i0] "=&v"(i0), [i1] "=&v"(i1), [i2] "=&v"(i2), [i3] "=&v"(i3)             \
+                 : [a0] "v"(At[0]), [a1] "v"(At[1]), [al0] "v"(At[2]), [ba0] "v"(bA[h][0]), [ba1] "v"(bA[h][1]), [bd0] "v"(bD[h][0]),               \
+                   [bd1] "v"(bD[h][1]), [bl0] "v"(bL[h]), [lab0] "v"(lab0), [cq] "v"(cq[h]), [kq] "v"(kq[h]), [lp0] "v"(lab_p[0]),                  \
+                   [lp1] "v"(lab_p[1]), [lp2] "v"(lab_p[2]), [lp3] "v"(lab_p[3]), [ap0] "v"(addr_p[0]), [ap1] "v"(addr_p[1]), [ap2] "v"(addr_p[2]), \
+                   [ap3] "v"(addr_p[3])                                                                                                             \
+                 : "memory")
+#define XMH_W_FUSED_PLAIN(LAB) \
+    asm volatile("s_nop 3\n\t" LAB("lab", "al0", "bl0", "lab0") XMH_W_MIN("i0", "lp0") XMH_W_MIN("i1", "lp1") XMH_W_MIN("i2", "lp2")                 \
+                 XMH_W_MIN("i3", "lp3") XMH_W_ADD("ap0", "i0") XMH_W_ADD("ap1", "i1") XMH_W_MFMA("addr", "a0", "ba0", "cq") XMH_W_ADD("ap2", "i2")   \
+                 XMH_W_ADD("ap3", "i3") XMH_W_MFMA("addr", "a1", "ba1", "addr")                                                                      \
+                 : [lab] "=&v"(lab), [addr] "=&v"(addr), [i0] "=&v"(i0), [i1] "=&v"(i1), [i2] "=&v"(i2), [i3] "=&v"(i3)                              \
+                 : [a0] "v"(At[0]), [a1] "v"(At[1]), [al0] "v"(At[2]), [ba0] "v"(bA[h][0]), [ba1] "v"(bA[h][1]), [bl0] "v"(bL[h]), [lab0] "v"(lab0), \
+                   [cq] "v"(cq[h]), [lp0] "v"(lab_p[0]), [lp1] "v"(lab_p[1]), [lp2] "v"(lab_p[2]), [lp3] "v"(lab_p[3]), [ap0] "v"(addr_p[0]),        \
+                   [ap1] "v"(addr_p[1]), [ap2] "v"(addr_p[2]), [ap3] "v"(addr_p[3])                                                                  \
+                 : "memory")
 template <int NML, int NW, int NQ, bool CACHE>
 __global__ __launch_bounds__(64 * NW) void k_scan_hist_r2w(MfmaArgs a, uint32_t* __restrict__ chunk_hist, uint4* __restrict__ pair_cache,
                                                            uint32_t* __restrict__ ovf) {
-    constexpr int NMC = 2, NMI = NMC + NML;
+    static_assert(NML == 1 || NML == 2, "one i8 label tile (at most 64 classes) or one FP4 label tile (65-128 classes)");
+    constexpr bool F4 = NML == 2;
+    constexpr int NMC = 2, NMI = NMC + 1;
     extern __shared__ __attribute__((aligned(16))) uint32_t lds[];
     int chunk_id, qtile;
     if (!mfma_map_block(a, chunk_id, qtile)) return;
@@ -438,7 +442,7 @@
     uint32_t* cnt = lds + (wave * NQ) * ncell;
     for (int e = lane; e < NQ * ncell; e += 64) cnt[e] = 0u;
     const int rsh = 4 * (slot & 1), rwi = slot >> 1;
-    v4i bA[NQ][NMC], bD[NQ][NMC], bL[NQ][NML], cq[NQ], kq[NQ];
+    v4i bA[NQ][NMC], bD[NQ][NMC], bL[NQ], cq[NQ], kq[NQ];
     bool valid[NQ];
 #pragma unroll
     for (int h = 0; h < NQ; ++h) {
@@ -464,13 +468,14 @@
                 }
             }
         }
-#pragma unroll
-        for (int m = 0; m < NML; ++m) {
+        if constexpr (F4) {
+            bL[h] = label_query_f4(valid[h] && slot < a.LW ? a.qlab[q * a.LW + slot] : 0u, 0x2u);
+        } else {
             uint32_t lw = 0u;
-            if (valid[h] && 2 * m + rwi < a.LW) lw = a.qlab[q * a.LW + 2 * m + rwi];
+            if (valid[h] && rwi < a.LW) lw = a.qlab[q * a.LW + rwi];
             lw >>= rsh;
 #pragma unroll
-            for (int j = 0; j < 4; ++j) bL[h][m][j] = (int)((lw >> j) & 0x01010101u);
+            for (int j = 0; j < 4; ++j) bL[h][j] = (int)((lw >> j) & 0x01010101u);
         }
         const int c0 = (int)(uint32_t)(uintptr_t)(__attribute__((address_space(3))) uint32_t*)(cnt + h * ncell) + ql * 4 + (valid[h] ? 64 * pcq : 0);
         const int k2 = valid[h] ? 2 * pcq : 0;
@@ -491,11 +496,11 @@
         crow[h] = CACHE ? pair_cache + ((int64_t)chunk_id * (a.qpad >> 4) + (t16 + h)) * ((a.chunk + 63) >> 6) * 64 + lane : nullptr;
     uint32_t wcur[4][NMI], wnxt[4][NMI];
     const int ritem = 4 * (lane & 3) + ((lane & 15) >> 2);
-    int wi_c[NMC], wi_l[NML];
+    int wi_c[NMC];
 #pragma unroll
     for (int c = 0; c < NMC; ++c) wi_c[c] = 2 * c + rwi < a.W ? 2 * c + rwi : a.W - 1;
-#pragma unroll
-    for (int m = 0; m < NML; ++m) wi_l[m] = 2 * m + rwi < a.LW ? 2 * m + rwi : (a.LW > 0 ? a.LW - 1 : 0);
+    const int lwi = F4 ? slot : rwi;
+    const int wi_l = lwi < a.LW ? lwi : (a.LW > 0 ? a.LW - 1 : 0);
     auto load_words = [&](int64_t batch, uint32_t (&w)[4][NMI]) {
         const int64_t first = batch * 64;
         if (first + 64 <= (int64_t)a.R) {
@@ -505,8 +510,7 @@
             for (int g = 0; g < 4; ++g) {
 #pragma unroll
                 for (int c = 0; c < NMC; ++c) w[g][c] = pc[g * 16 * a.W + wi_c[c]];
-#pragma unroll
-                for (int m = 0; m < NML; ++m) w[g][NMC + m] = pl[g * 16 * a.LW + wi_l[m]];
+                w[g][NMC] = pl[g * 16 * a.LW + wi_l];
             }
         } else {
 #pragma unroll
@@ -516,8 +520,7 @@
                 const uint32_t ok = item < a.R ? 0xffffffffu : 0u;
 #pragma unroll
                 for (int c = 0; c < NMC; ++c) w[g][c] = a.rbits[it * a.W + wi_c[c]] & ok;
-#pragma unroll
-                for (int m = 0; m < NML; ++m) w[g][NMC + m] = a.rlab[it * a.LW + wi_l[m]] & ok;
+                w[g][NMC] = a.rlab[it * a.LW + wi_l] & ok;
             }
         }
     };
@@ -530,11 +533,12 @@
             At[c][2] = (int)(xb & 0x01010101u);
             At[c][3] = (int)(xb & 0x02020202u);
         }
-#pragma unroll
-        for (int m = 0; m < NML; ++m) {
-            const uint32_t y = w[NMC + m] >> rsh;
-#pragma unroll
-            for (int j = 0; j < 4; ++j) At[NMC + m][j] = (int)(y & (0x01010101u << j));
+        if constexpr (F4) {
+            At[NMC] = label_item_f4(w[NMC]);
+        } else {
+            const uint32_t y = w[NMC] >> rsh;
+#pragma unroll
+            for (int j = 0; j < 4; ++j) At[NMC][j] = (int)(y & (0x01010101u << j));
         }
     };
     uint32_t dmax = 0u;
@@ -545,47 +549,10 @@
         uint32_t cw[NQ][4];
         v4i addr_p = {0, 0, 0, 0}, d2_p = {0, 0, 0, 0}, lab_p = {0, 0, 0, 0};
         auto fused = [&](const v4i (&At)[NMI], int h, v4i& addr, v4i& d2, v4i& lab, uint32_t& i0, uint32_t& i1, uint32_t& i2, uint32_t& i3) {
-            if (NML == 2 && CACHE) {
-                asm volatile("s_nop 3\n\t" XMH_W_MFMA("lab", "al0", "bl0", "lab0") XMH_W_MIN("i0", "lp0") XMH_W_MIN("i1", "lp1") XMH_W_MIN("i2", "lp2")
-                             XMH_W_MFMA("lab", "al1", "bl1", "lab") XMH_W_MIN("i3", "lp3") XMH_W_ADD("ap0", "i0") XMH_W_MFMA("addr", "a0", "ba0", "cq")
-                             XMH_W_ADD("ap1", "i1") XMH_W_MFMA("addr", "a1", "ba1", "addr") XMH_W_ADD("ap2", "i2") XMH_W_MFMA("d2", "a0", "bd0", "kq")
-                             XMH_W_ADD("ap3", "i3") XMH_W_MFMA("d2", "a1", "bd1", "d2")
-                             : [lab] "=&v"(lab), [addr] "=&v"(addr), [d2] "=&v"(d2), [i0] "=&v"(i0), [i1] "=&v"(i1), [i2] "=&v"(i2), [i3] "=&v"(i3)
-                             : [a0] "v"(At[0]), [a1] "v"(At[1]), [al0] "v"(At[2]), [al1] "v"(At[NMI - 1]), [ba0] "v"(bA[h][0]), [ba1] "v"(bA[h][1]),
-                               [bd0] "v"(bD[h][0]), [bd1] "v"(bD[h][1]), [bl0] "v"(bL[h][0]), [bl1] "v"(bL[h][NML - 1]), [lab0] "v"(lab0), [cq] "v"(cq[h]),
-                               [kq] "v"(kq[h]), [lp0] "v"(lab_p[0]), [lp1] "v"(lab_p[1]), [lp2] "v"(lab_p[2]), [lp3] "v"(lab_p[3]), [ap0] "v"(addr_p[0]),
-                               [ap1] "v"(addr_p[1]), [ap2] "v"(addr_p[2]), [ap3] "v"(addr_p[3])
-                             : "memory");
-            } else if (NML == 2) {
-                asm volatile("s_nop 3\n\t" XMH_W_MFMA("lab", "al0", "bl0", "lab0") XMH_W_MIN("i0", "lp0") XMH_W_MIN("i1", "lp1") XMH_W_MIN("i2", "lp2")
-                             XMH_W_MFMA("lab", "al1", "bl1", "lab") XMH_W_MIN("i3", "lp3") XMH_W_ADD("ap0", "i0") XMH_W_ADD("ap1", "i1")
-                             XMH_W_MFMA("addr", "a0", "ba0", "cq") XMH_W_ADD("ap2", "i2") XMH_W_ADD("ap3", "i3") XMH_W_MFMA("addr", "a1", "ba1", "addr")
-                             : [lab] "=&v"(lab), [addr] "=&v"(addr), [i0] "=&v"(i0), [i1] "=&v"(i1), [i2] "=&v"(i2), [i3] "=&v"(i3)
-                             : [a0] "v"(At[0]), [a1] "v"(At[1]), [al0] "v"(At[2]), [al1] "v"(At[NMI - 1]), [ba0] "v"(bA[h][0]), [ba1] "v"(bA[h][1]),
-                               [bl0] "v"(bL[h][0]), [bl1] "v"(bL[h][NML - 1]), [lab0] "v"(lab0), [cq] "v"(cq[h]), [lp0] "v"(lab_p[0]), [lp1] "v"(lab_p[1]),
-                               [lp2] "v"(lab_p[2]), [lp3] "v"(lab_p[3]), [ap0] "v"(addr_p[0]), [ap1] "v"(addr_p[1]), [ap2] "v"(addr_p[2]), [ap3] "v"(addr_p[3])
-                             : "memory");
-            } else if (CACHE) {
-                asm volatile("s_nop 3\n\t" XMH_W_MFMA("lab", "al0", "bl0", "lab0") XMH_W_MIN("i0", "lp0") XMH_W_MIN("i1", "lp1") XMH_W_MIN("i2", "lp2")
-                             XMH_W_MIN("i3", "lp3") XMH_W_ADD("ap0", "i0") XMH_W_MFMA("addr", "a0", "ba0", "cq") XMH_W_ADD("ap1", "i1")
-                             XMH_W_MFMA("addr", "a1", "ba1", "addr") XMH_W_ADD("ap2", "i2") XMH_W_MFMA("d2", "a0", "bd0", "kq") XMH_W_ADD("ap3", "i3")
-                             XMH_W_MFMA("d2", "a1", "bd1", "d2")
-                             : [lab] "=&v"(lab), [addr] "=&v"(addr), [d2] "=&v"(d2), [i0] "=&v"(i0), [i1] "=&v"(i1), [i2] "=&v"(i2), [i3] "=&v"(i3)
-                             : [a0] "v"(At[0]), [a1] "v"(At[1]), [al0] "v"(At[2]), [ba0] "v"(bA[h][0]), [ba1] "v"(bA[h][1]), [bd0] "v"(bD[h][0]),
-                               [bd1] "v"(bD[h][1]), [bl0] "v"(bL[h][0]), [lab0] "v"(lab0), [cq] "v"(cq[h]), [kq] "v"(kq[h]), [lp0] "v"(lab_p[0]),
-                               [lp1] "v"(lab_p[1]), [lp2] "v"(lab_p[2]), [lp3] "v"(lab_p[3]), [ap0] "v"(addr_p[0]), [ap1] "v"(addr_p[1]), [ap2] "v"(addr_p[2]),
-                               [ap3] "v"(addr_p[3])
-                             : "memory");
-            } else {
-                asm volatile("s_nop 3\n\t" XMH_W_MFMA("lab", "al0", "bl0", "lab0") XMH_W_MIN("i0", "lp0") XMH_W_MIN("i1", "lp1") XMH_W_MIN("i2", "lp2")
-                             XMH_W_MIN("i3", "lp3") XMH_W_ADD("ap0", "i0") XMH_W_ADD("ap1", "i1") XMH_W_MFMA("addr", "a0", "ba0", "cq") XMH_W_ADD("ap2", "i2")
-                             XMH_W_ADD("ap3", "i3") XMH_W_MFMA("addr", "a1", "ba1", "addr")
-                             : [lab] "=&v"(lab), [addr] "=&v"(addr), [i0] "=&v"(i0), [i1] "=&v"(i1), [i2] "=&v"(i2), [i3] "=&v"(i3)
-                             : [a0] "v"(At[0]), [a1] "v"(At[1]), [al0] "v"(At[2]), [ba0] "v"(bA[h][0]), [ba1] "v"(bA[h][1]), [bl0] "v"(bL[h][0]), [lab0] "v"(lab0),
-                               [cq] "v"(cq[h]), [lp0] "v"(lab_p[0]), [lp1] "v"(lab_p[1]), [lp2] "v"(lab_p[2]), [lp3] "v"(lab_p[3]), [ap0] "v"(addr_p[0]),
-                               [ap1] "v"(addr_p[1]), [ap2] "v"(addr_p[2]), [ap3] "v"(addr_p[3])
-                             : "memory");
-            }
+            if constexpr (F4 && CACHE) XMH_W_FUSED_CACHE(XMH_W_MFMA_F4);
+            else if constexpr (F4) XMH_W_FUSED_PLAIN(XMH_W_MFMA_F4);
+            else if constexpr (CACHE) XMH_W_FUSED_CACHE(XMH_W_MFMA);
+            else XMH_W_FUSED_PLAIN(XMH_W_MFMA);
         };
         auto pack = [&](uint32_t& w, const v4i& d, uint32_t i0, uint32_t i1, uint32_t i2, uint32_t i3) {
             uint32_t wb;
@@ -600,12 +567,10 @@
                          : [d0] "v"(d[0]), [d1] "v"(d[1]), [d2] "v"(d[2]), [d3] "v"(d[3]), [i0] "v"(i0), [i1] "v"(i1), [i2] "v"(i2), [i3] "v"(i3));
         };
         auto evaluate = [&](const v4i (&At)[NMI], int h, v4i& addr, v4i& d2, v4i& lab) {
-            if (NML == 2) {
-                asm volatile("s_nop 3\n\t" XMH_W_MFMA("lab", "al0", "bl0", "lab0") XMH_W_MFMA("lab", "al1", "bl1", "lab")
-                             : [lab] "=&v"(lab)
-                             : [al0] "v"(At[2]), [al1] "v"(At[NMI - 1]), [bl0] "v"(bL[h][0]), [bl1] "v"(bL[h][NML - 1]), [lab0] "v"(lab0));
+            if constexpr (F4) {
+                asm volatile("s_nop 3\n\t" XMH_W_MFMA_F4("lab", "al0", "bl0", "lab0") : [lab] "=&v"(lab) : [al0] "v"(At[2]), [bl0] "v"(bL[h]), [lab0] "v"(lab0));
             } else {
-                asm volatile("s_nop 3\n\t" XMH_W_MFMA("lab", "al0", "bl0", "lab0") : [lab] "=&v"(lab) : [al0] "v"(At[2]), [bl0] "v"(bL[h][0]), [lab0] "v"(lab0));
+                asm volatile("s_nop 3\n\t" XMH_W_MFMA("lab", "al0", "bl0", "lab0") : [lab] "=&v"(lab) : [al0] "v"(At[2]), [bl0] "v"(bL[h]), [lab0] "v"(lab0));
             }
             if (CACHE) {
                 asm volatile("s_nop 3\n\t" XMH_W_MFMA("addr", "a0", "ba0", "cq") XMH_W_MFMA("addr", "a1", "ba1", "addr") XMH_W_MFMA("d2", "a0", "bd0", "kq")
@@ -620,21 +585,12 @@
             }
         };
         auto consume = [&](uint32_t& i0, uint32_t& i1, uint32_t& i2, uint32_t& i3, const v4i (&live)[NMI]) {
-            if constexpr (NMI == 4) {
-                asm volatile(XMH_W_MIN("i0", "lp0") XMH_W_MIN("i1", "lp1") XMH_W_MIN("i2", "lp2") XMH_W_MIN("i3", "lp3") XMH_W_ADD("ap0", "i0")
-                             XMH_W_ADD("ap1", "i1") XMH_W_ADD("ap2", "i2") XMH_W_ADD("ap3", "i3")
-                             : [i0] "=&v"(i0), [i1] "=&v"(i1), [i2] "=&v"(i2), [i3] "=&v"(i3)
-                             : [lp0] "v"(lab_p[0]), [lp1] "v"(lab_p[1]), [lp2] "v"(lab_p[2]), [lp3] "v"(lab_p[3]), [ap0] "v"(addr_p[0]), [ap1] "v"(addr_p[1]),
-                               [ap2] "v"(addr_p[2]), [ap3] "v"(addr_p[3]), "v"(live[0]), "v"(live[1]), "v"(live[2]), "v"(live[3])
-                             : "memory");
-            } else {
-                asm volatile(XMH_W_MIN("i0", "lp0") XMH_W_MIN("i1", "lp1") XMH_W_MIN("i2", "lp2") XMH_W_MIN("i3", "lp3") XMH_W_ADD("ap0", "i0")
-                             XMH_W_ADD("ap1", "i1") XMH_W_ADD("ap2", "i2") XMH_W_ADD("ap3", "i3")
-                             : [i0] "=&v"(i0), [i1] "=&v"(i1), [i2] "=&v"(i2), [i3] "=&v"(i3)
-                             : [lp0] "v"(lab_p[0]), [lp1] "v"(lab_p[1]), [lp2] "v"(lab_p[2]), [lp3] "v"(lab_p[3]), [ap0] "v"(addr_p[0]), [ap1] "v"(addr_p[1]),
-                               [ap2] "v"(addr_p[2]), [ap3] "v"(addr_p[3]), "v"(live[0]), "v"(live[1]), "v"(live[2])
-                             : "memory");
-            }
+            asm volatile(XMH_W_MIN("i0", "lp0") XMH_W_MIN("i1", "lp1") XMH_W_MIN("i2", "lp2") XMH_W_MIN("i3", "lp3") XMH_W_ADD("ap0", "i0")
+                         XMH_W_ADD("ap1", "i1") XMH_W_ADD("ap2", "i2") XMH_W_ADD("ap3", "i3")
+                         : [i0] "=&v"(i0), [i1] "=&v"(i1), [i2] "=&v"(i2), [i3] "=&v"(i3)
+                         : [lp0] "v"(lab_p[0]), [lp1] "v"(lab_p[1]), [lp2] "v"(lab_p[2]), [lp3] "v"(lab_p[3]), [ap0] "v"(addr_p[0]), [ap1] "v"(addr_p[1]),
+                           [ap2] "v"(addr_p[2]), [ap3] "v"(addr_p[3]), "v"(live[0]), "v"(live[1]), "v"(live[2])
+                         : "memory");
         };
         auto group = [&](auto gc) {
             constexpr int G = decltype(gc)::value;
@@ -650,8 +606,7 @@
                 }
                 addr_p = addr; d2_p = d2; lab_p = lab;
                 if (G > 0 && h == 0) {
-                    if constexpr (NMI == 4) asm volatile("" ::"v"(A[G > 0 ? G - 1 : 0][0]), "v"(A[G > 0 ? G - 1 : 0][1]), "v"(A[G > 0 ? G - 1 : 0][2]), "v"(A[G > 0 ? G - 1 : 0][3]));
-                    else asm volatile("" ::"v"(A[G > 0 ? G - 1 : 0][0]), "v"(A[G > 0 ? G - 1 : 0][1]), "v"(A[G > 0 ? G - 1 : 0][2]));
+                    asm volatile("" ::"v"(A[G > 0 ? G - 1 : 0][0]), "v"(A[G > 0 ? G - 1 : 0][1]), "v"(A[G > 0 ? G - 1 : 0][2]));
                 }
             }
         };
@@ -707,6 +662,9 @@
     }
     if (CACHE && dmax >= 256u) *ovf = 1u;
 }
+#undef XMH_W_FUSED_PLAIN
+#undef XMH_W_FUSED_CACHE
+#undef XMH_W_MFMA_F4
 #undef XMH_W_MFMA
 #undef XMH_W_MIN
 #undef XMH_W_ADD
@@ -956,28 +914,26 @@
 #define XMH_AP2_SETA "v113", "v115", "v117", "v119", "v[112:113]", "v[114:115]", "v[116:117]", "v[118:119]"
 #define XMH_AP2_SETB "v121", "v123", "v125", "v127", "v[120:121]", "v[122:123]", "v[124:125]", "v[126:127]"
 #define XMH_AP2_MFMA(D, A, B, C) "v_mfma_i32_16x16x64_i8 %[" D "], %[" A "], %[" B "], " C "\n\t"
+#define XMH_AP2_MFMA_F4(D, A, B, C) "v_mfma_f32_16x16x128_f8f6f4 %[" D "], %[" A "], %[" B "], " C " cbsz:4 blgp:4\n\t"
 #define XMH_AP2_MAX(H, L) "v_max_i32 " H ", -1, %[" L "]\n\t"
 #define XMH_AP2_ADD(O, A, P) "ds_add_rtn_u64 %[" O "], %[" A "], " P "\n\t"
-#define XMH_AP2_FUSED2_(H0, H1, H2, H3, P0, P1, P2, P3)                                                                                   \
-    "s_nop 3\n\t" XMH_AP2_MFMA("lab", "a1", "q1", "0") XMH_AP2_MAX(H0, "l0") XMH_AP2_MAX(H1, "l1") XMH_AP2_MAX(H2, "l2")                \
-    XMH_AP2_MFMA("lab", "a2", "q2", "%[lab]") XMH_AP2_MAX(H3, "l3") XMH_AP2_ADD("o0", "p0", P0) XMH_AP2_ADD("o1", "p1", P1)            \
-    XMH_AP2_MFMA("addr", "a0", "q0", "%[c0]") XMH_AP2_ADD("o2", "p2", P2) XMH_AP2_ADD("o3", "p3", P3)
-#define XMH_AP2_FUSED1_(H0, H1, H2, H3, P0, P1, P2, P3)                                                                                   \
-    "s_nop 3\n\t" XMH_AP2_MFMA("lab", "a1", "q1", "0") XMH_AP2_MAX(H0, "l0") XMH_AP2_MAX(H1, "l1") XMH_AP2_MAX(H2, "l2") XMH_AP2_MAX(H3, "l3") \
+#define XMH_AP2_FUSED_(LAB, H0, H1, H2, H3, P0, P1, P2, P3)                                                                              \
+    "s_nop 3\n\t" LAB("lab", "a1", "q1", "0") XMH_AP2_MAX(H0, "l0") XMH_AP2_MAX(H1, "l1") XMH_AP2_MAX(H2, "l2") XMH_AP2_MAX(H3, "l3")    \
     XMH_AP2_MFMA("addr", "a0", "q0", "%[c0]") XMH_AP2_ADD("o0", "p0", P0) XMH_AP2_ADD("o1", "p1", P1) XMH_AP2_ADD("o2", "p2", P2)       \
     XMH_AP2_ADD("o3", "p3", P3)
 #define XMH_AP2_TAIL_(H0, H1, H2, H3, P0, P1, P2, P3)                                                                                     \
     XMH_AP2_MAX(H0, "l0") XMH_AP2_MAX(H1, "l1") XMH_AP2_MAX(H2, "l2") XMH_AP2_MAX(H3, "l3") XMH_AP2_ADD("o0", "p0", P0)                   \
     XMH_AP2_ADD("o1", "p1", P1) XMH_AP2_ADD("o2", "p2", P2) XMH_AP2_ADD("o3", "p3", P3)
-#define XMH_AP2_FUSED2(...) XMH_AP2_FUSED2_(__VA_ARGS__)
-#define XMH_AP2_FUSED1(...) XMH_AP2_FUSED1_(__VA_ARGS__)
+#define XMH_AP2_FUSED(...) XMH_AP2_FUSED_(__VA_ARGS__)
 #define XMH_AP2_TAIL(...) XMH_AP2_TAIL_(__VA_ARGS__)
 template <int NML, int NW, int NQ, bool CAPPED>
 __global__ __launch_bounds__(64 * NW) void k_scan_ap_r2(MfmaArgs a, const uint2* __restrict__ below, const uint2* __restrict__ dpre,
                                                         const uint32_t* __restrict__ cap_ws, float* __restrict__ ap_part,
                                                         const uint32_t* __restrict__ items_total, uint32_t kcap) {
     using u64 = unsigned long long;
-    constexpr int NMI = 1 + NML;
+    static_assert(NML == 1 || NML == 2, "one i8 label tile (at most 64 classes) or one FP4 label tile (65-128 classes)");
+    constexpr bool F4 = NML == 2;
+    constexpr int NMI = 2;
     extern __shared__ __attribute__((aligned(16))) uint32_t lds[];
     int chunk_id, qtile;
     if (!mfma_map_block(a, chunk_id, qtile)) return;
@@ -1014,7 +970,7 @@
             c[cell(e)] = pack(pb[at], pd[at]);
         }
     }
-    v4i bq[NQ], bl[NQ][NML], cq[NQ];
+    v4i bq[NQ], bl[NQ], cq[NQ];
     float capf[NQ], acc[NQ];
     const int rsh = 4 * (slot & 1), rwi = slot >> 1;
 #pragma unroll
@@ -1035,13 +991,14 @@
             if (j & 1) bq[h][j] = on ? (int)(0x20202020u ^ (t * 0xc0u)) : 0;
             else bq[h][j] = on ? (int)(0x40404040u ^ (t << 7)) : 0;
         }
-#pragma unroll
-        for (int m = 0; m < NML; ++m) {
+        if constexpr (F4) {
+            bl[h] = label_query_f4(valid && slot < a.LW ? a.qlab[q * a.LW + slot] : 0u, 0xAu);
+        } else {
             uint32_t lw = 0u;
-            if (valid && 2 * m + rwi < a.LW) lw = a.qlab[q * a.LW + 2 * m + rwi];
+            if (valid && rwi < a.LW) lw = a.qlab[q * a.LW + rwi];
             lw >>= rsh;
 #pragma unroll
-            for (int j = 0; j < 4; ++j) bl[h][m][j] = (int)(((lw >> j) & 0x01010101u) * 0xffu);
+            for (int j = 0; j < 4; ++j) bl[h][j] = (int)(((lw >> j) & 0x01010101u) * 0xffu);
         }
         const int c0 = (int)(uint32_t)(uintptr_t)(__attribute__((address_space(3))) u64*)(cnt + h * ncell) + ql * 8 + (valid ? 128 * pcq : 0);
         cq[h] = v4i{c0, c0, c0, c0};
@@ -1056,9 +1013,8 @@
     uint32_t wcur[4][NMI], wnxt[4][NMI];
     const int ritem = 4 * (lane & 3) + ((lane & 15) >> 2);
     const int wi_c = rwi < a.W ? rwi : a.W - 1;
-    int wi_l[NML];
-#pragma unroll
-    for (int m = 0; m < NML; ++m) wi_l[m] = 2 * m + rwi < a.LW ? 2 * m + rwi : (a.LW > 0 ? a.LW - 1 : 0);
+    const int lwi = F4 ? slot : rwi;
+    const int wi_l = lwi < a.LW ? lwi : (a.LW > 0 ? a.LW - 1 : 0);
     auto load_words = [&](int64_t batch, uint32_t (&w)[4][NMI]) {
         const int64_t first = batch * 64;
         if (first + 64 <= (int64_t)a.R) {
@@ -1067,8 +1023,7 @@
 #pragma unroll
             for (int g = 0; g < 4; ++g) {
                 w[g][0] = pc[g * 16 * a.W];
-#pragma unroll
-                for (int m = 0; m < NML; ++m) w[g][1 + m] = pl[g * 16 * a.LW + wi_l[m]];
+                w[g][1] = pl[g * 16 * a.LW + wi_l];
             }
         } else {
 #pragma unroll
@@ -1077,8 +1032,7 @@
                 const int64_t it = item < a.R ? item : (int64_t)a.R - 1;
                 const uint32_t ok = item < a.R ? 0xffffffffu : 0u;
                 w[g][0] = a.rbits[it * a.W + wi_c] & ok;
-#pragma unroll
-                for (int m = 0; m < NML; ++m) w[g][1 + m] = a.rlab[it * a.LW + wi_l[m]] & ok;
+                w[g][1] = a.rlab[it * a.LW + wi_l] & ok;
             }
         }
     };
@@ -1089,11 +1043,12 @@
         At[0][1] = (int)(xa & 0x04040404u);
         At[0][2] = (int)(xb & 0x02020202u);
         At[0][3] = (int)(xb & 0x04040404u);
-#pragma unroll
-        for (int m = 1; m < NMI; ++m) {
-            const uint32_t y = w[m] >> rsh;
-#pragma unroll
-            for (int j = 0; j < 4; ++j) At[m][j] = (int)(y & (0x01010101u << j));
+        if constexpr (F4) {
+            At[1] = label_item_f4(w[1]);
+        } else {
+            const uint32_t y = w[1] >> rsh;
+#pragma unroll
+            for (int j = 0; j < 4; ++j) At[1][j] = (int)(y & (0x01010101u << j));
         }
     };
     auto credit = [&](u64 old, uint32_t m, int h) {
@@ -1116,39 +1071,39 @@
         u64 oldA[4], oldB[4];
         v4i addr_p, lab_p;
         auto evaluate = [&](const v4i (&At)[NMI], int h, v4i& addr, v4i& lab) {
-            if constexpr (NML == 2)
-                asm volatile("s_nop 3\n\t" XMH_AP2_MFMA("lab", "a1", "q1", "0") XMH_AP2_MFMA("lab", "a2", "q2", "%[lab]") XMH_AP2_MFMA("addr", "a0", "q0", "%[c0]") "s_nop 7"
+            if constexpr (F4)
+                asm volatile("s_nop 3\n\t" XMH_AP2_MFMA_F4("lab", "a1", "q1", "0") XMH_AP2_MFMA("addr", "a0", "q0", "%[c0]") "s_nop 7"
                              : [lab] "=&v"(lab), [addr] "=&v"(addr)
-                             : [a1] "v"(At[1]), [q1] "v"(bl[h][0]), [a2] "v"(At[NMI - 1]), [q2] "v"(bl[h][NML - 1]), [a0] "v"(At[0]), [q0] "v"(bq[h]), [c0] "v"(cq[h]));
+                             : [a1] "v"(At[1]), [q1] "v"(bl[h]), [a0] "v"(At[0]), [q0] "v"(bq[h]), [c0] "v"(cq[h]));
             else
                 asm volatile("s_nop 3\n\t" XMH_AP2_MFMA("lab", "a1", "q1", "0") XMH_AP2_MFMA("addr", "a0", "q0", "%[c0]") "s_nop 7"
                              : [lab] "=&v"(lab), [addr] "=&v"(addr)
-                             : [a1] "v"(At[1]), [q1] "v"(bl[h][0]), [a0] "v"(At[0]), [q0] "v"(bq[h]), [c0] "v"(cq[h]));
+                             : [a1] "v"(At[1]), [q1] "v"(bl[h]), [a0] "v"(At[0]), [q0] "v"(bq[h]), [c0] "v"(cq[h]));
         };
 #define XMH_AP2_OUTS(OLD) [lab] "=&v"(lab), [addr] "=&v"(addr), [o0] "=&v"(OLD[0]), [o1] "=&v"(OLD[1]), [o2] "=&v"(OLD[2]), [o3] "=&v"(OLD[3])
 #define XMH_AP2_PREV [p0] "v"(addr_p[0]), [p1] "v"(addr_p[1]), [p2] "v"(addr_p[2]), [p3] "v"(addr_p[3]), [l0] "v"(lab_p[0]), [l1] "v"(lab_p[1]), [l2] "v"(lab_p[2]), [l3] "v"(lab_p[3])
         auto fusedA = [&](const v4i (&At)[NMI], int h, v4i& addr, v4i& lab) {
-            if constexpr (NML == 2)
-                asm volatile(XMH_AP2_FUSED2(XMH_AP2_SETA)
+            if constexpr (F4)
+                asm volatile(XMH_AP2_FUSED(XMH_AP2_MFMA_F4, XMH_AP2_SETA)
                              : XMH_AP2_OUTS(oldA), "+{v[112:115]}"(incA01), "+{v[116:119]}"(incA23)
-                             : [a1] "v"(At[1]), [q1] "v"(bl[h][0]), [a2] "v"(At[NMI - 1]), [q2] "v"(bl[h][NML - 1]), [a0] "v"(At[0]), [q0] "v"(bq[h]), [c0] "v"(cq[h]), XMH_AP2_PREV
+                             : [a1] "v"(At[1]), [q1] "v"(bl[h]), [a0] "v"(At[0]), [q0] "v"(bq[h]), [c0] "v"(cq[h]), XMH_AP2_PREV
                              : "memory");
             else
-                asm volatile(XMH_AP2_FUSED1(XMH_AP2_SETA)
+                asm volatile(XMH_AP2_FUSED(XMH_AP2_MFMA, XMH_AP2_SETA)
                              : XMH_AP2_OUTS(oldA), "+{v[112:115]}"(incA01), "+{v[116:119]}"(incA23)
-                             : [a1] "v"(At[1]), [q1] "v"(bl[h][0]), [a0] "v"(At[0]), [q0] "v"(bq[h]), [c0] "v"(cq[h]), XMH_AP2_PREV
+                             : [a1] "v"(At[1]), [q1] "v"(bl[h]), [a0] "v"(At[0]), [q0] "v"(bq[h]), [c0] "v"(cq[h]), XMH_AP2_PREV
                              : "memory");
         };
         auto fusedB = [&](const v4i (&At)[NMI], int h, v4i& addr, v4i& lab) {
-            if constexpr (NML == 2)
-                asm volatile(XMH_AP2_FUSED2(XMH_AP2_SETB)
+            if constexpr (F4)
+                asm volatile(XMH_AP2_FUSED(XMH_AP2_MFMA_F4, XMH_AP2_SETB)
                              : XMH_AP2_OUTS(oldB), "+{v[120:123]}"(incB01), "+{v[124:127]}"(incB23)
-                             : [a1] "v"(At[1]), [q1] "v"(bl[h][0]), [a2] "v"(At[NMI - 1]), [q2] "v"(bl[h][NML - 1]), [a0] "v"(At[0]), [q0] "v"(bq[h]), [c0] "v"(cq[h]), XMH_AP2_PREV
+                             : [a1] "v"(At[1]), [q1] "v"(bl[h]), [a0] "v"(At[0]), [q0] "v"(bq[h]), [c0] "v"(cq[h]), XMH_AP2_PREV
                              : "memory");
             else
-                asm volatile(XMH_AP2_FUSED1(XMH_AP2_SETB)
+                asm volatile(XMH_AP2_FUSED(XMH_AP2_MFMA, XMH_AP2_SETB)
                              : XMH_AP2_OUTS(oldB), "+{v[120:123]}"(incB01), "+{v[124:127]}"(incB23)
-                             : [a1] "v"(At[1]), [q1] "v"(bl[h][0]), [a0] "v"(At[0]), [q0] "v"(bq[h]), [c0] "v"(cq[h]), XMH_AP2_PREV
+                             : [a1] "v"(At[1]), [q1] "v"(bl[h]), [a0] "v"(At[0]), [q0] "v"(bq[h]), [c0] "v"(cq[h]), XMH_AP2_PREV
                              : "memory");
         };
         auto drainA = [&](int h, auto newer) {
@@ -1177,8 +1132,7 @@
             else fusedA(A[G], H, addr, lab);
             addr_p = addr; lab_p = lab;
             if constexpr (G > 0 && H == 0) {
-                if constexpr (NMI == 2) asm volatile("" ::"v"(A[G - 1][0]), "v"(A[G - 1][1]));
-                else asm volatile("" ::"v"(A[G - 1][0]), "v"(A[G - 1][1]), "v"(A[G - 1][NMI - 1]));
+                asm volatile("" ::"v"(A[G - 1][0]), "v"(A[G - 1][1]));
             }
             if constexpr (P >= 2) {
                 if constexpr ((P - 2) & 1) drainB((P - 2) % NQ, N4{});
```

New measurement: 1734 billion pairs/s (median of 6 runs). 4.3% higher.
